# facebookresearch/EgoT2

Measured on AMD Instinct MI355X. Metric: clips/sec fwd+bwd, 3-task TTM translator (B=256,T=15,d=128), higher is better.
Workload: dtype f32 (operands split exactly into 3 bf16 parts; 6 bf16 MFMA products per K-block, f32 accumulate); 1 GPU; configs[1]: TTM 3-task translator, 1 layer d=128 h=4 d_ff=2048, B=256/GPU T=15 S=45, synthetic N(0,1) features, random-init weights, train mode dropout=0.5 (+0.1 on PE), weighted CE (evaluated in the forward's head epilogue), fwd+bwd; global_batch=256, parallelism=dp1, impl=auto, workgroups_per_clip=1, launch=one hipGraph replay per step, deterministic=False, compute_is_module_default=True, loss=weighted CE in the forward's head epilogue (egx_ce)

## Files before the change

### egot2_amd/_lib.py

```python
from __future__ import annotations

import ctypes as C
import os

_PKG = os.path.dirname(os.path.abspath(__file__))
LIB_PATH = os.environ.get("EGX_LIB") or os.path.join(_PKG, "libegot2x.so")

EGX_ABI_VERSION = 18
EGX_MAX_SEGMENTS = 8
EGX_F32, EGX_BF16, EGX_F32_SPLIT = 0, 1, 2
EGX_IMPL_AUTO, EGX_IMPL_GENERIC, EGX_IMPL_FUSED, EGX_IMPL_WIDE, EGX_IMPL_TILED = 0, 1, 2, 3, 4

_fp = C.c_void_p


class Segment(C.Structure):
    _fields_ = [("feat", _fp), ("T", C.c_int), ("d_in", C.c_int), ("proj_w", _fp), ("proj_b", _fp),
                ("add_vec", _fp), ("pos", _fp), ("pos_stride", C.c_int), ("feat_bf16", C.c_int), ("pool", C.c_int)]


class SegmentGrads(C.Structure):
    _fields_ = [("proj_w", _fp), ("proj_b", _fp), ("add_vec", _fp), ("pos", _fp), ("feat", _fp)]


_LAYER_FIELDS = ["in_proj_w", "in_proj_b", "out_proj_w", "out_proj_b", "lin1_w", "lin1_b", "lin2_w", "lin2_b",
                 "norm1_w", "norm1_b", "norm2_w", "norm2_b"]


class Layer(C.Structure):
    _fields_ = [(n, _fp) for n in _LAYER_FIELDS]


class LayerGrads(C.Structure):
    _fields_ = [(n, _fp) for n in _LAYER_FIELDS]


class Head(C.Structure):
    _fields_ = [("ln_w", _fp), ("ln_b", _fp), ("W", _fp), ("b", _fp), ("n_out", C.c_int)]


class HeadGrads(C.Structure):
    _fields_ = [("ln_w", _fp), ("ln_b", _fp), ("W", _fp), ("b", _fp)]


class Config(C.Structure):
    _fields_ = [("d_model", C.c_int), ("n_heads", C.c_int), ("d_ff", C.c_int), ("n_layers", C.c_int),
                ("n_segments", C.c_int), ("ln_eps", C.c_float), ("compute", C.c_int), ("impl", C.c_int),
                ("p_drop", C.c_float), ("p_pos", C.c_float), ("p_feat", C.c_float), ("seed_ptr", _fp),
                ("advance_seed", C.c_int), ("zero_buf", _fp), ("zero_bytes", C.c_size_t), ("bwd_stage", C.c_int),
                ("deterministic", C.c_int), ("out_tokens", C.c_int), ("bucket_cb", C.c_void_p), ("bucket_user", C.c_void_p),
                ("weight_cache", _fp), ("weight_cache_valid", C.c_int), ("d_logits_scale", _fp), ("ce", C.c_void_p),
                ("token_ce", C.c_void_p)]


class Ce(C.Structure):
    _fields_ = [("target", _fp), ("class_weight", _fp), ("loss", _fp), ("d_logits", _fp)]


class TokenCe(C.Structure):
    _fields_ = [("W", _fp), ("b", _fp), ("target", _fp), ("class_weight", _fp), ("C", C.c_int), ("logits", _fp), ("probs", _fp), ("pred", _fp),
                ("loss", _fp), ("correct", _fp), ("d_logits", _fp), ("d_W", _fp), ("d_b", _fp)]


BUCKET_CB = C.CFUNCTYPE(None, C.c_void_p, C.c_int)


class DecConfig(C.Structure):
    _fields_ = [("d_model", C.c_int), ("n_heads", C.c_int), ("d_ff", C.c_int), ("n_layers", C.c_int), ("vocab", C.c_int),
                ("sy", C.c_int), ("S", C.c_int), ("ln_eps", C.c_float), ("compute", C.c_int), ("p_drop", C.c_float),
                ("p_pos", C.c_float), ("seed_ptr", C.c_void_p)]


_DEC_LAYER_FIELDS = ["sa_in_w", "sa_in_b", "sa_out_w", "sa_out_b", "norm1_w", "norm1_b", "ca_in_w", "ca_in_b", "ca_out_w",
                     "ca_out_b", "norm2_w", "norm2_b", "lin1_w", "lin1_b", "lin2_w", "lin2_b", "norm3_w", "norm3_b"]


class DecLayer(C.Structure):
    _fields_ = [(n, _fp) for n in _DEC_LAYER_FIELDS]


class DecLayerGrads(C.Structure):
    _fields_ = [(n, _fp) for n in _DEC_LAYER_FIELDS]


SIGNATURES = {
    "egx_abi_version": (C.c_int, []),
    "egx_last_error": (C.c_char_p, []),
    "egx_launch_count": (C.c_longlong, [C.c_int]),
    "egx_tuning_reload": (None, []),
    "egx_weight_cache_bytes": (C.c_size_t, [C.POINTER(Config), C.POINTER(Segment)]),
    "egx_encoder_workspace": (C.c_int, [C.POINTER(Config), C.POINTER(Segment), C.c_int,
                                        C.POINTER(C.c_size_t), C.POINTER(C.c_size_t)]),
    "egx_encoder_uses_fused": (C.c_int, [C.POINTER(Config), C.POINTER(Segment), C.c_int]),
    "egx_encoder_token_ce_ok": (C.c_int, [C.POINTER(Config), C.POINTER(Segment), C.c_int]),
    "egx_encoder_impl": (C.c_int, [C.POINTER(Config), C.POINTER(Segment), C.c_int]),
    "egx_encoder_slices": (C.c_int, [C.POINTER(Config), C.POINTER(Segment), C.c_int]),
    "egx_wide_gemm_scratch": (C.c_size_t, [C.c_int, C.c_int, C.c_int, C.c_int]),
    "egx_wide_gemm": (C.c_int, [C.c_int, _fp, _fp, _fp, _fp, C.c_int, C.c_int, C.c_int, _fp, C.c_int, _fp, _fp, _fp]),
    "egx_wide_attention_fwd": (C.c_int, [_fp, _fp, _fp, C.c_int, C.c_int, C.c_int, C.c_int, C.c_float, C.c_uint64, _fp]),
    "egx_wide_attention_bwd": (C.c_int, [_fp, _fp, _fp, _fp, _fp, _fp, C.c_int, C.c_int, C.c_int, C.c_int, C.c_float, C.c_uint64, _fp]),
    "egx_encoder_fwd": (C.c_int, [C.POINTER(Config), C.POINTER(Segment), _fp, _fp, C.POINTER(Layer), C.c_int,
                                  _fp, _fp, _fp, C.c_int, C.c_uint64, _fp]),
    "egx_encoder_bwd": (C.c_int, [C.POINTER(Config), C.POINTER(Segment), _fp, _fp, C.POINTER(Layer), C.c_int,
                                  _fp, _fp, _fp, C.POINTER(SegmentGrads), _fp, _fp, C.POINTER(LayerGrads),
                                  C.c_int, C.c_uint64, _fp]),
# ... 142 lines not shown
```

### egot2_amd/csrc/ffn_cut.hip

```cpp
#include <stdlib.h>
#include "common.h"
#include "kernels.h"
#include "fused.h"
#include "fused_dev.h"

namespace egx {

__device__ unsigned long long g_cstamps[32];
#ifdef EGX_STAMPS
#define CSTAMP_INIT() unsigned long long ct_prev = __builtin_amdgcn_s_memtime(), ct_acc[8] = {0, 0, 0, 0, 0, 0, 0, 0}
#define CSTAMP(k) do { __builtin_amdgcn_sched_barrier(0); unsigned long long t_ = __builtin_amdgcn_s_memtime(); ct_acc[k] += t_ - ct_prev; ct_prev = t_; __builtin_amdgcn_sched_barrier(0); } while (0)
#define CSTAMP_FLUSH(base) do { if (blockIdx.x == 0 && (threadIdx.x == 0 || threadIdx.x == 256)) for (int k_ = 0; k_ < 8; ++k_) g_cstamps[(base) + (threadIdx.x >> 8) * 8 + k_] = ct_acc[k_]; } while (0)
#define ASTAMP(i) do { if (blockIdx.x == 0 && threadIdx.x == 0) g_cstamps[i] = __builtin_amdgcn_s_memtime(); } while (0)
#else
#define ASTAMP(i) do { } while (0)
#define CSTAMP_INIT() do { } while (0)
#define CSTAMP(k) do { } while (0)
#define CSTAMP_FLUSH(base) do { } while (0)
#endif
int debug_read_cstamps(unsigned long long* out) {
    return hipMemcpyFromSymbol(out, HIP_SYMBOL(g_cstamps), sizeof(unsigned long long) * 32) == hipSuccess ? 0 : 1;
}
#ifdef EGX_DIAG_NOLOAD
#define RING_REFILL(slot, k, hb, hbn) do { } while (0)
// ... 65 lines not shown
        const int row = i >> 5, c = (i & 31) << 2;
        const f32x4 v = *reinterpret_cast<const f32x4*>(blk + row * LDX + c);
        *reinterpret_cast<uint2*>(plane + row * LDXH + c) = make_uint2(pack_bf16x2(v[0], v[1]), pack_bf16x2(v[2], v[3]));
    }
}
__device__ __forceinline__ void block_to_split_planes(unsigned short* planes, const float* blk) {
    const int row = threadIdx.x >> 2, c0 = (threadIdx.x & 3) * 32;
    if (row < CSP) {
        float g[32];
        uint32_t h[16], m[16], lo[16];
        load32(blk + row * LDX + c0, g);
        split32(g, h, m, lo);
        store_parts32(planes + row * LDXH + c0, (size_t)CPS, h, m, lo);
    }
}

template <int CM, bool FWD>
__device__ __forceinline__ void cut_walk(int wave, int nit, int& j_begin, int& n_mine, int shift_code = 0) {
    const int shift = shift_code ? shift_code - 1 : (CM == CM_BF16 ? 0 : (FWD ? nit / 4 : nit / 8));
    const int n_old = nit + shift;
    j_begin = wave < 4 ? 0 : n_old;
    n_mine = wave < 4 ? n_old : 2 * nit - n_old;
}
constexpr int CP_FLOATS = 1024 + 8 * FD;
constexpr int CP_HEAD_ROWS = 8;
__device__ __forceinline__ int cut_rot(int rot_mode, int clip, int nit) {
    return rot_mode == 0 ? (int)((clip * 11u + (clip >> 3) * 5u) % (unsigned)nit)
         : rot_mode == 4 ? (int)(((unsigned)(clip >> 3) & 3u) % (unsigned)nit)
         : rot_mode == 5 ? (int)(((unsigned)(clip >> 3) & 7u) % (unsigned)nit) : 0;
}

__device__ __forceinline__ void reduce_partials8(f32x4 (&y)[8][CNT], float* blk0, int wave, int r, int q) {
    if (wave >= 4) {
        float* mine = blk0 + (wave - 4) * CBLK;
#pragma unroll
        for (int i = 0; i < 8; ++i)
#pragma unroll
            for (int t = 0; t < CNT; ++t)
                *reinterpret_cast<f32x4*>(mine + (t * 16 + r) * LDX + i * 16 + 4 * q) = y[i][t];
    }
    __syncthreads();
    if (wave < 4) {
        float* mine = blk0 + wave * CBLK;
#pragma unroll
        for (int i = 0; i < 8; ++i)
#pragma unroll
            for (int t = 0; t < CNT; ++t) {
                f32x4* a = reinterpret_cast<f32x4*>(mine + (t * 16 + r) * LDX + i * 16 + 4 * q);
                *a = y[i][t] + *a;
            }
    }
    __syncthreads();
}
}

template <int CM>
__global__ __launch_bounds__(CT) void ffn_fwd_kernel(FusedFwdParams p, int l) {
    extern __shared__ __attribute__((aligned(16))) float lds[];
    float* X1 = lds;
    float* R = lds + CBLK;
    unsigned short* XP = reinterpret_cast<unsigned short*>(R);
    constexpr int NPL = CM == CM_SPLIT ? 3 : 1;
    constexpr int D = RingDepth<CM>::v;
    const int tid = threadIdx.x, wave = tid >> 6, lane = tid & 63, r = lane & 15, q = lane >> 4;
    const int clip = blockIdx.x, S = p.S;
    const size_t tokbase = (size_t)clip * S;
    const FusedLayer& w = p.layer[l];
    const bool dev_seed = p.seed_ptr != nullptr;
    const uint64_t seed_dev = dev_seed ? *p.seed_ptr : 0ull;
    const uint64_t k_ffn = dev_seed ? site_key(seed_dev, l, SITE_FFN) : w.ffn_key;
    const uint64_t k_res2 = dev_seed ? site_key(seed_dev, l, SITE_RES2) : w.res2_key;

    ASTAMP(16);
    Touched tch = {{0, 0, 0, 0}};
    if (p.touch.n) tch = touch_lines<CT>(p.touch, blockIdx.x, gridDim.x, tid);
    const int nhb = p.d_ff / 32;
    int j_begin_, n_mine_;
    cut_walk<CM, true>(wave, nhb / 8, j_begin_, n_mine_, p.rot_mode >> 8);
    const int nit = __builtin_amdgcn_readfirstlane(n_mine_), j_begin = __builtin_amdgcn_readfirstlane(j_begin_);
    const int pair_s = __builtin_amdgcn_readfirstlane(wave & 3);
    const int rot = cut_rot(p.rot_mode & 255, clip, nit);
    auto hb_of = [&](int it) { int j = it + rot; if (j >= nit) j -= nit; return pair_s + 4 * (j_begin + j); };
    float* CP = lds + 5 * CBLK;
    const bool cp_hd = p.head.n_out > 0 && l + 1 == p.n_layers;
    const int cp_g = tid >> 5, cp_c4 = (tid & 31) << 2;
    f32x4 cp_v, cp_w;
    float cp_b;
    {
        const float* src = cp_g == 0 ? w.norm2_w : cp_g == 1 ? w.norm2_b : (cp_g == 3 && cp_hd) ? p.head.ln_w : (cp_g == 4 && cp_hd) ? p.head.ln_b : w.lin2_b;
        cp_v = *reinterpret_cast<const f32x4*>(src + cp_c4);
        const int nb = cp_hd ? p.head.n_out : 0, nw = cp_hd && p.head.n_out <= CP_HEAD_ROWS ? p.head.n_out * 32 : 0;
        cp_b = nb ? p.head.b[min(max(tid - 160, 0), nb - 1)] : 0.f;
        cp_w = *reinterpret_cast<const f32x4*>(nw ? p.head.W + (size_t)min(max(tid - 256, 0), nw - 1) * 4 : w.lin2_b);
    }
    auto cp_store = [&] {
        if (cp_g < 3 || (cp_g < 5 && cp_hd)) *reinterpret_cast<f32x4*>(CP + cp_g * FD + cp_c4) = cp_v;
        if (cp_hd) {
            if (tid >= 160 && tid < 160 + p.head.n_out) CP[5 * FD + (tid - 160)] = cp_b;
            if (p.head.n_out <= CP_HEAD_ROWS && tid >= 256 && tid < 256 + p.head.n_out * 32) *reinterpret_cast<f32x4*>(CP + 1024 + (tid - 256) * 4) = cp_w;
        }
    };
    auto frag_load = [&](int k, int hb) -> WRaw<CM> {
        return k < 8 ? load_w<CM>(w.lin1_wp, hb * 2 + (k & 1), FD / 32, k >> 1, lane) : load_w<CM>(w.lin2_wp, k - 8, nhb, hb, lane);
    };
    WRaw<CM> ring[D];
    float4 b1r[2];
    {
        const int hb0 = hb_of(0);
#pragma unroll
        for (int k = 0; k < D; ++k) ring[k] = frag_load(k, hb0);
#pragma unroll
        for (int i = 0; i < 2; ++i) b1r[i] = *reinterpret_cast<const float4*>(w.lin1_b + hb0 * 32 + i * 16 + 4 * q);
    }
    {
        constexpr int XR = CSP * (FD / 4) / CT;
        constexpr int NPV = CM == CM_F32 ? 1 : (NPL * CSP * (FD / 8) + CT - 1) / CT;
        static_assert(CSP * (FD / 4) % CT == 0, "the x1 block must divide among the threads");
        f32x4 xr[XR];
        u32x4 pv[NPV];
        const f32x4* xs = reinterpret_cast<const f32x4*>(p.x1f_out + ((size_t)l * p.Ntok + tokbase) * FD);
        const int nx = S * (FD / 4);
#pragma unroll
        for (int k = 0; k < XR; ++k) { const int i = tid + CT * k; xr[k] = xs[i < nx ? i : nx - 1]; }
        const bool have_planes = CM != CM_F32 && p.x1p_out != nullptr;
        if constexpr (CM != CM_F32) {
            constexpr int NPIECE = NPL * CSP * (FD / 8);
            const size_t plane = CM == CM_SPLIT ? (size_t)p.B * CSP * FD : 0;
            const unsigned short* src = !have_planes ? reinterpret_cast<const unsigned short*>(p.x1f_out)
                                      : CM == CM_SPLIT ? p.x1p_out + (size_t)l * 3 * plane + (size_t)clip * CSP * FD
                                                       : p.x1p_out + ((size_t)l * p.B + clip) * CSP * FD;
#pragma unroll
            for (int k = 0; k < NPV; ++k) {
                int i = tid + CT * k;
                i = i < NPIECE ? i : NPIECE - 1;
                const int part = i / (CSP * (FD / 8)), rem = i - part * (CSP * (FD / 8));
                pv[k] = *reinterpret_cast<const u32x4*>(src + (have_planes ? part * plane + (size_t)rem * 8 : 0));
            }
        }
        for (int i = tid; i < (CSP - S) * LDX; i += CT) X1[S * LDX + i] = 0.f;
        cp_store();
#pragma unroll
        for (int k = 0; k < XR; ++k) {
            const int i = tid + CT * k, row = i >> 5, c = (i & 31) << 2;
            if (i < nx) *reinterpret_cast<f32x4*>(X1 + row * LDX + c) = xr[k];
        }
        if constexpr (CM != CM_F32) {
            constexpr int NPIECE = NPL * CSP * (FD / 8);
            if (have_planes) {
#pragma unroll
                for (int k = 0; k < NPV; ++k) {
                    const int i = tid + CT * k;
                    const int part = i / (CSP * (FD / 8)), rem = i - part * (CSP * (FD / 8));
                    const int row = rem >> 4, c8 = rem & 15;
                    if (i < NPIECE) {
                        unsigned short* d = XP + part * CPS + row * LDXH + c8 * 8;
                        const bool live = row < S;
                        *reinterpret_cast<uint2*>(d) = live ? make_uint2(pv[k][0], pv[k][1]) : make_uint2(0, 0);
                        *reinterpret_cast<uint2*>(d + 4) = live ? make_uint2(pv[k][2], pv[k][3]) : make_uint2(0, 0);
                    }
                }
            }
        }
        __syncthreads();
        touch_sink(tch);
        if (CM != CM_F32 && !have_planes) {
            if constexpr (CM == CM_SPLIT) block_to_split_planes(XP, X1);
            else if constexpr (CM == CM_BF16) block_to_plane(XP, X1);
            __syncthreads();
        }
    }

    ASTAMP(17);
    f32x4 y[8][CNT];
#pragma unroll
    for (int i = 0; i < 8; ++i)
#pragma unroll
        for (int t = 0; t < CNT; ++t) y[i][t] = f32x4{0, 0, 0, 0};
    const float bscale = w.ffn_thresh ? w.drop_inv : 1.f;
    const size_t bits_base = ((size_t)l * p.B + clip) * nhb * 64 + lane;
    constexpr int ESZ = CM == CM_BF16 ? 2 : 4;
    const int nht = p.d_ff / 16;
    char* const hid_base = (char*)p.hid_out + ((size_t)l * p.B + clip) * CNT * nht * (size_t)(HTILE_ELEMS * ESZ);

    CSTAMP_INIT();
    for (int it = 0; it < nit; ++it) {
        const int hb = hb_of(it);
        const int hbn = hb_of(it + 1 < nit ? it + 1 : it);
        __builtin_amdgcn_sched_barrier(0);
        CSTAMP(0);
        f32x4 hacc[2][CNT];
#pragma unroll
        for (int i = 0; i < 2; ++i)
#pragma unroll
            for (int t = 0; t < CNT; ++t) hacc[i][t] = f32x4{0, 0, 0, 0};
        Frag<CM> xb[CNT];
#pragma unroll
        for (int k = 0; k < 8; ++k) {
            const int i = k & 1, kb = k >> 1;
            if (i == 0) {
#pragma unroll
                for (int t = 0; t < CNT; ++t) xb[t] = operand_frag<CM>(XP, X1, t * 16 + r, kb * 32, q);
            }
            pin(ring[k % D]);
            if (k == 0) { CSTAMP(1); }
            Frag<CM> a = w_frag<CM>(ring[k % D]);
#pragma unroll
            for (int t = 0; t < CNT; ++t) mma<CM>(hacc[i][t], a, xb[t]);
            __builtin_amdgcn_sched_barrier(0);
            RING_REFILL(k % D, k, hb, hbn);
            __builtin_amdgcn_sched_barrier(0);
        }
        CSTAMP(2);
        float bv[2][4];
#pragma unroll
        for (int i = 0; i < 2; ++i) {
            bv[i][0] = b1r[i].x * bscale; bv[i][1] = b1r[i].y * bscale; bv[i][2] = b1r[i].z * bscale; bv[i][3] = b1r[i].w * bscale;
        }
        __builtin_amdgcn_sched_barrier(0);
#pragma unroll
        for (int i = 0; i < 2; ++i) b1r[i] = *reinterpret_cast<const float4*>(w.lin1_b + hbn * 32 + i * 16 + 4 * q);
        __builtin_amdgcn_sched_barrier(0);
        if (w.ffn_thresh) {
#pragma unroll
            for (int i = 0; i < 2; ++i) {
                const uint32_t cq = (uint32_t)(hb * 32 + i * 16 + 4 * q) >> 2;
#pragma unroll
// ... 12 lines not shown
                for (int t = 0; t < CNT; ++t)
#pragma unroll
                    for (int e = 0; e < 4; ++e) hacc[i][t][e] += bv[i][e];
        }
        uint32_t dead = 0;
#pragma unroll
        for (int k = 2 * CNT * 4 - 1; k >= 0; --k) {
            const int i = k / (CNT * 4), t = (k / 4) % CNT, e = k & 3;
            dead = __builtin_amdgcn_alignbit(dead, __float_as_uint(hacc[i][t][e]), 31);
        }
        p.relu_bits[bits_base + (size_t)hb * 64] = ~dead & ((1u << (2 * CNT * 4)) - 1u);
#pragma unroll
        for (int i = 0; i < 2; ++i)
#pragma unroll
            for (int t = 0; t < CNT; ++t)
#pragma unroll
                for (int e = 0; e < 4; ++e) hacc[i][t][e] = __int_as_float(max(__float_as_int(hacc[i][t][e]), 0));
        Frag<CM> hbq[CNT];
#pragma unroll
        for (int t = 0; t < CNT; ++t) hbq[t] = chain_frag<CM>(hacc[0][t], hacc[1][t]);
#ifndef EGX_DIAG_NOSTORE
        {
            char* hb_base = hid_base + (size_t)hb * 2 * (HTILE_ELEMS * ESZ);
#pragma unroll
            for (int t = 0; t < CNT; ++t) {
                if constexpr (CM == CM_BF16) {
                    const u32x4 u = __builtin_bit_cast(u32x4, hbq[t].v);
                    store_hid_tile_bf16(hb_base + (size_t)t * nht * (HTILE_ELEMS * ESZ), u, lane, S - t * 16);
                } else {
#pragma unroll
                    for (int i = 0; i < 2; ++i)
                        store_hid_tile<CM>(hb_base + ((size_t)t * nht + i) * (HTILE_ELEMS * ESZ), hacc[i][t], lane, S - t * 16);
                }
            }
        }
#endif
        __builtin_amdgcn_sched_barrier(0);
        CSTAMP(3);
#pragma unroll
        for (int k = 8; k < 16; ++k) {
            pin(ring[k % D]);
            if (k == 8) { CSTAMP(4); }
            Frag<CM> a = w_frag<CM>(ring[k % D]);
#pragma unroll
            for (int t = 0; t < CNT; ++t) mma<CM>(y[k - 8][t], a, hbq[t]);
            __builtin_amdgcn_sched_barrier(0);
            RING_REFILL(k % D, k, hb, hbn);
            __builtin_amdgcn_sched_barrier(0);
        }
    }
    CSTAMP(5);
    CSTAMP_FLUSH(0);
    ASTAMP(18);
    __syncthreads();
    ASTAMP(19);
    reduce_partials8(y, R, wave, r, q);
    ASTAMP(20);

    for (int i = tid; i < S * (FD / 4); i += CT) {
        const int row = i >> 5, c = (i & 31) << 2, o = row * LDX + c;
        const f32x4 a0 = *reinterpret_cast<const f32x4*>(R + o), a1 = *reinterpret_cast<const f32x4*>(R + CBLK + o);
        const f32x4 a2 = *reinterpret_cast<const f32x4*>(R + 2 * CBLK + o), a3 = *reinterpret_cast<const f32x4*>(R + 3 * CBLK + o);
        f32x4 f = ((a0 + a1) + (a2 + a3)) + *reinterpret_cast<const f32x4*>(CP + 2 * FD + c);
        if (w.res_thresh) {
            float m4[4];
            drop_scale4(k_res2, (uint32_t)(tokbase + row), (uint32_t)c, w.res_thresh, w.drop_inv, m4);
            f = f * f32x4{m4[0], m4[1], m4[2], m4[3]};
        }
        *reinterpret_cast<f32x4*>(X1 + o) = f + *reinterpret_cast<const f32x4*>(X1 + o);
    }
    __syncthreads();
    ASTAMP(21);
    const bool last = l + 1 == p.n_layers;
    float* Y = R;
    ln_rows(X1, S, CP, CP + FD, p.eps, [&](int row, int c0, float (&x)[32], float (&yv)[32]) {
        if (last && p.tokens_out && row < p.out_T) store32(p.tokens_out + ((size_t)clip * p.out_T + row) * FD + c0, yv);
        store32(Y + row * LDX + c0, yv);
    }, [&] { rows_from_lds(p.saved_res + ((size_t)(2 * l + 1) * p.B + clip) * S * FD, X1, S); });
    __syncthreads();
    ASTAMP(22);
    if (!last) {
        rows_from_lds(p.xin_out + ((size_t)(l + 1) * p.B + clip) * S * FD, Y, S);
        return;
    }
    if (p.head.n_out > 0) {
        float* pooled = X1;
        const FusedCe ce{p.ce_target, p.ce_weight, p.ce_loss, p.ce_dlogits, p.ce_B, nullptr};
        CeReq rq;
        if (ce.target) { ce_request_labels<CT>(ce, tid, rq); ce_request_weights(ce, p.head.n_out, rq); }
        if (tid < FD) pooled[tid] = colsum_lds(Y, 0, S, tid) * (1.f / (float)S);
        if (ce.target) ce_weight_partials<CT>(ce, p.head.n_out, tid, rq, pooled + 256);
        __syncthreads();
        if (wave == 0) {
            float2 x = *reinterpret_cast<float2*>(pooled + 2 * lane);
            float mean = wsum(x.x + x.y) * (1.f / FD);
            float dx = x.x - mean, dy = x.y - mean;
            float rstd = rsqrtf(wsum(dx * dx + dy * dy) * (1.f / FD) + p.eps);
            float2 lw = *reinterpret_cast<const float2*>(CP + 3 * FD + 2 * lane);
            float2 lb = *reinterpret_cast<const float2*>(CP + 4 * FD + 2 * lane);
            float y0 = dx * rstd * lw.x + lb.x, y1 = dy * rstd * lw.y + lb.y;
            const bool w_lds = p.head.n_out <= CP_HEAD_ROWS;
            float zmine = 0.f;
            for (int o = 0; o < p.head.n_out; ++o) {
                float2 wv = w_lds ? *reinterpret_cast<const float2*>(CP + 1024 + o * FD + 2 * lane) : *reinterpret_cast<const float2*>(p.head.W + (size_t)o * FD + 2 * lane);
                float sdot = wsum(y0 * wv.x + y1 * wv.y) + CP[5 * FD + o];
                if (lane == 0) p.logits_out[(size_t)clip * p.head.n_out + o] = sdot;
                zmine = lane == o ? sdot : zmine;
            }
            if (ce.target) ce_clip<CT>(ce, p.head.n_out, clip, lane, zmine, pooled + 256, true);
        }
    }
    ASTAMP(23);
}

template <int CM>
__global__ __launch_bounds__(CT) void ffn_bwd_kernel(FusedBwdParams p, int l) {
    extern __shared__ __attribute__((aligned(16))) float lds[];
    float* B1 = lds;
    float* Gs = lds + 1 * CBLK;
    float* B2 = lds + 2 * CBLK;
    float* B3 = lds + 3 * CBLK;
    float* B4 = lds + 4 * CBLK;
    unsigned short* GP = reinterpret_cast<unsigned short*>(B3);
    constexpr int D = RingDepth<CM>::v;
    const int tid = threadIdx.x, wave = tid >> 6, lane = tid & 63, r = lane & 15, q = lane >> 4;
    const int clip = blockIdx.x, S = p.S;
    const size_t tok0 = (size_t)clip * S;
    const FusedBwdLayer& w = p.layer[l];
    const bool dev_seed = p.seed_ptr != nullptr;
    const uint64_t seed_dev = dev_seed ? *p.seed_ptr : 0ull;
    const uint64_t k_res2 = dev_seed ? site_key(seed_dev, l, SITE_RES2) : w.res2_key;
    const bool last = l + 1 == p.n_layers;

    ASTAMP(24);
    Touched tch = {{0, 0, 0, 0}};
    if (p.touch.n) tch = touch_lines<CT>(p.touch, blockIdx.x, gridDim.x, tid);
    if (p.zero_buf) {
        const size_t n4 = p.zero_n / 4, per = (n4 + gridDim.x - 1) / gridDim.x;
        const size_t b0 = (size_t)blockIdx.x * per, b1 = b0 + per < n4 ? b0 + per : n4;
        for (size_t k = b0 + threadIdx.x; k < b1; k += CT) reinterpret_cast<float4*>(p.zero_buf)[k] = make_float4(0, 0, 0, 0);
    }
    float* part = p.partials + (size_t)clip * p.P;
    float* pl = part + l * FUSED_P_LAYER;

    const int nhb = p.d_ff / 32;
    int j_begin_, n_mine_;
    cut_walk<CM, false>(wave, nhb / 8, j_begin_, n_mine_, p.rot_mode >> 8);
    const int nit = __builtin_amdgcn_readfirstlane(n_mine_), j_begin = __builtin_amdgcn_readfirstlane(j_begin_);
    const int pair_s = __builtin_amdgcn_readfirstlane(wave & 3);
    const int rot = cut_rot(p.rot_mode & 255, clip, nit);
    auto hb_of = [&](int it) { int j = it + rot; if (j >= nit) j -= nit; return pair_s + 4 * (j_begin + j); };
    float* CP = lds + 5 * CBLK;
    const bool cp_hd = p.head.n_out > 0 && last;
    const int cp_g = tid >> 5, cp_c4 = (tid & 31) << 2;
    f32x4 cp_v, cp_w;
    float cp_b;
    {
        const float* src = cp_g == 1 ? w.norm2_b : (cp_g == 3 && cp_hd) ? p.head.ln_w : (cp_g == 4 && cp_hd) ? p.head.ln_b : w.norm2_w;
        cp_v = *reinterpret_cast<const f32x4*>(src + cp_c4);
        const int nb = cp_hd ? p.head.n_out : 0, nw = cp_hd && p.head.n_out <= CP_HEAD_ROWS ? p.head.n_out * 32 : 0;
        cp_b = nb ? p.d_logits[(size_t)clip * p.head.n_out + min(max(tid - 160, 0), nb - 1)] : 0.f;
        if (nb && p.d_logits_scale) cp_b *= *p.d_logits_scale;
        cp_w = *reinterpret_cast<const f32x4*>(nw ? p.head.W + (size_t)min(max(tid - 256, 0), nw - 1) * 4 : w.norm2_w);
    }
    auto cp_store = [&] {
        if (cp_g < 2 || ((cp_g == 3 || cp_g == 4) && cp_hd)) *reinterpret_cast<f32x4*>(CP + cp_g * FD + cp_c4) = cp_v;
        if (cp_hd) {
            if (tid >= 160 && tid < 160 + p.head.n_out) CP[5 * FD + 64 + (tid - 160)] = cp_b;
            if (p.head.n_out <= CP_HEAD_ROWS && tid >= 256 && tid < 256 + p.head.n_out * 32) *reinterpret_cast<f32x4*>(CP + 1024 + (tid - 256) * 4) = cp_w;
        }
    };
    auto frag_load = [&](int k, int hb) -> WRaw<CM> {
        return k < 8 ? load_w<CM>(w.lin2_wtp, hb * 2 + (k & 1), FD / 32, k >> 1, lane) : load_w<CM>(w.lin1_wtp, k - 8, nhb, hb, lane);
    };
    const uint32_t* relu_bits = p.relu_bits + ((size_t)l * p.B + clip) * (size_t)nhb * 64 + lane;
    WRaw<CM> ring[D];
    uint32_t relu_word;
    {
        const int hb0 = hb_of(0);
#pragma unroll
        for (int k = 0; k < D; ++k) ring[k] = frag_load(k, hb0);
        relu_word = relu_bits[(size_t)hb0 * 64];
    }
    const float* res2 = p.saved_res + ((size_t)(2 * l + 1) * p.B + clip) * S * FD;
    const bool head_bwd = last && p.head.n_out > 0;
    {
        constexpr int XR = CSP * (FD / 4) / CT;
        f32x4 rr[XR], dr[XR];
        const f32x4* rs = reinterpret_cast<const f32x4*>(res2);
        const int ndy_rows = head_bwd ? 0 : (last ? p.out_T : S);
        const f32x4* ds = head_bwd ? rs : reinterpret_cast<const f32x4*>(last ? p.d_tokens + (size_t)clip * p.out_T * FD : p.dxin + tok0 * FD);
        const int nx = S * (FD / 4), nd = ndy_rows * (FD / 4);
#pragma unroll
        for (int k = 0; k < XR; ++k) {
            const int i = tid + CT * k;
            rr[k] = rs[i < nx ? i : nx - 1];
            dr[k] = ds[i < nd ? i : (nd > 0 ? nd - 1 : 0)];
        }
        for (int i = tid; i < 5 * CBLK / 4; i += CT) reinterpret_cast<f32x4*>(lds)[i] = f32x4{0, 0, 0, 0};
        cp_store();
        __syncthreads();
#pragma unroll
        for (int k = 0; k < XR; ++k) {
            const int i = tid + CT * k, row = i >> 5, c = (i & 31) << 2;
            if (i < nx) {
                *reinterpret_cast<f32x4*>(B1 + row * LDX + c) = rr[k];
                if (head_bwd) *reinterpret_cast<f32x4*>(Gs + row * LDX + c) = rr[k];
            }
            if (i < nd) *reinterpret_cast<f32x4*>(Gs + row * LDX + c) = dr[k];
        }
        touch_sink(tch);
    }
    ASTAMP(25);
    if (head_bwd) {
        float* hp = part + p.head_off;
        __syncthreads();
        ln_rows(Gs, S, CP, CP + FD, p.eps, [&](int row, int c0, float (&x)[32], float (&y)[32]) { store32(Gs + row * LDX + c0, y); });
        __syncthreads();
        float* pooled = B2;
        if (tid < FD) pooled[tid] = colsum_lds(Gs, 0, S, tid) * (1.f / (float)S);
        __syncthreads();
        if (wave == 0) {
            float2 x = *reinterpret_cast<float2*>(pooled + 2 * lane);
            float mean = wsum(x.x + x.y) * (1.f / FD);
            float xh0 = x.x - mean, xh1 = x.y - mean;
            float rstd = rsqrtf(wsum(xh0 * xh0 + xh1 * xh1) * (1.f / FD) + p.eps);
            xh0 *= rstd; xh1 *= rstd;
            float2 lw = *reinterpret_cast<const float2*>(CP + 3 * FD + 2 * lane);
            float2 lb = *reinterpret_cast<const float2*>(CP + 4 * FD + 2 * lane);
            float y0 = xh0 * lw.x + lb.x, y1 = xh1 * lw.y + lb.y;
            float d0 = 0.f, d1 = 0.f;
            const bool w_lds = p.head.n_out <= CP_HEAD_ROWS;
            for (int o = 0; o < p.head.n_out; ++o) {
                float go = CP[5 * FD + 64 + o];
                float2 wv = w_lds ? *reinterpret_cast<const float2*>(CP + 1024 + o * FD + 2 * lane) : *reinterpret_cast<const float2*>(p.head.W + (size_t)o * FD + 2 * lane);
                d0 += go * wv.x; d1 += go * wv.y;
                *reinterpret_cast<float2*>(hp + 256 + FUSED_HEAD_MAX_OUT + o * FD + 2 * lane) = make_float2(go * y0, go * y1);
                if (lane == 0) hp[256 + o] = go;
            }
            *reinterpret_cast<float2*>(hp + 2 * lane) = make_float2(d0 * xh0, d1 * xh1);
            *reinterpret_cast<float2*>(hp + 128 + 2 * lane) = make_float2(d0, d1);
            float g0 = d0 * lw.x, g1 = d1 * lw.y;
            float s1 = wsum(g0 + g1) * (1.f / FD);
            float s2 = wsum(g0 * xh0 + g1 * xh1) * (1.f / FD);
            float inv_s = 1.f / (float)S;
            *reinterpret_cast<float2*>(pooled + 128 + 2 * lane) =
                make_float2(rstd * (g0 - s1 - xh0 * s2) * inv_s, rstd * (g1 - s1 - xh1 * s2) * inv_s);
        }
        __syncthreads();
        f32x4 dp[1];
        {
            const int c = (tid & 31) << 2;
            dp[0] = *reinterpret_cast<const f32x4*>(pooled + 128 + c);
        }
        __syncthreads();
        for (int i = tid; i < S * (FD / 4); i += CT) {
            const int row = i >> 5, c = (i & 31) << 2;
            *reinterpret_cast<f32x4*>(Gs + row * LDX + c) = dp[0];
        }
        if (tid < 64) *reinterpret_cast<f32x4*>(B2 + 4 * tid) = f32x4{0, 0, 0, 0};
    }
    __syncthreads();
    ASTAMP(26);
    ln_bwd_rows(S, CP, p.eps,
        [&](int row, int c0, float (&dy)[32], float (&x)[32]) { load32(Gs + row * LDX + c0, dy); load32(B1 + row * LDX + c0, x); },
        [&](int row, int c0, float (&dy)[32], float (&dx)[32], float (&dyx)[32]) {
            store32(B1 + row * LDX + c0, dx);
            store32(B3 + row * LDX + c0, dyx);
            if (w.res_thresh) {
                const uint32_t orow = (uint32_t)(tok0 + row);
#pragma unroll
                for (int j = 0; j < 32; ++j) dx[j] *= drop_scale(k_res2, orow, (uint32_t)(c0 + j), w.res_thresh, w.drop_inv);
            }
            store32(B2 + row * LDX + c0, dx);
        });
    __syncthreads();
    if (tid < 128) pl[0 + tid] = colsum_lds(B3, 0, S, tid);
    else if (tid < 256) pl[128 + (tid - 128)] = colsum_lds(Gs, 0, S, tid - 128);
    else if (tid < 384) pl[256 + (tid - 256)] = colsum_lds(B2, 0, S, tid - 256);
    if (!(CM != CM_F32 && p.xg_planes)) rows_from_lds(w.g2_out + tok0 * FD, B2, S);
    __syncthreads();
    if constexpr (CM == CM_SPLIT) block_to_split_planes(GP, B2);
    else if constexpr (CM == CM_BF16) block_to_plane(GP, B2);
    __syncthreads();
    if (CM != CM_F32 && p.xg_planes) {
        if constexpr (CM == CM_SPLIT) {
            const size_t plane = (size_t)p.B * CSP * FD;
            planes_from_lds<3>(reinterpret_cast<unsigned short*>(w.g2_out) + (size_t)clip * CSP * FD, plane, GP);
        } else {
            planes_from_lds<1>(reinterpret_cast<unsigned short*>(w.g2_out) + (size_t)clip * CSP * FD, 0, GP);
        }
    }

    ASTAMP(27);
    f32x4 dxa[8][CNT];
#pragma unroll
    for (int i = 0; i < 8; ++i)
#pragma unroll
        for (int t = 0; t < CNT; ++t) dxa[i][t] = f32x4{0, 0, 0, 0};
    constexpr int ESZ = CM == CM_BF16 ? 2 : 4;
    const int nht = p.d_ff / 16;
    char* const dhid_base = (char*)p.dhid_out + ((size_t)l * p.B + clip) * CNT * nht * (size_t)(HTILE_ELEMS * ESZ);
    for (int it = 0; it < nit; ++it) {
        const int hb = hb_of(it);
        const int hbn = hb_of(it + 1 < nit ? it + 1 : it);
        __builtin_amdgcn_sched_barrier(0);
        f32x4 dacc[2][CNT];
#pragma unroll
        for (int i = 0; i < 2; ++i)
#pragma unroll
            for (int t = 0; t < CNT; ++t) dacc[i][t] = f32x4{0, 0, 0, 0};
        Frag<CM> gb[CNT];
#pragma unroll
        for (int k = 0; k < 8; ++k) {
            const int i = k & 1, kb = k >> 1;
            if (i == 0) {
#pragma unroll
                for (int t = 0; t < CNT; ++t) gb[t] = operand_frag<CM>(GP, B2, t * 16 + r, kb * 32, q);
            }
            pin(ring[k % D]);
            Frag<CM> a2 = w_frag<CM>(ring[k % D]);
#pragma unroll
            for (int t = 0; t < CNT; ++t) mma<CM>(dacc[i][t], a2, gb[t]);
            __builtin_amdgcn_sched_barrier(0);
            RING_REFILL(k % D, k, hb, hbn);
            __builtin_amdgcn_sched_barrier(0);
        }
        const uint32_t bits = relu_word;
        __builtin_amdgcn_sched_barrier(0);
        relu_word = relu_bits[(size_t)hbn * 64];
        __builtin_amdgcn_sched_barrier(0);
#pragma unroll
        for (int i = 0; i < 2; ++i)
#pragma unroll
            for (int t = 0; t < CNT; ++t)
#pragma unroll
                for (int e = 0; e < 4; ++e) {
                    const int k = (i * CNT + t) * 4 + e;
                    const int32_t m = ((int32_t)(bits << (31 - k))) >> 31;
                    dacc[i][t][e] = __uint_as_float(__float_as_uint(dacc[i][t][e]) & (uint32_t)m);
                }
        Frag<CM> dq_[CNT];
#pragma unroll
        for (int t = 0; t < CNT; ++t) dq_[t] = chain_frag<CM>(dacc[0][t], dacc[1][t]);
        {
            char* hb_base = dhid_base + (size_t)hb * 2 * (HTILE_ELEMS * ESZ);
#pragma unroll
            for (int t = 0; t < CNT; ++t) {
                if constexpr (CM == CM_BF16) {
                    const u32x4 u = __builtin_bit_cast(u32x4, dq_[t].v);
                    store_hid_tile_bf16(hb_base + (size_t)t * nht * (HTILE_ELEMS * ESZ), u, lane, S - t * 16);
                } else {
#pragma unroll
                    for (int i = 0; i < 2; ++i)
                        store_hid_tile<CM>(hb_base + ((size_t)t * nht + i) * (HTILE_ELEMS * ESZ), dacc[i][t], lane, S - t * 16);
                }
            }
        }
        __builtin_amdgcn_sched_barrier(0);
#pragma unroll
        for (int k = 8; k < 16; ++k) {
            pin(ring[k % D]);
            Frag<CM> a = w_frag<CM>(ring[k % D]);
#pragma unroll
            for (int t = 0; t < CNT; ++t) mma<CM>(dxa[k - 8][t], a, dq_[t]);
            __builtin_amdgcn_sched_barrier(0);
            RING_REFILL(k % D, k, hb, hbn);
            __builtin_amdgcn_sched_barrier(0);
        }
    }
    ASTAMP(28);
    __syncthreads();
    ASTAMP(29);
    reduce_partials8(dxa, Gs, wave, r, q);
    ASTAMP(30);
    {
        f32x4* dst = reinterpret_cast<f32x4*>(p.dy1 + tok0 * FD);
        for (int i = tid; i < S * (FD / 4); i += CT) {
            const int o = (i >> 5) * LDX + ((i & 31) << 2);
            const f32x4 a0 = *reinterpret_cast<const f32x4*>(Gs + o), a1 = *reinterpret_cast<const f32x4*>(B2 + o);
            const f32x4 a2 = *reinterpret_cast<const f32x4*>(B3 + o), a3 = *reinterpret_cast<const f32x4*>(B4 + o);
            dst[i] = (((a0 + a1) + a2) + a3) + *reinterpret_cast<const f32x4*>(B1 + o);
        }
    }
    ASTAMP(31);
}

bool ffn_cut_supported(int d_ff) { return d_ff % 256 == 0 && d_ff >= 256; }
size_t ffn_cut_lds_bytes() { return (size_t)(5 * CBLK + CP_FLOATS) * sizeof(float); }

template <int CM>
static int launch_cut_fwd(const FusedFwdParams& p, int l, hipStream_t st) {
    const size_t lds = ffn_cut_lds_bytes();
    static bool attr_set = false;
    if (!attr_set) {
        EGX_HIP(hipFuncSetAttribute(reinterpret_cast<const void*>(&ffn_fwd_kernel<CM>), hipFuncAttributeMaxDynamicSharedMemorySize, (int)lds));
        attr_set = true;
    }
    timing_begin(TIMER_FFN_FWD, st);
    hipLaunchKernelGGL((ffn_fwd_kernel<CM>), dim3(p.B), dim3(CT), lds, st, p, l);
    timing_end(TIMER_FFN_FWD, st);
    EGX_LAUNCH_CHECK();
    return 0;
}
template <int CM>
static int launch_cut_bwd(const FusedBwdParams& p, int l, hipStream_t st) {
    const size_t lds = ffn_cut_lds_bytes();
    static bool attr_set = false;
    if (!attr_set) {
        EGX_HIP(hipFuncSetAttribute(reinterpret_cast<const void*>(&ffn_bwd_kernel<CM>), hipFuncAttributeMaxDynamicSharedMemorySize, (int)lds));
        attr_set = true;
    }
    timing_begin(TIMER_FFN_BWD, st);
    hipLaunchKernelGGL((ffn_bwd_kernel<CM>), dim3(p.B), dim3(CT), lds, st, p, l);
    timing_end(TIMER_FFN_BWD, st);
    EGX_LAUNCH_CHECK();
    return 0;
}

int ffn_cut_forward(const FusedFwdParams& p, int l, int compute, hipStream_t st) {
    EGX_CHECK(ffn_cut_supported(p.d_ff) && p.S <= CSP && l >= 0 && l < p.n_layers, "ffn_cut_forward: d_ff=%d S=%d layer %d", p.d_ff, p.S, l);
    EGX_CHECK(p.x1f_out && p.xin_out && p.saved_res && p.relu_bits && p.hid_out, "ffn_cut_forward: missing buffers");
    return compute == CM_BF16 ? launch_cut_fwd<CM_BF16>(p, l, st) : compute == CM_SPLIT ? launch_cut_fwd<CM_SPLIT>(p, l, st) : launch_cut_fwd<CM_F32>(p, l, st);
}
int ffn_cut_backward(const FusedBwdParams& p, int l, int compute, hipStream_t st) {
    EGX_CHECK(ffn_cut_supported(p.d_ff) && p.S <= CSP && l >= 0 && l < p.n_layers, "ffn_cut_backward: d_ff=%d S=%d layer %d", p.d_ff, p.S, l);
    EGX_CHECK(p.dy1 && p.saved_res && p.relu_bits && p.dhid_out && p.partials && (l + 1 == p.n_layers || p.dxin), "ffn_cut_backward: missing buffers");
    return compute == CM_BF16 ? launch_cut_bwd<CM_BF16>(p, l, st) : compute == CM_SPLIT ? launch_cut_bwd<CM_SPLIT>(p, l, st) : launch_cut_bwd<CM_F32>(p, l, st);
}

}
```

### egot2_amd/csrc/fused.h

```cpp
#pragma once
#include "common.h"

namespace egx {

constexpr int FUSED_MAX_SEG = 4;
constexpr int FUSED_MAX_LAYERS = 6;

constexpr int TOUCH_MAX = 4;
struct TouchList { const void* base[TOUCH_MAX]; unsigned lines[TOUCH_MAX]; int n; };
static inline void touch_add(TouchList& t, const void* base, size_t bytes) {
    if (base && bytes >= 128 && t.n < TOUCH_MAX) { t.base[t.n] = base; t.lines[t.n] = (unsigned)(bytes >> 7); ++t.n; }
}

struct FusedSeg {
    const float* feat;
    const void* proj_wp;
    const float* proj_b;
    const float* add_vec;
    const float* pos;
    int T, d_in, off, pos_stride;
    int row0, Tfull;
    int seg_id, pad_;
};

// ... 6 lines not shown
    const float* norm2_w; const float* norm2_b;
    uint64_t attn_key, res1_key, ffn_key, res2_key;
    uint32_t attn_thresh, res_thresh, ffn_thresh;
    float drop_inv;
};

struct FusedHead {
    const float* ln_w; const float* ln_b;
    const float* W; const float* b;
    int n_out;
};
constexpr int FUSED_HEAD_MAX_OUT = 64;
static inline int fused_head_partial_len(int n_out) { return n_out > 0 ? 256 + FUSED_HEAD_MAX_OUT + n_out * 128 : 0; }

struct FusedFwdParams {
    FusedSeg seg[FUSED_MAX_SEG];
    FusedLayer layer[FUSED_MAX_LAYERS];
    const float* ln_w; const float* ln_b;
    float eps;
    int nseg, n_layers, B, S, d_ff;
    int rot_mode;
    float* tokens_out;
    int out_T;
    FusedHead head; float* logits_out;
    float* saved_pre;
    float* saved_res;
    uint32_t* relu_bits;
    void* hid_out;
    unsigned short* x1p_out;
    float* xin_out;
    float* qkv_out;
    uint64_t pos_key; uint32_t pos_thresh; float pos_inv;
    const uint64_t* seed_ptr;
    uint64_t feat_key[FUSED_MAX_SEG]; uint32_t feat_thresh; float feat_inv;
    int n_heads;
    int tpc, S_clip;
    size_t Ntok;
    int mode, l0;
    const float* attn_in;
    int n_slices;
    float* xchg;
    unsigned* xflags;
    int slice_drop;
    float* x1f_out;
    const int64_t* ce_target; const float* ce_weight; float* ce_loss; float* ce_dlogits; int ce_B;
    float* zero_word;
    const float* tce_W; const float* tce_b; const int64_t* tce_target; const float* tce_cw; int tce_C;
    float* tce_logits; float* tce_probs; float* tce_pred; float* tce_loss; float* tce_correct; float* tce_dlogits;
    unsigned* tce_ticket;
    unsigned* ce_ticket;
    TouchList touch;
    const int* rtab; int B_clips;
};
enum { FUSED_MODE_FULL = 0, FUSED_MODE_PRE = 1, FUSED_MODE_POST = 2, FUSED_MODE_ATTN = 3 };

struct PackDesc {
    const float* src; void* dst;
    int R, K, ld, transpose, first_block;
    float scale;
};
constexpr int PACK_MAX = 56;
struct PackParams {
    PackDesc d[PACK_MAX];
    int n, mode;
    uint64_t* seed_advance;
    unsigned* zero_words; int n_zero;
    float* zero_word2;
    unsigned* zero_ctl;
};
int pack_weights(PackParams& pp, hipStream_t st);
static inline size_t packed_bytes(int R, int K, int mode) { return (size_t)R * K * (mode == 1 ? 2 : mode == 2 ? 6 : 4); }

struct FfnDwParams {
    const float* x1;
    const float* g;
    const void* w1p;
    const void* w2tp;
    const float* b1;
    int N, S, d_ff;
    uint64_t drop_key; uint32_t drop_thresh; float drop_inv;
    const uint64_t* seed_ptr; int layer;
    const void* hs; const void* dhs; int B;
    int xg_planes;
    float* slab_w1; float* slab_w2t; float* slab_b1;
    int splits, kb_per_split;
};
constexpr int FUSED_TOK_TILES = 3;
constexpr int FUSED_TOK_PAD = FUSED_TOK_TILES * 16;
static inline size_t fused_hid_bytes(int B, int d_ff, int bf16) {
    return (size_t)B * FUSED_TOK_TILES * (d_ff / 16) * 256 * (bf16 ? 2 : 4);
}
size_t ffn_dw_scratch_bytes(int N, int d_ff, int* splits_out);
constexpr int FFN_ROT_XCD_STAGGER = 4;
struct ReducePartialsParams;
constexpr int SLAB_REDUCE_MAX = 3 * FUSED_MAX_LAYERS;
struct SlabReduce { const float* slab[SLAB_REDUCE_MAX]; float* out[SLAB_REDUCE_MAX]; size_t n[SLAB_REDUCE_MAX]; int nslab, narr; };
int ffn_dw(FfnDwParams p, int compute, float* dW1, float* db1, float* dW2, void* slabs, hipStream_t st,
           const ReducePartialsParams* rp = nullptr, bool deterministic = false, SlabReduce* defer = nullptr);
int ffn_dw_reduce(const SlabReduce& a, const ReducePartialsParams* rp, bool deterministic, hipStream_t st);

struct FusedBwdLayer {
    const void* in_proj_wp;
    const void* in_proj_wtp;
    const void* out_proj_wtp;
    const void* lin1_wp;
    const void* lin2_wtp;
    const void* lin1_wtp;
    const float* in_proj_b; const float* lin1_b;
    const float* norm1_w; const float* norm1_b; const float* norm2_w; const float* norm2_b;
    uint64_t attn_key, res1_key, ffn_key, res2_key;
    uint32_t attn_thresh, res_thresh, ffn_thresh;
    float drop_inv;
    float* x1_out; float* g2_out; float* attn_o_out; float* g1_out; float* x_in_out; float* dqkv_out;
};

constexpr int FUSED_P_LAYER = 1152;
static inline int fused_partial_len(int L, int nseg) { return L * FUSED_P_LAYER + 256 + nseg * 256; }

struct FusedBwdParams {
    FusedSeg seg[FUSED_MAX_SEG];
    float* dseg_out[FUSED_MAX_SEG];
    FusedBwdLayer layer[FUSED_MAX_LAYERS];
    const float* ln_w; const float* ln_b;
    float eps;
    int nseg, n_layers, B, S, d_ff;
    int rot_mode;
    const float* d_tokens;
    int out_T;
    FusedHead head; const float* d_logits; int head_off;
    const float* pooled;
    const float* saved_pre;
    const float* saved_res;
    const float* saved_qkv;
    const uint32_t* relu_bits;
    int xg_planes;
    void* dhid_out;
    float* zero_buf; size_t zero_n;
    float* partials; int P;
    uint64_t pos_key; uint32_t pos_thresh; float pos_inv;
    const uint64_t* seed_ptr;
    uint64_t feat_key[FUSED_MAX_SEG]; uint32_t feat_thresh; float feat_inv;
    int n_heads;
    float* dx0_out;
    int tpc, S_clip; size_t Ntok;
    int tiled, l_front, l_back;
    float* datt;
    float* dres;
    int n_slices; float* xchg; unsigned* xflags; int slice_drop;
    int cut, cut_layer;
    float* dy1;
    float* dxin;
    const float* d_logits_scale;
    const float* tce_W; const float* tce_dlogits; int tce_C;
    TouchList touch;
    const int* rtab; int B_clips; const int* rseg;
};
int fused_backward(const FusedBwdParams& p, int compute, hipStream_t st);
bool ffn_cut_supported(int d_ff);
size_t ffn_cut_lds_bytes();
int ffn_cut_forward(const FusedFwdParams& p, int l, int compute, hipStream_t st);
int ffn_cut_backward(const FusedBwdParams& p, int l, int compute, hipStream_t st);

struct SmallDwProblem {
    const float* G; const float* X; float* out;
    int R, C, K, ldg, ldx, first_block, splits;
};
constexpr int SMALL_DW_MAX = 8;
struct SmallDwParams {
    SmallDwProblem pr[SMALL_DW_MAX];
    int n, per;
    float* slabs;
};
int small_dw(SmallDwParams& p, int compute, hipStream_t st, void* slabs = nullptr, size_t slab_bytes = 0, bool reduce_here = true);
int seed_advance(uint64_t* seed, hipStream_t st);

struct PartialDst { float* dst; int off, len; };
constexpr int PARTIAL_MAX_DST = 64;
struct ReducePartialsParams {
    PartialDst d[PARTIAL_MAX_DST];
    int n, B, P;
    const float* partials;
};
int reduce_partials(const ReducePartialsParams& rp, hipStream_t st, bool deterministic = false);
struct SmallDwTail { SlabReduce red; ReducePartialsParams rp; unsigned slab_blocks; int rp_units, chunks; uint64_t* seed_advance;  TouchList touch;  };
int tail_reduce(const SmallDwParams* sp, const SlabReduce* red, const ReducePartialsParams* rp, uint64_t* seed_advance_ptr, const TouchList* touch, hipStream_t st);

enum { TIMER_FUSED_FWD = 0, TIMER_FUSED_BWD = 1, TIMER_FFN_DW = 2, TIMER_FFN_FWD = 3, TIMER_FFN_BWD = 4, TIMER_WIDE_GEMM = 5,
       TIMER_WIDE_ATTN_FWD = 6, TIMER_WIDE_ATTN_BWD = 7, TIMER_COUNT = 8 };
void timing_enable(int on);
void timing_begin(int which, hipStream_t st);
void timing_end(int which, hipStream_t st);
int timing_read(int which, double* total_ms, int* count);

struct TiledAttnParams {
    const float* qkv;
    float* attn_o;
    float* lse;
    const float* d_o;
    float* delta;
    float* dqkv;
    int B, S, tpc;
    uint64_t drop_key; uint32_t drop_thresh; float drop_inv;
    const uint64_t* seed_ptr; int layer;
    const int* rtab;
};
constexpr int TILED_MAX_S = 512;
constexpr int RAGGED_REC = 16;
enum { RG_TILE0 = 0, RG_S = 1, RG_TOK0 = 2, RG_OUT0 = 3, RG_OUTN = 4, RG_T = 5 , RG_OFF = 9  };
static_assert(RG_OFF + FUSED_MAX_SEG <= RAGGED_REC, "ragged clip record");
int upload_words(int* dst, const int* src, size_t n, hipStream_t st);
int ragged_rows(float* padded, float* packed, const int* rtab, const int* rseg, int B, int T_pad, int C, int k, int to_packed, hipStream_t st);
int tiled_attn_fwd(const TiledAttnParams& p, int compute, hipStream_t st);
int tiled_attn_bwd(const TiledAttnParams& p, int compute, hipStream_t st);

bool fused_supported(int d_model, int n_heads, int d_ff, int S, int nseg, const int* d_in, const int* T, const bool* has_proj);
size_t fused_lds_bytes(int NT);
long long slices_stolen_fwd(int reset);
long long slices_stolen_bwd(int reset);
int debug_read_stamps(unsigned long long* out, int n);
int debug_read_bstamps(unsigned long long* out, int n);
int fused_forward(const FusedFwdParams& p, int compute, hipStream_t st);

}
```

### egot2_amd/csrc/fused.hip

```cpp
#include "common.h"
#include "kernels.h"
#include "fused.h"
#include "fused_dev.h"
#include <stdlib.h>
#include <string.h>
#include <type_traits>
#include <vector>

namespace egx {

__global__ __launch_bounds__(64) void pack_weights_kernel(PackParams pp) {
    int blk = blockIdx.x;
    if (pp.seed_advance && blk == 0 && threadIdx.x == 0)
        *pp.seed_advance = *pp.seed_advance * 6364136223846793005ull + 1442695040888963407ull;
    if (pp.zero_words)
        for (int i = blk * 64 + threadIdx.x; i < pp.n_zero; i += gridDim.x * 64) pp.zero_words[i] = 0u;
    if (pp.zero_word2 && blk == 0 && threadIdx.x == 0) *pp.zero_word2 = 0.f;
    if (pp.zero_ctl && blk == 0 && threadIdx.x < 8) pp.zero_ctl[threadIdx.x] = 0u;
    if (pp.n == 0) return;
    int di = 0;
    while (di + 1 < pp.n && blk >= pp.d[di + 1].first_block) ++di;
    const PackDesc& d = pp.d[di];
    int local = blk - d.first_block;
    int nkb = d.K / 32;
// ... 1016 lines not shown
        if (lane == 0) { red[4 + wave] = lterm; red[8 + wave] = cterm; }
        __syncthreads();
        STAMP(13);
        if (tid == 0) {
            const float l = ((red[4] + red[5]) + (red[6] + red[7])) * inv, cn = (red[8] + red[9]) + (red[10] + red[11]);
            float* tacc = reinterpret_cast<float*>(p.tce_ticket + 1);
            atomicAdd(tacc, l);
            __threadfence();
            const unsigned mine = 1u + ((unsigned)cn << 12);
            const unsigned old = atomicAdd(p.tce_ticket, mine);
            if ((old & 4095u) == (unsigned)p.B - 1u) {
                __threadfence();
                *p.tce_loss = atomicExch(tacc, 0.f);
                if (p.tce_correct) *p.tce_correct = (float)((old + mine) >> 12);
                atomicExch(p.tce_ticket, 0u);
            }
        }
        STAMP(14);
    }

    if (!TILED && p.head.n_out > 0) {
        float* pooled = X1;
        const FusedCe ce{p.ce_target, p.ce_weight, p.ce_loss, p.ce_dlogits, p.ce_B, p.ce_ticket};
        CeReq rq;
        if (ce.target) { ce_request_labels<256>(ce, tid, rq); ce_request_weights(ce, p.head.n_out, rq); }
        if (tid < FD) pooled[tid] = colsum_lds(Xs, 0, S, tid) * (1.f / (float)S);
        if (ce.target) ce_weight_partials<256>(ce, p.head.n_out, tid, rq, pooled + 256);
        __syncthreads();
        if (wave == 0) {
            float2 x = *reinterpret_cast<float2*>(pooled + 2 * lane);
            float mean = wsum(x.x + x.y) * (1.f / FD);
            float dx = x.x - mean, dy = x.y - mean;
            float rstd = rsqrtf(wsum(dx * dx + dy * dy) * (1.f / FD) + p.eps);
            float2 lw = *reinterpret_cast<const float2*>(p.head.ln_w + 2 * lane);
            float2 lb = *reinterpret_cast<const float2*>(p.head.ln_b + 2 * lane);
            float y0 = dx * rstd * lw.x + lb.x, y1 = dy * rstd * lw.y + lb.y;
            float zmine = 0.f;
            for (int o = 0; o < p.head.n_out; ++o) {
                float2 wv = *reinterpret_cast<const float2*>(p.head.W + (size_t)o * FD + 2 * lane);
                float sdot = wsum(y0 * wv.x + y1 * wv.y) + p.head.b[o];
                if (lane == 0) p.logits_out[(size_t)clip * p.head.n_out + o] = sdot;
                zmine = lane == o ? sdot : zmine;
            }
            if (ce.target) ce_clip<256>(ce, p.head.n_out, clip, lane, zmine, pooled + 256, slice == 0);
        }
    }
}

namespace {
struct TimerSlot { std::vector<hipEvent_t> a, b; int n = 0; };
TimerSlot g_timers[TIMER_COUNT];
int g_timing_on = 0;
constexpr int TIMER_MAX_EVENTS = 4096;
}
void timing_enable(int on) {
    g_timing_on = on;
    for (int i = 0; i < TIMER_COUNT; ++i) g_timers[i].n = 0;
}
void timing_begin(int which, hipStream_t st) {
    if (!g_timing_on) return;
    TimerSlot& t = g_timers[which];
    if (t.n >= TIMER_MAX_EVENTS) return;
    if ((int)t.a.size() <= t.n) {
        hipEvent_t ea, eb;
        (void)hipEventCreate(&ea); (void)hipEventCreate(&eb);
        t.a.push_back(ea); t.b.push_back(eb);
    }
    (void)hipEventRecord(t.a[t.n], st);
}
void timing_end(int which, hipStream_t st) {
    if (!g_timing_on) return;
    TimerSlot& t = g_timers[which];
    if (t.n < (int)t.a.size() && t.n < TIMER_MAX_EVENTS) { (void)hipEventRecord(t.b[t.n], st); ++t.n; }
}
int timing_read(int which, double* total_ms, int* count) {
    if (which < 0 || which >= TIMER_COUNT) return 1;
    TimerSlot& t = g_timers[which];
    double tot = 0;
    for (int i = 0; i < t.n; ++i) {
        float ms = 0.f;
        if (hipEventSynchronize(t.b[i]) != hipSuccess || hipEventElapsedTime(&ms, t.a[i], t.b[i]) != hipSuccess) return 1;
        tot += ms;
    }
    if (total_ms) *total_ms = tot;
    if (count) *count = t.n;
    return 0;
}

size_t fused_lds_bytes(int NT) {
    int SP = NT * 16;
    return (size_t)(4 * SP * LDX + FD * LDV) * sizeof(float) + FUSED_MAX_SEG * sizeof(FusedSeg) + 16 + 21 * FD * sizeof(float);
}

bool fused_supported(int d_model, int n_heads, int d_ff, int S, int nseg, const int* d_in, const int* T, const bool* has_proj) {
    if (d_model != FD || (n_heads != FH && n_heads != 2 * FH)) return false;
    if (d_ff % 128 != 0 || d_ff < 128) return false;
    if (S < 1 || S > 48) return false;
    for (int i = 0; i < nseg; ++i) {
        if (!has_proj[i]) return false;
        if (d_in[i] % 128 != 0) return false;
        if (T[i] < 1) return false;
    }
    return true;
}

template <int CM, bool TILED, int DH>
static int launch_fwd(const FusedFwdParams& p, hipStream_t st) {
    EGX_CHECK(p.S <= 48, "fused: S=%d unsupported", p.S);
    const size_t lds = fused_lds_bytes(3);
    static bool attr_set = false;
    if (!attr_set) {
        EGX_HIP(hipFuncSetAttribute(reinterpret_cast<const void*>(&fused_fwd_kernel<CM, 3, TILED, DH>), hipFuncAttributeMaxDynamicSharedMemorySize, (int)lds));
        if constexpr (!TILED)
            EGX_HIP(hipFuncSetAttribute(reinterpret_cast<const void*>(&fused_fwd_kernel<CM, 3, false, DH, true>), hipFuncAttributeMaxDynamicSharedMemorySize, (int)lds));
        attr_set = true;
    }
    timing_begin(TIMER_FUSED_FWD, st);
    bool sliced = false;
    if constexpr (!TILED) sliced = p.n_slices > 1;
    if constexpr (!TILED) {
        if (p.mode == FUSED_MODE_ATTN) {
            static bool cut_attr = false;
            if (!cut_attr) {
                EGX_HIP(hipFuncSetAttribute(reinterpret_cast<const void*>(&fused_fwd_kernel<CM, 3, false, DH, false, true>), hipFuncAttributeMaxDynamicSharedMemorySize, (int)lds));
                cut_attr = true;
            }
            EGX_CHECK(!sliced && p.x1f_out, "cut mode: one workgroup per clip, x1f_out set");
            hipLaunchKernelGGL((fused_fwd_kernel<CM, 3, false, DH, false, true>), dim3(p.B), dim3(256), lds, st, p);
            timing_end(TIMER_FUSED_FWD, st);
            EGX_LAUNCH_CHECK();
            return 0;
        }
    }
    if (sliced) {
        if constexpr (!TILED)
            hipLaunchKernelGGL((fused_fwd_kernel<CM, 3, false, DH, true>), dim3((p.B + 7) / 8 * 8 * p.n_slices), dim3(256), lds, st, p);
    } else {
        hipLaunchKernelGGL((fused_fwd_kernel<CM, 3, TILED, DH>), dim3(p.B), dim3(256), lds, st, p);
// ... 53 lines not shown
```

### egot2_amd/csrc/fused_dev.h

```cpp
#pragma once
#include "common.h"
#include "fused.h"

namespace egx {

constexpr int FD = 128;
constexpr int FH = 4;
constexpr int FDH = 32;
constexpr int LDX = FD + 4;
constexpr int LDV = 64 + 4;

enum { CM_F32 = 0, CM_BF16 = 1, CM_SPLIT = 2 };
typedef uint32_t u32x4 __attribute__((ext_vector_type(4)));

template <int CM> struct Frag { float v[8]; };
template <> struct Frag<CM_BF16> { bf16x8 v; };
template <> struct Frag<CM_SPLIT> { bf16x8 p[3]; };

__device__ __forceinline__ uint32_t pack_bf16(float a, float b) { return pack_bf16x2(a, b); }

__device__ __forceinline__ void split_pair(float x, float y, uint32_t& h, uint32_t& m, uint32_t& l) {
    typedef float f32x2 __attribute__((ext_vector_type(2)));
    h = pack_bf16(x, y);
    f32x2 v = {x, y};
// ... 259 lines not shown
        t.v[k] = *reinterpret_cast<const uint32_t*>(reinterpret_cast<const char*>(tl.base[kk]) + ((size_t)i << 7));
    }
    return t;
}
__device__ __forceinline__ void touch_sink(const Touched& t) {
#pragma unroll
    for (int k = 0; k < TOUCH_MAX; ++k) asm volatile("" :: "v"(t.v[k]));
}

__device__ __forceinline__ float wmax(float v) {
#pragma unroll
    for (int o = 32; o > 0; o >>= 1) v = fmaxf(v, __shfl_xor(v, o, 64));
    return v;
}

struct FusedCe {
    const int64_t* target;
    const float* class_weight;
    float* loss;
    float* d_logits;
    int B;
    unsigned* ticket;
};
struct CeReq { int64_t y[2]; float w[2]; };
template <int NTHREADS>
__device__ __forceinline__ void ce_request_labels(const FusedCe& ce, int tid, CeReq& rq) {
#pragma unroll
    for (int k = 0; k < 2; ++k) { const int i = tid + k * NTHREADS; rq.y[k] = ce.target[i < ce.B ? i : ce.B - 1]; }
}
__device__ __forceinline__ void ce_request_weights(const FusedCe& ce, int n_out, CeReq& rq) {
#pragma unroll
    for (int k = 0; k < 2; ++k) {
        const int64_t y = rq.y[k];
        const int yc = (y >= 0 && y < n_out) ? (int)y : 0;
        rq.w[k] = ce.class_weight ? ce.class_weight[yc] : 1.f;
    }
}
template <int NTHREADS>
__device__ __forceinline__ void ce_weight_partials(const FusedCe& ce, int n_out, int tid, const CeReq& rq, float* red) {
    float s = 0.f;
#pragma unroll
    for (int k = 0; k < 2; ++k) {
        const int i = tid + k * NTHREADS;
        s += (i < ce.B && rq.y[k] >= 0 && rq.y[k] < n_out) ? rq.w[k] : 0.f;
    }
    for (int i = tid + 2 * NTHREADS; i < ce.B; i += NTHREADS) {
        const int64_t y = ce.target[i];
        if (y >= 0 && y < n_out) s += ce.class_weight ? ce.class_weight[y] : 1.f;
    }
    s = wsum(s);
    if ((tid & 63) == 0) red[tid >> 6] = s;
}
template <int NTHREADS>
__device__ __forceinline__ void ce_clip(const FusedCe& ce, int n_out, int clip, int lane, float z, const float* red, bool add_loss) {
    float wtot = 0.f;
#pragma unroll
    for (int w = 0; w < NTHREADS / 64; ++w) wtot += red[w];
    const int64_t y = ce.target[clip];
    const bool valid = y >= 0 && y < n_out;
    const float wy = valid ? (ce.class_weight ? ce.class_weight[y] : 1.f) : 0.f;
    const float zl = lane < n_out ? z : -INFINITY;
    const float m = wmax(zl);
    const float e = lane < n_out ? __expf(zl - m) : 0.f;
    const float s = wsum(e);
    const float zy = __shfl(zl, valid ? (int)y : 0, 64);
    const float k = wy / wtot;
    if (lane < n_out) ce.d_logits[(size_t)clip * n_out + lane] = valid ? k * (e / s - (lane == (int)y ? 1.f : 0.f)) : 0.f;
    if (lane == 0 && add_loss) {
        float term = valid ? k * (m + __logf(s) - zy) : 0.f;
        if (wtot == 0.f && clip == 0) term = __builtin_nanf("");
        if (!ce.ticket) {
            atomicAdd(ce.loss, term);
        } else {
            float* acc = reinterpret_cast<float*>(ce.ticket + 1);
            atomicAdd(acc, term);
            __threadfence();
            if (atomicInc(ce.ticket, (unsigned)ce.B - 1u) == (unsigned)ce.B - 1u) {
                __threadfence();
                *ce.loss = atomicExch(acc, 0.f);
            }
        }
    }
}


__device__ __forceinline__ float quad_sum4(float v) {
    v += __shfl_xor(v, 1, 64);
    v += __shfl_xor(v, 2, 64);
    return v;
}
template <class Fn, class Hook>
__device__ __forceinline__ void ln_rows(const float* buf, int S, const float* __restrict__ w, const float* __restrict__ b,
                                        float eps, Fn&& fn, Hook&& after_w) {
    const int row = threadIdx.x >> 2, part = threadIdx.x & 3;
    const int c0 = part * 32;
    f32x4 wq[8], bq[8];
#pragma unroll
    for (int j = 0; j < 8; ++j) {
        wq[j] = *reinterpret_cast<const f32x4*>(w + c0 + 4 * j);
        bq[j] = *reinterpret_cast<const f32x4*>(b + c0 + 4 * j);
    }
    after_w();
    if (row < S) {
        float x[32], y[32];
        float s = 0.f;
#pragma unroll
        for (int j = 0; j < 8; ++j) {
            float4 v = *reinterpret_cast<const float4*>(buf + row * LDX + c0 + 4 * j);
            x[4 * j] = v.x; x[4 * j + 1] = v.y; x[4 * j + 2] = v.z; x[4 * j + 3] = v.w;
            s += (v.x + v.y) + (v.z + v.w);
        }
        float mean = quad_sum4(s) * (1.f / FD);
        float ss = 0.f;
#pragma unroll
        for (int j = 0; j < 32; ++j) { float t = x[j] - mean; ss += t * t; }
        float rstd = rsqrtf(quad_sum4(ss) * (1.f / FD) + eps);
#pragma unroll
        for (int j = 0; j < 8; ++j) {
#pragma unroll
            for (int e = 0; e < 4; ++e) y[4 * j + e] = (x[4 * j + e] - mean) * rstd * wq[j][e] + bq[j][e];
        }
        fn(row, c0, x, y);
    } else {
        (void)quad_sum4(0.f);
        (void)quad_sum4(0.f);
    }
}
template <class Fn>
__device__ __forceinline__ void ln_rows(const float* buf, int S, const float* __restrict__ w, const float* __restrict__ b,
                                        float eps, Fn&& fn) {
    ln_rows(buf, S, w, b, eps, fn, [] {});
}
template <class Fn, class Hook>
__device__ __forceinline__ void ln_rows_lds(const float* buf, int S, const float* wl, const float* bl, float eps, Fn&& fn, Hook&& hook) {
    const int row = threadIdx.x >> 2, part = threadIdx.x & 3;
// ... 310 lines not shown
```

### egot2_amd/csrc/fused_host.hip

```cpp
#include <string.h>
#include <vector>

#include "../../include/egot2x.h"
#include "common.h"
#include "kernels.h"
#include "fused.h"
#include "fused_host.h"

namespace egx {

bool packed_feats(const egx_segment* segs, int nseg) {
    for (int i = 0; i < nseg; ++i)
        if (segs[i].feat_bf16 || segs[i].pool > 1) return true;
    return false;
}
bool fused_ok(const egx_config* cfg, const egx_segment* segs, const Plan& pl) {
    if (pl.nseg > FUSED_MAX_SEG || pl.L > FUSED_MAX_LAYERS || pl.L < 1) return false;
    if (packed_feats(segs, pl.nseg)) return false;
    int d_in[EGX_MAX_SEGMENTS], T[EGX_MAX_SEGMENTS];
    bool hp[EGX_MAX_SEGMENTS];
    for (int i = 0; i < pl.nseg; ++i) { d_in[i] = segs[i].d_in; T[i] = segs[i].T; hp[i] = segs[i].proj_w != nullptr; }
    return fused_supported(pl.d, pl.H, pl.dff, pl.S, pl.nseg, d_in, T, hp);
}
static size_t fused_mask_words(const Plan& pl) { return (size_t)pl.L * pl.vB * (pl.dff / 32) * 64; }
// ... 8 lines not shown
    FusedPackLayout L;
    memset(&L, 0, sizeof(L));
    int bf = cfg->compute;
    size_t cur = 0;
    auto take_p = [&](int R, int K) -> void* { void* q = base ? base + cur : nullptr; cur += align_up(packed_bytes(R, K, bf), 256); return q; };
    for (int i = 0; i < pl.nseg; ++i) L.proj[i] = take_p(pl.d, segs[i].d_in);
    for (int l = 0; l < pl.L && l < FUSED_MAX_LAYERS; ++l) {
        L.layer[l].in_w = take_p(3 * pl.d, pl.d);
        L.layer[l].in_wt = take_p(pl.d, 3 * pl.d);
        L.layer[l].out_w = take_p(pl.d, pl.d);
        L.layer[l].out_wt = take_p(pl.d, pl.d);
        L.layer[l].lin1_w = take_p(pl.dff, pl.d);
        L.layer[l].lin1_wt = take_p(pl.d, pl.dff);
        L.layer[l].lin2_w = take_p(pl.d, pl.dff);
        L.layer[l].lin2_wt = take_p(pl.dff, pl.d);
    }
    L.bytes = cur;
    return L;
}
static char* fused_pack_base(const egx_config* cfg, const void* saved, const Plan& vp) {
    return cfg->weight_cache ? (char*)cfg->weight_cache : (char*)const_cast<void*>(saved) + fused_act_bytes(vp);
}
static size_t fused_hid_total(const egx_config* cfg, const Plan& pl) {
    return align_up((size_t)pl.L * fused_hid_bytes(pl.vB, pl.dff, cfg->compute == EGX_BF16), 256);
}
static size_t fused_hid_offset(const egx_config* cfg, const egx_segment* segs, const Plan& pl) {
    return align_up(fused_act_bytes(pl) + fused_pack_layout(cfg, segs, pl, nullptr).bytes, 256);
}
static bool split_planes(const egx_config* cfg) {
    return cfg->compute == EGX_F32_SPLIT || cfg->compute == EGX_BF16;
}
static size_t plane_elem_bytes(const egx_config* cfg) { return cfg->compute == EGX_BF16 ? 2 : 6; }
static size_t fused_x1p_offset(const egx_config* cfg, const egx_segment* segs, const Plan& pl) {
    return fused_hid_offset(cfg, segs, pl) + fused_hid_total(cfg, pl);
}
static size_t fused_xin_offset(const egx_config* cfg, const egx_segment* segs, const Plan& pl) {
    return fused_x1p_offset(cfg, segs, pl) + (split_planes(cfg) ? align_up((size_t)pl.L * pl.vB * FUSED_TOK_PAD * pl.d * plane_elem_bytes(cfg), 256) : 0);
}
static size_t fused_qkv_offset(const egx_config* cfg, const egx_segment* segs, const Plan& pl) {
    return fused_xin_offset(cfg, segs, pl) + align_up((size_t)pl.L * pl.N * pl.d * 4, 256);
}
static size_t fused_x1f_offset(const egx_config* cfg, const egx_segment* segs, const Plan& pl) {
    return fused_qkv_offset(cfg, segs, pl) + align_up((size_t)pl.L * pl.vB * FUSED_TOK_PAD * 3 * pl.d * 4, 256);
}
static size_t fused_core_bytes(const egx_config* cfg, const egx_segment* segs, const Plan& pl) {
    return fused_x1f_offset(cfg, segs, pl) + (pl.tpc > 1 ? (size_t)0 : align_up((size_t)pl.L * pl.N * pl.d * 4, 256));
}
static bool use_cut(const Plan& pl, int n_slices, bool tiled, int compute) {
    if (tiled || n_slices != 1 || !ffn_cut_supported(pl.dff)) return false;
    if (tuning().ffn_cut >= 0) return tuning().ffn_cut != 0;
    return compute == EGX_F32_SPLIT && pl.L == 1 && pl.dff >= 1024;
}
static int fused_slices_layout(const Plan& pl);
static size_t sliced_xchg_bytes(const Plan& pl, int n);
static size_t sliced_flag_bytes(const Plan& pl, int n);
static size_t fused_saved_bytes(const egx_config* cfg, const egx_segment* segs, const Plan& pl) {
    const int n = (pl.tpc > 1 || pl.S > FUSED_TOK_PAD) ? 1 : fused_slices_layout(pl);
    return fused_core_bytes(cfg, segs, pl) + sliced_xchg_bytes(pl, n) + sliced_flag_bytes(pl, n);
}
static int device_cus() {
    static int cus[64] = {0};
    int dev = 0;
    if (hipGetDevice(&dev) != hipSuccess || dev < 0 || dev >= 64) return 0;
    if (!cus[dev]) {
        int v = 0;
        if (hipDeviceGetAttribute(&v, hipDeviceAttributeMultiprocessorCount, dev) != hipSuccess) return 0;
        cus[dev] = v;
    }
    return cus[dev];
}
static int slice_drop_mask(int n) {
    if (!tuning().has_drop) return 0;
    const int m = (int)tuning().slice_drop & ((1 << n) - 1);
    return m == (1 << n) - 1 ? 0 : m;
}
static bool device_slicing_ok() {
    static int ok[64] = {0};
    int dev = 0;
    if (hipGetDevice(&dev) != hipSuccess || dev < 0 || dev >= 64) return false;
    if (!ok[dev]) {
        hipDeviceProp_t pr;
        ok[dev] = (hipGetDeviceProperties(&pr, dev) == hipSuccess && (strncmp(pr.gcnArchName, "gfx950", 6) == 0 || strncmp(pr.gcnArchName, "gfx942", 6) == 0)) ? 1 : 2;
    }
    return ok[dev] == 1;
}
constexpr int SLICE_LAYOUT_CUS = 304;
static int fused_slices_layout(const Plan& pl) {
    const int nit = pl.dff / 128, bq = (pl.B + 7) / 8 * 8;
    int n = 1;
    while (n * 2 <= 8 && nit % (n * 2) == 0 && bq * n * 2 <= SLICE_LAYOUT_CUS) n *= 2;
    return n;
}
int fused_slices(const Plan& pl, int compute) {
    if (!device_slicing_ok()) return 1;
    const bool e = tuning().has_slices;
    int cap = e ? tuning().slices_cap : (compute == EGX_BF16 ? 4 : 8);
    if (cap < 1) cap = 1;
    const int cus = device_cus(), nit = pl.dff / 128, bq = (pl.B + 7) / 8 * 8;
    int n = 1;
    while (n * 2 <= cap && n * 2 <= 8 && nit % (n * 2) == 0 && bq * n * 2 <= cus) n *= 2;
    if (compute == EGX_BF16 && n == 2 && !e) n = 1;
    const int cap_layout = fused_slices_layout(pl);
    return n < cap_layout ? n : cap_layout;
}
static size_t sliced_xchg_bytes(const Plan& pl, int n) { return n > 1 ? align_up((size_t)pl.L * pl.B * n * FUSED_TOK_PAD * pl.d * 4, 256) : 0; }
static size_t sliced_flag_words(const Plan& pl) { return (size_t)pl.L * pl.B * 8; }
static size_t sliced_flag_bytes(const Plan& pl, int n) { return n > 1 ? align_up(2 * sliced_flag_words(pl) * 4, 256) : 0; }

static void plan_tiled(Plan& pl) { pl.tpc = cdiv(pl.S, FUSED_TOK_PAD); pl.vB = pl.B * pl.tpc; }
static size_t tiled_attn_offset(const egx_config* cfg, const egx_segment* segs, const Plan& vp) { return align_up(fused_saved_bytes(cfg, segs, vp), 256); }
static size_t tiled_lse_offset(const egx_config* cfg, const egx_segment* segs, const Plan& vp) { return tiled_attn_offset(cfg, segs, vp) + align_up((size_t)vp.L * vp.N * vp.d * 4, 256); }
static size_t tiled_tokens_offset(const egx_config* cfg, const egx_segment* segs, const Plan& vp) { return tiled_lse_offset(cfg, segs, vp) + align_up((size_t)vp.L * vp.B * vp.H * vp.S * 4, 256); }
static size_t tiled_saved_bytes(const egx_config* cfg, const egx_segment* segs, const Plan& vp) {
    return tiled_tokens_offset(cfg, segs, vp) + align_up((vp.N + (size_t)vp.B) * vp.d * 4, 256);
}
bool tiled_ok(const egx_config* cfg, const egx_segment* segs, const Plan& pl) {
    if (pl.d != 128 || pl.H != 4 || pl.dff % 128 != 0 || pl.dff < 128) return false;
    if (pl.S <= FUSED_TOK_PAD || pl.S > TILED_MAX_S) return false;
    if (pl.nseg > FUSED_MAX_SEG || pl.L > FUSED_MAX_LAYERS || pl.L < 1) return false;
    if (packed_feats(segs, pl.nseg) || cfg->p_feat > 0.f) return false;
    if (cfg->compute != EGX_BF16 && cfg->compute != EGX_F32_SPLIT) return false;
    if (cfg->out_tokens != 0 && cfg->out_tokens != pl.S) return false;
    for (int i = 0; i < pl.nseg; ++i)
        if (!segs[i].proj_w || segs[i].d_in % 128 != 0) return false;
    return true;
}

struct FusedBwdScratch {
    size_t x1[FUSED_MAX_LAYERS], g2[FUSED_MAX_LAYERS], attn_o[FUSED_MAX_LAYERS], g1[FUSED_MAX_LAYERS], dqkv[FUSED_MAX_LAYERS];
    size_t dseg[EGX_MAX_SEGMENTS];
    size_t partials, slabs, slab_bytes, dhid, bytes, dx0;
    size_t sdw_tiles, sdw_bytes;
    size_t dy1, dxin;
    size_t xchg;
    size_t datt, dres, delta, dtok;
    size_t ffn_slab[FUSED_MAX_LAYERS];
    int P;
};
static size_t bwd_scratch_prefix(FusedBwdScratch& s, const egx_config* cfg, const egx_segment* segs, const Plan& pl, const size_t* seg_rows, int head_n_out) {
    memset(&s, 0, sizeof(s));
    size_t cur = 0;
    const size_t nd = pl.N * pl.d * 4;
    const size_t nd3 = (size_t)pl.vB * FUSED_TOK_PAD * pl.d * 6;
    for (int l = 0; l < pl.L && l < FUSED_MAX_LAYERS; ++l) {
        s.x1[l] = take(cur, nd); s.g2[l] = take(cur, nd3); s.attn_o[l] = take(cur, nd);
        s.g1[l] = take(cur, nd); s.dqkv[l] = take(cur, 3 * nd);
    }
    for (int i = 0; i < pl.nseg; ++i) s.dseg[i] = take(cur, seg_rows[i] * pl.d * 4);
    s.P = fused_partial_len(pl.L, pl.nseg) + fused_head_partial_len(head_n_out);
    s.partials = take(cur, (size_t)pl.vB * s.P * 4);
    size_t slab = ffn_dw_scratch_bytes((int)pl.N, pl.dff, nullptr);
    slab = size_max(slab, gemm_scratch_bytes(2, 3 * pl.d, pl.d, (int)pl.N));
    slab = size_max(slab, gemm_scratch_bytes(2, pl.d, pl.d, (int)pl.N));
    for (int i = 0; i < pl.nseg; ++i) slab = size_max(slab, gemm_scratch_bytes(2, pl.d, segs[i].d_in, (int)seg_rows[i]));
    slab = size_max(slab, (size_t)(512 + SMALL_DW_MAX * 16) * 64 * 128 * sizeof(float));
    s.slab_bytes = slab;
    s.slabs = take(cur, slab);
    s.ffn_slab[0] = s.slabs;
    for (int l = 1; l < pl.L && l < FUSED_MAX_LAYERS; ++l) s.ffn_slab[l] = take(cur, ffn_dw_scratch_bytes((int)pl.N, pl.dff, nullptr));
    s.sdw_bytes = (size_t)(512 + SMALL_DW_MAX * 16) * 64 * 128 * sizeof(float);
    s.sdw_tiles = take(cur, s.sdw_bytes);
    s.dhid = take(cur, fused_hid_total(cfg, pl));
    return cur;
}
static FusedBwdScratch fused_bwd_scratch(const egx_config* cfg, const egx_segment* segs, const Plan& pl, int head_n_out = 0) {
    FusedBwdScratch s;
    size_t seg_rows[EGX_MAX_SEGMENTS];
    for (int i = 0; i < pl.nseg; ++i) seg_rows[i] = (size_t)pl.B * segs[i].T;
    size_t cur = bwd_scratch_prefix(s, cfg, segs, pl, seg_rows, head_n_out);
    const size_t nd = pl.N * pl.d * 4;
    s.dx0 = take(cur, nd);
    s.dy1 = take(cur, nd); s.dxin = take(cur, nd);
    if (pl.tpc > 1 || pl.S > FUSED_TOK_PAD) {
        s.datt = take(cur, nd); s.dres = take(cur, nd);
        s.delta = take(cur, (size_t)pl.B * pl.H * pl.S * 4);
        s.dtok = take(cur, nd);
    } else {
        s.xchg = take(cur, sliced_xchg_bytes(pl, fused_slices_layout(pl)));
    }
    s.bytes = cur;
    return s;
}

struct Packer {
    PackParams& pk;
    bool cache_hit;
    const void* operator()(const float* src, void* dst, int R, int K, int ld, int transpose, float scale = 1.f) {
        if (cache_hit) return dst;
        PackDesc& dsc = pk.d[pk.n++];
        dsc.src = src; dsc.dst = dst; dsc.R = R; dsc.K = K; dsc.ld = ld; dsc.transpose = transpose; dsc.scale = scale;
        return dst;
    }
};
static void fill_seg(FusedSeg& fs, const egx_segment& s, int i, const void* proj_wp = nullptr) {
    if (proj_wp) { fs.feat = s.feat; fs.proj_wp = proj_wp; fs.proj_b = s.proj_b; }
    fs.add_vec = s.add_vec; fs.pos = s.pos; fs.T = s.T; fs.d_in = s.d_in; fs.pos_stride = s.pos_stride;
    fs.Tfull = s.T; fs.seg_id = i;
}
static void fill_layer(FusedLayer& fl, const egx_layer& w, const FusedPackLayout::Layer& P, int d, int dff, float ffn_scale, Packer& pack) {
    fl.in_proj_wp = pack(w.in_proj_w, P.in_w, 3 * d, d, d, 0); fl.in_proj_b = w.in_proj_b;
    fl.out_proj_wp = pack(w.out_proj_w, P.out_w, d, d, d, 0); fl.out_proj_b = w.out_proj_b;
    fl.lin1_wp = pack(w.lin1_w, P.lin1_w, dff, d, d, 0, ffn_scale); fl.lin1_b = w.lin1_b;
    fl.lin2_wp = pack(w.lin2_w, P.lin2_w, d, dff, dff, 0); fl.lin2_b = w.lin2_b;
    pack(w.in_proj_w, P.in_wt, d, 3 * d, d, 1);
    pack(w.out_proj_w, P.out_wt, d, d, d, 1);
    pack(w.lin1_w, P.lin1_wt, d, dff, d, 1);
    pack(w.lin2_w, P.lin2_wt, dff, d, dff, 1, ffn_scale);
    fl.norm1_w = w.norm1_w; fl.norm1_b = w.norm1_b; fl.norm2_w = w.norm2_w; fl.norm2_b = w.norm2_b;
}
static void fill_bwd_layer(FusedBwdLayer& fl, const egx_layer& w, const FusedPackLayout::Layer& P) {
    fl.in_proj_wp = P.in_w; fl.in_proj_wtp = P.in_wt; fl.out_proj_wtp = P.out_wt;
    fl.lin1_wp = P.lin1_w; fl.lin2_wtp = P.lin2_wt; fl.lin1_wtp = P.lin1_wt;
    fl.in_proj_b = w.in_proj_b; fl.lin1_b = w.lin1_b;
    fl.norm1_w = w.norm1_w; fl.norm1_b = w.norm1_b; fl.norm2_w = w.norm2_w; fl.norm2_b = w.norm2_b;
}
template <class LayerT>
static void set_layer_drop(LayerT& fl, int training, float p, uint64_t seed, int l) {
    const Drop da = make_drop(training, p, seed, (uint32_t)l, SITE_ATTN);
    fl.attn_key = da.key; fl.attn_thresh = da.thresh; fl.drop_inv = da.inv_keep;
    fl.res_thresh = da.thresh; fl.ffn_thresh = da.thresh;
    fl.res1_key = make_drop(training, p, seed, (uint32_t)l, SITE_RES1).key;
    fl.ffn_key = make_drop(training, p, seed, (uint32_t)l, SITE_FFN).key;
// ... 189 lines not shown
        const FusedBwdLayer& fl = bp.layer[l];
        TiledAttnParams ap = tiled_attn_params(v, vp, l, bp.saved_qkv, fl.attn_o_out, fl.attn_key, fl.attn_thresh, fl.drop_inv, cfg->seed_ptr);
        ap.d_o = bp.datt; ap.delta = fptr(scratch, SC.delta); ap.dqkv = fl.dqkv_out;
        if (tiled_attn_bwd(ap, comp, st)) return 1;
    }
    bp.l_back = -1; bp.l_front = 0;
    return fused_backward(bp, comp, st);
}

static void partial_dsts(ReducePartialsParams& rp, const FusedBwdParams& bp, const egx_layer_grads* layer_grads, float* d_ln_w, float* d_ln_b,
                         const egx_segment_grads* seg_grads, const egx_head* head, const egx_head_grads* head_grads, const egx_token_ce* tce) {
    memset(&rp, 0, sizeof(rp));
    rp.B = bp.B; rp.P = bp.P; rp.partials = bp.partials;
    auto add_dst = [&](float* dst, int off, int len) { if (dst) { rp.d[rp.n].dst = dst; rp.d[rp.n].off = off; rp.d[rp.n].len = len; ++rp.n; } };
    for (int l = 0; l < bp.n_layers; ++l) {
        const egx_layer_grads& gw = layer_grads[l];
        int o = l * FUSED_P_LAYER;
        add_dst(gw.norm2_w, o + 0, 128); add_dst(gw.norm2_b, o + 128, 128); add_dst(gw.lin2_b, o + 256, 128);
        add_dst(gw.norm1_w, o + 384, 128); add_dst(gw.norm1_b, o + 512, 128); add_dst(gw.out_proj_b, o + 640, 128);
        add_dst(gw.in_proj_b, o + 768, 384);
    }
    const int og = bp.n_layers * FUSED_P_LAYER, oh = fused_partial_len(bp.n_layers, bp.nseg);
    add_dst(d_ln_w, og, 128); add_dst(d_ln_b, og + 128, 128);
    for (int i = 0; i < bp.nseg && seg_grads; ++i) {
        add_dst(seg_grads[i].add_vec, og + 256 + i * 256, 128);
        add_dst(seg_grads[i].proj_b, og + 256 + i * 256 + 128, 128);
    }
    if (head && head->W && head_grads) {
        add_dst(head_grads->ln_w, oh, 128); add_dst(head_grads->ln_b, oh + 128, 128);
        add_dst(head_grads->b, oh + 256, head->n_out);
        add_dst(head_grads->W, oh + 256 + FUSED_HEAD_MAX_OUT, head->n_out * 128);
    }
    if (tce) {
        add_dst(tce->d_b, oh + 256, tce->C);
        add_dst(tce->d_W, oh + 256 + FUSED_HEAD_MAX_OUT, tce->C * 128);
    }
}

static int launch_ffn_dw(int l, const FusedBwdParams& bp, const FusedPackLayout& PL, const FusedBwdScratch& SC, const TiledView& v, const egx_config* cfg,
                         const egx_segment* segs, const Plan& vp, const egx_layer* layers, const egx_layer_grads* layer_grads, void* scratch,
                         SlabReduce& red, hipStream_t st) {
    const egx_layer_grads& gw = layer_grads[l];
    if (!(gw.lin1_w || gw.lin1_b || gw.lin2_w)) return 0;
    const int comp = cfg->compute;
    FfnDwParams fp;
    memset(&fp, 0, sizeof(fp));
    fp.x1 = bp.layer[l].x1_out; fp.g = bp.layer[l].g2_out;
    fp.w1p = PL.layer[l].lin1_w; fp.w2tp = PL.layer[l].lin2_wt; fp.b1 = layers[l].lin1_b;
    fp.N = (int)vp.N; fp.S = vp.S; fp.d_ff = vp.dff;
    fp.drop_key = bp.layer[l].ffn_key; fp.drop_thresh = bp.layer[l].ffn_thresh; fp.drop_inv = bp.layer[l].drop_inv;
    fp.seed_ptr = cfg->seed_ptr; fp.layer = l;
    const size_t lo = (size_t)l * fused_hid_bytes(vp.vB, vp.dff, comp == EGX_BF16);
    fp.hs = v.base + fused_hid_offset(cfg, segs, vp) + lo;
    fp.dhs = (const char*)scratch + SC.dhid + lo;
    fp.B = vp.vB;
    fp.xg_planes = bp.xg_planes;
    if (fp.xg_planes) fp.x1 = (const float*)(v.base + fused_x1p_offset(cfg, segs, vp) + (size_t)l * vp.vB * FUSED_TOK_PAD * vp.d * plane_elem_bytes(cfg));
    return ffn_dw(fp, comp, gw.lin1_w, gw.lin1_b, gw.lin2_w, (char*)scratch + SC.ffn_slab[l], st, nullptr, cfg->deterministic != 0, &red);
}

struct TailArgs { const SlabReduce* red; const ReducePartialsParams* rp; uint64_t* adv; const TouchList* tl; };
struct SmallDwQueue {
    int comp; hipStream_t st;
    void* slabs; size_t slab_bytes;
    const TailArgs* tail;
    SmallDwParams sp;
    bool first;
    SmallDwQueue(int comp_, hipStream_t st_, void* slabs_, size_t slab_bytes_, const TailArgs* tail_)
        : comp(comp_), st(st_), slabs(slabs_), slab_bytes(slab_bytes_), tail(tail_), first(true) { memset(&sp, 0, sizeof(sp)); }
    int flush() {
        if (sp.n && small_dw(sp, comp, st, slabs, slab_bytes, !tail)) return 1;
        const int rc = (tail && (sp.n || first)) ? tail_reduce(sp.n ? &sp : nullptr, first ? tail->red : nullptr, first ? tail->rp : nullptr,
                                                               first ? tail->adv : nullptr, first ? tail->tl : nullptr, st) : 0;
        first = false;
        memset(&sp, 0, sizeof(sp));
        return rc;
    }
    int add(const float* G, int ldg, const float* X, int ldx, float* out, int R, int Cc, int K) {
        if (!out || K <= 0) return 0;
        if (sp.n == SMALL_DW_MAX && flush()) return 1;
        SmallDwProblem& q = sp.pr[sp.n++];
        q.G = G; q.X = X; q.out = out; q.R = R; q.C = Cc; q.K = K; q.ldg = ldg; q.ldx = ldx;
        return 0;
    }
};
static int small_dw_all(SmallDwQueue& q, const FusedBwdParams& bp, const Plan& vp, const egx_layer_grads* layer_grads, const egx_segment* segs,
                        const egx_segment_grads* seg_grads, const float* const* feat, const size_t* seg_rows) {
    const int d = vp.d, N = (int)vp.N;
    for (int l = 0; l < vp.L; ++l) {
        const egx_layer_grads& gw = layer_grads[l];
        if (q.add(bp.layer[l].g1_out, d, bp.layer[l].attn_o_out, d, gw.out_proj_w, d, d, N)) return 1;
        if (q.add(bp.layer[l].dqkv_out, 3 * d, bp.layer[l].x_in_out, d, gw.in_proj_w, 3 * d, d, N)) return 1;
    }
    for (int i = 0; i < vp.nseg && seg_grads; ++i)
        if (q.add(bp.dseg_out[i], d, feat[i], segs[i].d_in, seg_grads[i].proj_w, d, segs[i].d_in, (int)seg_rows[i])) return 1;
    return q.flush();
}

int fused_path_fwd(const egx_config* cfg, const egx_segment* segs, const Plan& pl, bool tiled, const float* ln_w, const float* ln_b,
                   const egx_layer* layers, const egx_head* head, float* tokens_out, float* logits_out, void* saved, int training,
                   uint64_t seed, hipStream_t st) {
    const int d = pl.d, S = pl.S, B = pl.B, comp = cfg->compute;
    const bool with_head = head && head->W;
    const egx_ce* ce = cfg->ce;
    const egx_token_ce* tce = cfg->token_ce;
    Plan vp = pl;
    if (tiled) plan_tiled(vp);
    const TiledView v = uniform_view(cfg, segs, vp, saved, tiled);
    FusedPackLayout PL = fused_pack_layout(cfg, segs, vp, fused_pack_base(cfg, saved, vp));
    FusedFwdParams fp;
    PackParams pk;
    fill_fwd(fp, pk, PL, v, cfg, segs, vp, ln_w, ln_b, layers, training, seed);
    for (int i = 0; i < pl.nseg; ++i) {
        fp.seg[i].off = pl.seg_off[i]; fp.seg[i].row0 = 0;
        Drop df = make_drop(training, cfg->p_feat, seed, (uint32_t)i, SITE_FEAT);
        fp.feat_key[i] = df.key; fp.feat_thresh = df.thresh; fp.feat_inv = df.inv_keep;
    }
    fp.tokens_out = tokens_out;
    fp.out_T = cfg->out_tokens > 0 ? cfg->out_tokens : S;
    if (tiled) {
        if (!fp.tokens_out) fp.tokens_out = (float*)(v.base + v.off_tokens);
        if (pack_weights(pk, st)) return 1;
        return tiled_forward(fp, v, cfg, vp, head, logits_out, st);
    }
    if (with_head) {
        fp.head.ln_w = head->ln_w; fp.head.ln_b = head->ln_b; fp.head.W = head->W; fp.head.b = head->b; fp.head.n_out = head->n_out;
        fp.logits_out = logits_out;
    }
    fp.n_slices = fused_slices(pl, comp);
    if (fp.n_slices > 1) {
        fp.xchg = (float*)((char*)saved + fused_core_bytes(cfg, segs, vp));
        fp.xflags = (unsigned*)((char*)saved + fused_core_bytes(cfg, segs, vp) + sliced_xchg_bytes(pl, fused_slices_layout(pl)));
        pk.zero_words = fp.xflags; pk.n_zero = (int)sliced_flag_words(pl);
        fp.slice_drop = slice_drop_mask(fp.n_slices);
    }
    fp.x1f_out = (float*)((char*)saved + fused_x1f_offset(cfg, segs, vp));
    const bool cut = use_cut(pl, fp.n_slices, false, comp);
    const bool ce_fused = ce && with_head && !cfg->deterministic;
    if (ce_fused) {
        fp.ce_target = ce->target; fp.ce_weight = ce->class_weight; fp.ce_loss = ce->loss; fp.ce_dlogits = ce->d_logits; fp.ce_B = B;
        if (pk.n || pk.seed_advance || pk.zero_words) pk.zero_word2 = ce->loss;
        else if (cut) fp.zero_word = ce->loss;
        else if (cfg->weight_cache) fp.ce_ticket = (unsigned*)((char*)cfg->weight_cache + align_up(PL.bytes, 256));
        else EGX_HIP(hipMemsetAsync(ce->loss, 0, sizeof(float), st));
    }
    if (tce) {
        fp.tce_W = tce->W; fp.tce_b = tce->b; fp.tce_target = tce->target; fp.tce_cw = tce->class_weight; fp.tce_C = tce->C;
        fp.tce_logits = tce->logits; fp.tce_probs = tce->probs; fp.tce_pred = tce->pred; fp.tce_loss = tce->loss; fp.tce_correct = tce->correct;
        fp.tce_dlogits = tce->d_logits;
        fp.tce_ticket = (unsigned*)((char*)cfg->weight_cache + align_up(PL.bytes, 256)) + 4;
    }
    if (pack_weights(pk, st)) return 1;
    const bool touch = cfg->weight_cache != nullptr;
    const size_t ffn_pb = packed_bytes(pl.dff, d, comp), in_pb = packed_bytes(3 * d, d, comp), out_pb = packed_bytes(d, d, comp);
    if (cut) {
        fp.mode = FUSED_MODE_ATTN;
        for (int l = 0; l < pl.L; ++l) {
            fp.l0 = l;
            memset(&fp.touch, 0, sizeof(fp.touch));
            if (touch) { touch_add(fp.touch, PL.layer[l].lin1_w, ffn_pb); touch_add(fp.touch, PL.layer[l].lin2_w, ffn_pb); }
            if (fused_forward(fp, comp, st)) return 1;
            fp.zero_word = nullptr;
            memset(&fp.touch, 0, sizeof(fp.touch));
            if (touch && l + 1 < pl.L) { touch_add(fp.touch, PL.layer[l + 1].in_w, in_pb); touch_add(fp.touch, PL.layer[l + 1].out_w, out_pb); }
            else if (touch && training) { touch_add(fp.touch, PL.layer[l].lin2_wt, ffn_pb); touch_add(fp.touch, PL.layer[l].lin1_wt, ffn_pb); }
            if (ffn_cut_forward(fp, l, comp, st)) return 1;
        }
    } else {
        if (touch) {
            touch_add(fp.touch, PL.layer[0].lin1_w, ffn_pb); touch_add(fp.touch, PL.layer[0].lin2_w, ffn_pb);
            if (training) { touch_add(fp.touch, PL.layer[pl.L - 1].lin2_wt, ffn_pb); touch_add(fp.touch, PL.layer[pl.L - 1].lin1_wt, ffn_pb); }
        }
        if (fused_forward(fp, comp, st)) return 1;
    }
    if (ce && with_head && !ce_fused) return weighted_ce(logits_out, ce->target, ce->class_weight, B, head->n_out, ce->loss, ce->d_logits, st);
    return 0;
}

int fused_path_bwd(const egx_config* cfg, const egx_segment* segs, const Plan& pl, bool tiled, const float* ln_w, const float* ln_b,
                   const egx_layer* layers, const egx_head* head, float* d_tokens, const float* d_logits, const void* saved, void* scratch,
                   const egx_segment_grads* seg_grads, float* d_ln_w, float* d_ln_b, const egx_layer_grads* layer_grads,
                   const egx_head_grads* head_grads, int training, uint64_t seed, hipStream_t st) {
    const int d = pl.d, S = pl.S, B = pl.B, comp = cfg->compute;
    const bool with_head = head && head->W;
    Plan vp = pl;
    if (tiled) plan_tiled(vp);
    const TiledView v = uniform_view(cfg, segs, vp, saved, tiled);
    FusedPackLayout PL = fused_pack_layout(cfg, segs, vp, fused_pack_base(cfg, saved, vp));
    const egx_token_ce* tce = cfg->token_ce;
    if (tce) {
        EGX_CHECK(!with_head && !tiled && fused_token_ce_ok(cfg, pl), "egx_config.token_ce: not on this configuration (egx_encoder_token_ce_ok)");
        EGX_CHECK(tce->W && tce->d_logits && tce->C >= 1 && tce->C <= 8, "egx_config.token_ce: W, d_logits and 1 <= C <= 8 must be set");
    }
    FusedBwdScratch SC = fused_bwd_scratch(cfg, segs, vp, with_head ? head->n_out : tce ? tce->C : 0);
    FusedBwdParams bp;
    if (fill_bwd(bp, PL, SC, v, cfg, segs, vp, ln_w, ln_b, layers, head, d_logits, d_tokens, scratch, training, seed)) return 1;
    const bool touch = cfg->weight_cache != nullptr && !tiled;
    const size_t ffn_pb = packed_bytes(pl.dff, d, comp), in_pb = packed_bytes(3 * d, d, comp), out_pb = packed_bytes(d, d, comp);
    for (int i = 0; i < pl.nseg; ++i) {
        bp.seg[i].off = pl.seg_off[i]; bp.seg[i].row0 = 0;
        Drop df = make_drop(training, cfg->p_feat, seed, (uint32_t)i, SITE_FEAT);
        bp.feat_key[i] = df.key; bp.feat_thresh = df.thresh; bp.feat_inv = df.inv_keep;
    }
    bool want_pos = false;
    for (int i = 0; i < pl.nseg && seg_grads; ++i) want_pos = want_pos || seg_grads[i].pos;
    bp.dx0_out = want_pos ? fptr(scratch, SC.dx0) : nullptr;
    bp.out_T = cfg->out_tokens > 0 ? cfg->out_tokens : S;
    if (tce) {
        bp.tce_W = tce->W; bp.tce_dlogits = tce->d_logits; bp.tce_C = tce->C;
        bp.d_logits_scale = cfg->d_logits_scale;
        bp.head_off = fused_partial_len(pl.L, pl.nseg);
    }
    const int stage = cfg->bwd_stage;
    EGX_CHECK(stage >= 0 && stage <= 2, "bwd_stage=%d", stage);
    if (stage == 2) bp.zero_buf = nullptr;
    if (!tiled) bp.n_slices = fused_slices(pl, comp);
    if (bp.n_slices > 1 && stage != 2) {
        bp.xchg = fptr(scratch, SC.xchg);
        bp.xflags = (unsigned*)((char*)const_cast<void*>(saved) + fused_core_bytes(cfg, segs, vp) + sliced_xchg_bytes(pl, fused_slices_layout(pl))) + sliced_flag_words(pl);
        EGX_HIP(hipMemsetAsync(bp.xflags, 0, sliced_flag_words(pl) * 4, st));
        bp.slice_drop = slice_drop_mask(bp.n_slices);
    }
    if (stage != 2 && tiled) {
        if (tiled_backward(bp, SC, v, cfg, vp, scratch, st)) return 1;
    } else if (stage != 2 && use_cut(pl, bp.n_slices, tiled, comp)) {
        bp.cut = 1; bp.dy1 = fptr(scratch, SC.dy1); bp.dxin = fptr(scratch, SC.dxin);
        for (int l = pl.L - 1; l >= 0; --l) {
            bp.cut_layer = l;
            memset(&bp.touch, 0, sizeof(bp.touch));
            if (touch) { touch_add(bp.touch, PL.layer[l].out_wt, out_pb); touch_add(bp.touch, PL.layer[l].in_wt, in_pb); }
            if (ffn_cut_backward(bp, l, comp, st)) return 1;
            bp.zero_buf = nullptr;
            memset(&bp.touch, 0, sizeof(bp.touch));
            if (touch && l > 0) { touch_add(bp.touch, PL.layer[l - 1].lin2_wt, ffn_pb); touch_add(bp.touch, PL.layer[l - 1].lin1_wt, ffn_pb); }
            if (fused_backward(bp, comp, st)) return 1;
        }
    } else if (stage != 2) {
        if (touch) { touch_add(bp.touch, PL.layer[pl.L - 1].out_wt, out_pb); touch_add(bp.touch, PL.layer[pl.L - 1].in_wt, in_pb); }
        if (fused_backward(bp, comp, st)) return 1;
    }

    for (int i = 0; i < pl.nseg && seg_grads; ++i)
        EGX_CHECK(!seg_grads[i].feat, "fused backward: feature gradients are not supported (use impl=generic)");
    ReducePartialsParams rp;
    partial_dsts(rp, bp, layer_grads, d_ln_w, d_ln_b, seg_grads, head, head_grads, tce);
    if (bp.dx0_out && stage != 2)
        for (int i = 0; i < pl.nseg; ++i)
            if (seg_grads[i].pos && pos_grad_accum(bp.dx0_out, B, S, pl.seg_off[i], segs[i].T, d, seg_grads[i].pos, segs[i].pos_stride, 0, 0, 1.f, st)) return 1;
    bool rp_pending = stage != 2;
    SlabReduce red;
    red.narr = 0; red.nslab = 0;
    for (int l = 0; l < pl.L && stage != 2; ++l)
        if (launch_ffn_dw(l, bp, PL, SC, v, cfg, segs, vp, layers, layer_grads, scratch, red, st)) return 1;
    uint64_t* adv = (cfg->advance_seed == 2 && cfg->seed_ptr && training && stage != 1) ? const_cast<uint64_t*>(cfg->seed_ptr) : nullptr;
    const float* feat[EGX_MAX_SEGMENTS];
    size_t seg_rows[EGX_MAX_SEGMENTS];
    for (int i = 0; i < pl.nseg; ++i) { feat[i] = segs[i].feat; seg_rows[i] = (size_t)(B * segs[i].T); }
    if (stage == 0) {
        TouchList tl;
        memset(&tl, 0, sizeof(tl));
        if (touch) {
            touch_add(tl, PL.proj[0], (size_t)((const char*)PL.layer[0].in_wt - (const char*)PL.proj[0]));
            touch_add(tl, PL.layer[0].out_w, out_pb);
        }
        const TailArgs tail = {&red, &rp, adv, &tl};
        SmallDwQueue q(comp, st, (char*)scratch + SC.sdw_tiles, SC.sdw_bytes, &tail);
        return small_dw_all(q, bp, vp, layer_grads, segs, seg_grads, feat, seg_rows);
    }
    if (red.narr) {
        if (ffn_dw_reduce(red, rp_pending ? &rp : nullptr, cfg->deterministic != 0, st)) return 1;
        rp_pending = false;
    }
    if (rp_pending && reduce_partials(rp, st, cfg->deterministic != 0)) return 1;
    if (stage != 1) {
        SmallDwQueue q(comp, st, cfg->deterministic ? (char*)scratch + SC.slabs : nullptr, SC.slab_bytes, nullptr);
        if (small_dw_all(q, bp, vp, layer_grads, segs, seg_grads, feat, seg_rows)) return 1;
    }
    if (adv && seed_advance(adv, st)) return 1;
    return 0;
}

// ... 249 lines not shown
```

### egot2_amd/functional.py

```python
from __future__ import annotations

import ctypes as C
import dataclasses
from dataclasses import dataclass, field
from typing import List, Optional, Sequence

import torch

from . import _lib
from ._lib import (Ce, Config, Head, HeadGrads, Layer, LayerGrads, Segment, SegmentGrads, check, ptr,
                   EGX_F32, EGX_BF16, EGX_F32_SPLIT, EGX_IMPL_AUTO, EGX_IMPL_GENERIC, EGX_IMPL_FUSED, EGX_IMPL_WIDE, EGX_IMPL_TILED)

COMPUTE = {"f32": EGX_F32, "fp32": EGX_F32, "float32": EGX_F32, "bf16": EGX_BF16, "bfloat16": EGX_BF16, "f32s": EGX_F32_SPLIT}
IMPL = {"auto": EGX_IMPL_AUTO, "generic": EGX_IMPL_GENERIC, "fused": EGX_IMPL_FUSED, "wide": EGX_IMPL_WIDE, "tiled": EGX_IMPL_TILED}


@dataclass
class SegmentSpec:
    T: int
    d_in: int
    has_proj: bool
    add_row: Optional[int] = None
    pos_row0: Optional[int] = None
    pool: int = 1


_weights_epoch = [0]


def note_weights_changed():
    _weights_epoch[0] += 1


class WeightCache:

    def __init__(self, frozen: bool = False):
        self.buf: Optional[torch.Tensor] = None
        self.sig = None
        self.frozen = bool(frozen)
        self.hits = 0
        self.packs = 0

    def invalidate(self):
        self.sig = None


@dataclass
class EncoderSpec:
    d_model: int
    n_heads: int
    d_ff: int
    n_layers: int
    segments: List[SegmentSpec] = field(default_factory=list)
    ln_eps: float = 1e-5
    compute: str = "f32"
    impl: str = "auto"
    p_drop: float = 0.0
    p_pos: float = 0.0
    p_feat: float = 0.0
    training: bool = False
    seed: int = 0
    seed_ptr: int = 0
    head_n_out: int = 0
    advance_seed: int = 0
    defer_small: bool = False
    deterministic: bool = False
    out_tokens: int = 0
    wcache: Optional[WeightCache] = None
    token_ce: int = 0
    ce: bool = False

    def config(self) -> Config:
        return Config(self.d_model, self.n_heads, self.d_ff, self.n_layers, len(self.segments), float(self.ln_eps),
                      COMPUTE[self.compute], IMPL[self.impl], float(self.p_drop), float(self.p_pos), float(self.p_feat),
                      self.seed_ptr or None, int(self.advance_seed) if self.seed_ptr else 0, None, 0, 0,
                      int(bool(self.deterministic)), int(self.out_tokens))


reload_tuning_each_call = False

_scratch_cache = {}
_last_impl = [EGX_IMPL_AUTO]
_last_slices = [1]
IMPL_RAGGED, IMPL_GROUPED = 100, 101
_IMPL_NAMES = {**{v: k for k, v in IMPL.items()}, IMPL_RAGGED: "ragged", IMPL_GROUPED: "grouped"}


def last_encoder_slices() -> int:
    return _last_slices[0]


def last_encoder_impl() -> str:
    return _IMPL_NAMES.get(_last_impl[0], "auto")

_POISON = bool(int(__import__("os").environ.get("EGX_POISON", "0") or 0))


def _workspace(tag: str, device: torch.device, nbytes: int) -> torch.Tensor:
    key = (tag, device.index)
    buf = _scratch_cache.get(key)
    if buf is None or buf.numel() < nbytes:
        buf = torch.empty(max(nbytes, 256), dtype=torch.uint8, device=device)
        _scratch_cache[key] = buf
    if _POISON:
        buf.fill_(255)
    return buf


def _stream() -> int:
    return torch.cuda.current_stream().cuda_stream


def _dev_f32(t: torch.Tensor, name: str) -> torch.Tensor:
    if not t.is_cuda:
        raise _lib.EgxError(f"{name} is on {t.device}: the translator runs only on the GPU through libegot2x.so "
                            "(no CPU fallback)")
    if t.dtype != torch.float32:
        raise _lib.EgxError(f"{name} has dtype {t.dtype}; libegot2x stores activations and weights in fp32")
    return t.contiguous()


def _dev_feat(t: torch.Tensor, name: str) -> torch.Tensor:
    if not t.is_cuda:
# ... 276 lines not shown
    ttgt = ttgt.contiguous()
    t_logits = torch.empty((Mrows, Cn), dtype=torch.float32, device=device)
    t_probs, t_dl = torch.empty_like(t_logits), torch.empty_like(t_logits)
    t_pred = torch.empty((Mrows,), dtype=torch.float32, device=device)
    t_loss = torch.empty((), dtype=torch.float32, device=device)
    t_correct = torch.empty((), dtype=torch.float32, device=device)
    tce_struct = _lib.TokenCe(ptr(tw), ptr(tb), ptr(ttgt), ptr(tcw), Cn, ptr(t_logits), ptr(t_probs), ptr(t_pred), ptr(t_loss),
                              ptr(t_correct), ptr(t_dl), None, None)
    cfg.token_ce = C.cast(C.pointer(tce_struct), C.c_void_p)
    if not lib.egx_encoder_token_ce_ok(C.byref(cfg), segs, B):
        raise _lib.EgxError(refusal)
    return (tw, tb, ttgt, tcw, tce_struct), (t_loss, t_logits, t_probs, t_pred, t_correct), t_dl, tw, tb


class EncoderFn(torch.autograd.Function):

    @staticmethod
    def forward(ctx, spec: EncoderSpec, task_embed, pos_table, ln_w, ln_b, *rest):
        lib = _load()
        nseg = len(spec.segments)
        nhead = 4 if spec.head_n_out else 0
        if spec.token_ce and (nhead or spec.ce):
            raise _lib.EgxError("EncoderSpec.token_ce cannot be combined with the pooled head")
        if spec.ce and not nhead:
            raise _lib.EgxError("EncoderSpec.ce needs the pooled head (head_n_out > 0)")
        feats, proj, layer_t, head_t, tail = _EncArgs.split(spec, rest)
        feats, proj, layer_t, head_t, ln_w, ln_b, task_embed, pos_table = _dev_params(feats, proj, layer_t, head_t, ln_w, ln_b, task_embed,
                                                                                      pos_table)
        assert len(layer_t) == 12 * spec.n_layers, "layer parameter count mismatch"
        d = spec.d_model
        B = feats[0].shape[0]
        device = feats[0].device
        segs = _segments(spec, feats, proj, task_embed, pos_table, B)
        layers = _layers(layer_t, spec.n_layers)

        nig = ctx.needs_input_grad
        if spec.impl == "auto" and (nig[2] or any(nig[5:5 + nseg])):
            feat_grad = [bool(nig[5 + i]) for i in range(nseg)]
            probe_cfg = spec.config()
            wide_ident_only = (lib.egx_encoder_impl(C.byref(probe_cfg), segs, B) == EGX_IMPL_WIDE
                               and not any(fg and ss.has_proj for fg, ss in zip(feat_grad, spec.segments)))
            if any(feat_grad) and not wide_ident_only:
                spec = dataclasses.replace(spec, impl="generic")
        py_slice = 0
        if spec.out_tokens and nhead:
            raise _lib.EgxError("out_tokens (first-tokens-only output) cannot be combined with the fused pooled head: the head pools "
                                "every token of the clip")
        if spec.out_tokens:
            full = dataclasses.replace(spec, out_tokens=0)
            probe = full.config()
            if nhead or lib.egx_encoder_impl(C.byref(probe), segs, B) != EGX_IMPL_FUSED:
                py_slice, spec = spec.out_tokens, full
        cfg = spec.config()
        sv, sc = C.c_size_t(0), C.c_size_t(0)
        ws = lib.egx_translator_workspace if nhead else lib.egx_encoder_workspace
        check(ws(C.byref(cfg), segs, B, C.byref(sv), C.byref(sc)))
        S = sum(s.T for s in spec.segments)
        saved = _saved_buffer(any(nig), "saved", device, sv.value)
        scratch = _workspace("scratch", device, sc.value)
        seed = _seed64(spec.seed)
        wc, wc_sig = _attach_weight_cache(lib, spec, cfg, segs, proj, layer_t, device)
        keep = tw = tb = None
        if spec.ce:
            loss, ctx.ce_dl, keep = _ce_attach(spec, cfg, tail[0], tail[1], B, device)
        if spec.token_ce:
            keep, tce_out, ctx.tce_dl, tw, tb = _token_ce_attach(lib, spec, cfg, segs, tail, wc is not None and not py_slice, B, S, device)
        if nhead:
            head = _head(head_t, spec.head_n_out)
            tokens = torch.empty((B, spec.head_n_out), dtype=torch.float32, device=device)
            check(lib.egx_translator_fwd(C.byref(cfg), segs, ptr(ln_w), ptr(ln_b), layers, C.byref(head), B, ptr(tokens),
                                         None, ptr(saved), ptr(scratch), int(spec.training), seed, _stream()))
        else:
            tokens = torch.empty((B, spec.out_tokens or S, d), dtype=torch.float32, device=device)
            check(lib.egx_encoder_fwd(C.byref(cfg), segs, ptr(ln_w), ptr(ln_b), layers, B, ptr(tokens), ptr(saved),
                                      ptr(scratch), int(spec.training), seed, _stream()))
            if py_slice:
                tokens = tokens[:, :py_slice].contiguous()
        del keep
        if wc is not None:
            wc.sig = wc_sig
        ctx.wcache_buf = wc.buf if wc is not None else None
        ctx.py_slice, ctx.S, ctx.B = py_slice, S, B
        ctx.spec = spec
        ctx.impl = lib.egx_encoder_impl(C.byref(cfg), segs, B)
        _last_impl[0] = ctx.impl
        _last_slices[0] = lib.egx_encoder_slices(C.byref(cfg), segs, B) if ctx.impl == EGX_IMPL_FUSED else 1
        ctx.saved_buf, ctx.scratch_bytes = saved, sc.value
        _EncArgs.save(ctx, task_embed, pos_table, ln_w, ln_b, feats, proj, layer_t, head_t, [t for t in (tw, tb) if t is not None])
        if spec.token_ce:
            ctx.mark_non_differentiable(*tce_out[1:])
            ctx.set_materialize_grads(False)
            return (tokens,) + tce_out
        if spec.ce:
            ctx.set_materialize_grads(False)
            return tokens, loss
        return tokens

    @staticmethod
    def backward(ctx, d_tokens, d_loss=None, *_aux):
        spec: EncoderSpec = ctx.spec
        dl_scale = None
        if spec.token_ce:
            if d_tokens is not None:
                raise _lib.EgxError("EncoderSpec.token_ce: a gradient through the returned tokens as well as through the fused loss is not supported "
                                    "(compose encoder() and linear_cross_entropy() instead)")
            if d_loss is None:
                return (None,) * len(ctx.needs_input_grad)
            dl_scale = _f32c(d_loss)
            d_tokens = ctx.tce_dl
        if spec.ce:
            up = _ce_upstream(ctx, d_tokens, d_loss)
            if up is None:
                return (None,) * len(ctx.needs_input_grad)
            d_tokens, dl_scale = up
        if ctx.py_slice:
            full = torch.zeros((d_tokens.shape[0], ctx.S, d_tokens.shape[2]), dtype=torch.float32, device=d_tokens.device)
            full[:, :ctx.py_slice] = d_tokens
            d_tokens = full
        lib = _load()
        tensors = _EncArgs.load(ctx)
        task_embed, pos_table, ln_w, ln_b, feats, proj, layer_t, head_t, tce_t = tensors
        B = ctx.B
        device = d_tokens.device
        hook = bucket_hook
        gr = _EncGrads(spec, ctx.needs_input_grad, 5, tensors, device, late=hook is None, bucketed=hook is not None)
        pk = gr.pk
        segs, sgr = _segments(spec, feats, proj, task_embed, pos_table, B, grads=gr.segments())
        layers, lgr = _layers(layer_t, spec.n_layers, gr.layers)

        cfg = spec.config()
        gr.attach(cfg)
        if ctx.wcache_buf is not None:
            cfg.weight_cache = ctx.wcache_buf.data_ptr()
        if dl_scale is not None:
            cfg.d_logits_scale = dl_scale.data_ptr()
        tce_keep = None
        if spec.token_ce:
            tce_keep = _lib.TokenCe(ptr(tce_t[0]), None, None, None, int(spec.token_ce), None, None, None, None, None, ptr(ctx.tce_dl),
                                    *map(ptr, (gr.tail + [None])[:2]))
            cfg.token_ce = C.cast(C.pointer(tce_keep), C.c_void_p)
        announced = set()
        cb_keep = None
        if hook is not None and ctx.impl == EGX_IMPL_WIDE:
            flat_for_cb, spans = pk.flat, dict(pk.rank_span)

            cb_error = []

            def _cb(_user, bucket):
                if cb_error or bucket not in spans or bucket in announced:
                    return
                try:
                    hook(flat_for_cb, spans[bucket][0], spans[bucket][1])
                    announced.add(bucket)
                except BaseException as e:
                    cb_error.append(e)
            cb_keep = _lib.BUCKET_CB(_cb)
            cfg.bucket_cb = C.cast(cb_keep, C.c_void_p)
        defer = bool(spec.defer_small) and ctx.impl == EGX_IMPL_FUSED
        cfg.bwd_stage = 1 if defer else 0
        scratch = _workspace("scratch", device, ctx.scratch_bytes)
        seed = _seed64(spec.seed)
        saved_buf = ctx.saved_buf
        p_lnw, p_lnb, flat_buf = ptr(gr.first[2]), ptr(gr.first[3]), pk.flat
        if head_t:
            head, hg = _head(head_t, spec.head_n_out), gr.head_grads()
            dtok = _f32c(d_tokens)

            def launch(c):
                check(lib.egx_translator_bwd(C.byref(c), segs, ptr(ln_w), ptr(ln_b), layers, C.byref(head), B, ptr(dtok),
                                             ptr(saved_buf), ptr(scratch), sgr, p_lnw, p_lnb, lgr,
                                             C.byref(hg), int(spec.training), seed, _stream()))
        else:
            if spec.token_ce:
                dtok = None
            else:
                dtok = _f32c(d_tokens)
                if dtok.data_ptr() == d_tokens.data_ptr() and ctx.impl == EGX_IMPL_GENERIC:
                    dtok = dtok.clone()

            def launch(c):
                check(lib.egx_encoder_bwd(C.byref(c), segs, ptr(ln_w), ptr(ln_b), layers, B, ptr(dtok), ptr(saved_buf),
                                          ptr(scratch), sgr, p_lnw, p_lnb, lgr, int(spec.training), seed,
                                          _stream()))
        launch(cfg)
        del tce_keep
        if cb_keep is not None and cb_error:
            raise cb_error[0]
        if hook is not None and not defer:
            done = sorted(pk.rank_span[b] for b in announced)
            cur = 0
            for lo, hi in done + [(pk.total, pk.total)]:
                if lo > cur:
                    hook(pk.flat, cur, lo)
                cur = max(cur, hi)
        last_grad_layout.update(flat=pk.flat, late_floats=pk.late_floats if defer else 0)
        if defer:
            cfg2 = spec.config()
            cfg2.bwd_stage = 2
            if ctx.wcache_buf is not None:
                cfg2.weight_cache = ctx.wcache_buf.data_ptr()
            keep = (flat_buf, tensors, dtok, scratch, saved_buf)

            def finish(_keep=keep):
                launch(cfg2)
            _deferred.append(finish)
        return gr.result(2 if spec.ce else 4 - len(gr.tail) if spec.token_ce else 0)


def encoder(spec: EncoderSpec, feats: Sequence[torch.Tensor], task_embed, pos_table, ln_w, ln_b,
            proj: Sequence[torch.Tensor], layer_params: Sequence[torch.Tensor],
            head_params: Sequence[torch.Tensor] = (), ce=None):
    if spec.ce:
        return EncoderFn.apply(spec, task_embed, pos_table, ln_w, ln_b, *feats, *proj, *layer_params, *head_params, ce[0], ce[1])
    return EncoderFn.apply(spec, task_embed, pos_table, ln_w, ln_b, *feats, *proj, *layer_params, *head_params)


def ragged_lengths(lengths, B: int, T_pad: Sequence[int], order: Optional[Sequence[int]] = None) -> torch.Tensor:
    K = len(T_pad)
    t = lengths.detach() if isinstance(lengths, torch.Tensor) else torch.as_tensor(lengths)
    if t.dtype.is_floating_point or t.dtype.is_complex or t.dtype == torch.bool:
        raise ValueError(f"lengths must be integers, got {t.dtype}")
    t = t.to("cpu", torch.int64)
    if t.dim() == 1:
        t = t[:, None].expand(t.shape[0], K)
    if t.dim() != 2 or tuple(t.shape) != (B, K):
        raise ValueError(f"lengths has shape {tuple(t.shape)}: expected ({B},) or ({B}, {K}), one column per feature")
    if order is not None:
        t = t[:, list(order)]
    for k in range(K):
        col = t[:, k]
        if B and (int(col.min()) < 1 or int(col.max()) > T_pad[k]):
            raise ValueError(f"lengths of segment {k} must lie in 1 .. {T_pad[k]} (the padded length of its feature), got "
                             f"{int(col.min())} .. {int(col.max())}")
    return t.to(torch.int32).contiguous()


def _check_host_lengths(lengths, B: int, nseg: int) -> torch.Tensor:
    if not isinstance(lengths, torch.Tensor) or lengths.dtype != torch.int32 or lengths.device.type != "cpu" or tuple(lengths.shape) != (B, nseg):
        raise ValueError(f"lengths must be the ({B}, {nseg}) int32 host tensor of ragged_lengths()")
    return lengths.contiguous()


def _length_groups(spec: EncoderSpec, feats, lengths: torch.Tensor, first_only: bool = False):
    groups = {}
    for b, row in enumerate(lengths.tolist()):
        groups.setdefault(tuple(row), []).append(b)
    for key, idx in groups.items():
        it = torch.tensor(idx, dtype=torch.int64, device=feats[0].device)
        fs = [f.index_select(0, it)[:, :T * max(ss.pool, 1)] for f, T, ss in zip(feats, key, spec.segments)]
        gspec = dataclasses.replace(spec, segments=[dataclasses.replace(ss, T=T) for ss, T in zip(spec.segments, key)],
                                    out_tokens=key[0] if first_only else spec.out_tokens)
# ... 1081 lines not shown
```

### egot2_amd/translator.py

```python
from __future__ import annotations

import math
from typing import List, Optional, Sequence

import torch
import torch.nn as nn

from . import functional as F_egx
from .functional import EncoderSpec, SegmentSpec


class PositionalEncoding(nn.Module):

    def __init__(self, d_model, dropout=0.1, max_len=1000):
        super().__init__()
        self.dropout = nn.Dropout(p=dropout)
        pe = torch.zeros(max_len, d_model)
        position = torch.arange(0, max_len, dtype=torch.float).unsqueeze(1)
        div_term = torch.exp(torch.arange(0, d_model, 2).float() * (-math.log(10000.0) / d_model))
        pe[:, 0::2] = torch.sin(position * div_term)
        pe[:, 1::2] = torch.cos(position * div_term)
        pe = pe.unsqueeze(0).transpose(0, 1)
        self.register_buffer('pe', pe)

    def forward(self, x):
        x = x + self.pe[:x.size(0), :]
        return self.dropout(x)


def encoder_layer_tensors(encoder: nn.TransformerEncoder) -> List[torch.Tensor]:
    out = []
    for layer in encoder.layers:
        if getattr(layer, "norm_first", False):
            raise ValueError("libegot2x implements the post-LN encoder layer only (norm_first=False)")
        sa = layer.self_attn
        if sa.in_proj_weight is None:
            raise ValueError("separate q/k/v projection weights are not supported")
        out += [sa.in_proj_weight, sa.in_proj_bias, sa.out_proj.weight, sa.out_proj.bias,
                layer.linear1.weight, layer.linear1.bias, layer.linear2.weight, layer.linear2.bias,
                layer.norm1.weight, layer.norm1.bias, layer.norm2.weight, layer.norm2.bias]
    return out


class TranslatorMixin:

    egx_compute: str = "f32s"
    egx_impl: str = "auto"
    egx_defer_small: bool = False
    egx_deterministic: bool = False
    _egx_step: int = 0

    def set_compute(self, compute: str = "f32", impl: str = "auto"):
        assert compute in F_egx.COMPUTE and impl in F_egx.IMPL
        self.egx_compute, self.egx_impl = compute, impl
        return self

    def set_deterministic(self, on: bool = True):
        self.egx_deterministic = bool(on)
        return self

    def enable_weight_cache(self, frozen: bool = False):
        self._egx_wcache = F_egx.WeightCache(frozen=frozen)
        return self

    def disable_weight_cache(self):
        self._egx_wcache = None
        return self

    def invalidate_weight_cache(self):
        wc = getattr(self, "_egx_wcache", None)
        if wc is not None:
            wc.invalidate()
        return self

    def enable_device_seed(self, device=None):
        dev = device or next(self.parameters()).device
        self._egx_seed_dev = torch.tensor([torch.initial_seed() & (2**62 - 1)], dtype=torch.int64, device=dev)
        return self

    def _egx_seed(self) -> int:
        self._egx_step += 1
        return (torch.initial_seed() * 0x9E3779B97F4A7C15 + self._egx_step * 0xD1B54A32D192ED03) & (2**63 - 1)

    def _egx_spec(self, segments, encoder: nn.TransformerEncoder, ln: nn.LayerNorm, projs, head, **call):
        layer0 = encoder.layers[0]
        spec = EncoderSpec(d_model=ln.normalized_shape[0], n_heads=layer0.self_attn.num_heads, d_ff=layer0.linear1.out_features,
                           n_layers=len(encoder.layers), segments=segments, ln_eps=ln.eps, compute=self.egx_compute, impl=self.egx_impl,
                           head_n_out=head[1].out_features if head is not None else 0, **call)
        proj_t = [t for s, p in zip(segments, projs) if s.has_proj for t in (p.weight, p.bias)]
        head_t = (head[0].weight, head[0].bias, head[1].weight, head[1].bias) if head is not None else ()
        return spec, proj_t, head_t

    def _egx_check_inference(self, what: str, subject: str = "ragged batches are"):
        if self.training:
            raise ValueError(f"{subject} inference-only: call model.eval() before passing {what}")
        if torch.is_grad_enabled() and any(p.requires_grad for p in self.parameters()):
            raise ValueError(f"{subject} inference-only: run them under torch.no_grad() / torch.inference_mode() "
                             "(or with every parameter frozen)")

    def _egx_encode(self, feats: Sequence[torch.Tensor], segments: List[SegmentSpec], *, encoder: nn.TransformerEncoder,
                    ln: nn.LayerNorm, projs: Sequence[Optional[nn.Linear]], task_embed: Optional[torch.Tensor],
                    pos_table: Optional[torch.Tensor], p_drop: float, p_pos: float = 0.0, p_feat: float = 0.0,
                    head=None, out_tokens: int = 0, ce=None, token_ce=None, lengths=None) -> torch.Tensor:
        if lengths is not None:
            return self._egx_encode_ragged(feats, segments, lengths, encoder=encoder, ln=ln, projs=projs, task_embed=task_embed,
                                           pos_table=pos_table, head=head, ce=ce, token_ce=token_ce)
        seed_dev = getattr(self, "_egx_seed_dev", None)
        wcache = getattr(self, "_egx_wcache", None)
        adv = 0 if (seed_dev is None or not self.training) else (2 if (wcache is not None and wcache.frozen and torch.is_grad_enabled()) else 1)
        spec, proj_t, head_t = self._egx_spec(segments, encoder, ln, projs, head, p_drop=p_drop, p_pos=p_pos, p_feat=p_feat,
                                              training=bool(self.training), seed=self._egx_seed() if self.training else 0,
                                              seed_ptr=seed_dev.data_ptr() if seed_dev is not None else 0,
                                              advance_seed=adv,
                                              defer_small=bool(self.egx_defer_small), deterministic=bool(self.egx_deterministic),
                                              out_tokens=int(out_tokens), wcache=wcache, ce=ce is not None)
        if ce is not None and head is None:
            raise ValueError("the fused cross entropy needs the pooled head")
        if token_ce is not None:
            if head is not None or not out_tokens:
                raise ValueError("the token classifier works on the first out_tokens tokens of every clip, without the pooled head")
            return F_egx.encoder_token_ce(spec, list(feats), task_embed, pos_table, ln.weight, ln.bias, proj_t,
                                          encoder_layer_tensors(encoder), *token_ce)
        return F_egx.encoder(spec, list(feats), task_embed, pos_table, ln.weight, ln.bias, proj_t,
                             encoder_layer_tensors(encoder), head_t, ce=ce)

    def _egx_encode_ragged(self, feats, segments, lengths, *, encoder, ln, projs, task_embed, pos_table, head, ce, token_ce):
        self._egx_check_inference("lengths=")
        if ce is not None or token_ce is not None:
            raise ValueError("ragged batches are inference-only: no fused loss (target= / lossav=); apply the loss to the returned outputs")
        lens = F_egx.ragged_lengths(lengths, feats[0].shape[0], [s.T for s in segments])
        spec, proj_t, head_t = self._egx_spec(segments, encoder, ln, projs, head, wcache=getattr(self, "_egx_wcache", None))
        return F_egx.encoder_ragged(spec, list(feats), lens, task_embed, pos_table, ln.weight, ln.bias, proj_t,
                                    encoder_layer_tensors(encoder), head_t)

    def _egx_train_ragged(self, feats, segments, lengths, *, encoder, ln, projs, task_embed, pos_table, p_drop, p_pos=0.0, head=None,
                          ce=None):
        if self.egx_defer_small:
            raise ValueError("ragged training: the staged backward (egx_defer_small) is not supported; clear it for ragged batches")
        if ce is not None and head is None:
            raise ValueError("the fused cross entropy needs the pooled head")
        seed_dev = getattr(self, "_egx_seed_dev", None)
        training = bool(self.training)
        spec, proj_t, head_t = self._egx_spec(segments, encoder, ln, projs, head, p_drop=p_drop, p_pos=p_pos, training=training,
                                              seed=self._egx_seed() if training else 0,
                                              seed_ptr=seed_dev.data_ptr() if seed_dev is not None else 0,
                                              advance_seed=1 if (seed_dev is not None and training) else 0,
                                              deterministic=bool(self.egx_deterministic), ce=ce is not None)
        return F_egx.encoder_ragged_train(spec, list(feats), lengths, task_embed, pos_table, ln.weight, ln.bias, proj_t,
                                          encoder_layer_tensors(encoder), head_t, ce=ce)
```

### include/egot2x.h

```cpp
#ifndef EGOT2X_H
#define EGOT2X_H

#include <stddef.h>
#include <stdint.h>

#ifdef __cplusplus
extern "C" {
#endif

#define EGX_ABI_VERSION 18
#define EGX_MAX_SEGMENTS 8

enum { EGX_F32 = 0, EGX_BF16 = 1, EGX_F32_SPLIT = 2 };
enum { EGX_IMPL_AUTO = 0, EGX_IMPL_GENERIC = 1, EGX_IMPL_FUSED = 2, EGX_IMPL_WIDE = 3, EGX_IMPL_TILED = 4 };

typedef struct egx_segment {
    const float* feat;
    int T;
    int d_in;
    const float* proj_w;
    const float* proj_b;
    const float* add_vec;
    const float* pos;
    int pos_stride;
// ... 17 lines not shown
    const float* lin1_w;
    const float* lin1_b;
    const float* lin2_w;
    const float* lin2_b;
    const float* norm1_w;
    const float* norm1_b;
    const float* norm2_w;
    const float* norm2_b;
} egx_layer;

typedef struct egx_layer_grads {
    float* in_proj_w;
    float* in_proj_b;
    float* out_proj_w;
    float* out_proj_b;
    float* lin1_w;
    float* lin1_b;
    float* lin2_w;
    float* lin2_b;
    float* norm1_w;
    float* norm1_b;
    float* norm2_w;
    float* norm2_b;
} egx_layer_grads;

struct egx_ce;
struct egx_token_ce;
typedef struct egx_config {
    int d_model;
    int n_heads;
    int d_ff;
    int n_layers;
    int n_segments;
    float ln_eps;
    int compute;
    int impl;
    float p_drop;
    float p_pos;
    float p_feat;
    const uint64_t* seed_ptr;
    int advance_seed;
    void* zero_buf;
    size_t zero_bytes;
    int bwd_stage;
    int deterministic;
    int out_tokens;
    void (*bucket_cb)(void* user, int bucket);
    void* bucket_user;
    void* weight_cache;
    int weight_cache_valid;
    const float* d_logits_scale;
    const struct egx_ce* ce;
    const struct egx_token_ce* token_ce;
} egx_config;

typedef struct egx_ce {
    const int64_t* target;
    const float* class_weight;
    float* loss;
    float* d_logits;
} egx_ce;

typedef struct egx_token_ce {
    const float* W;
    const float* b;
    const int64_t* target;
    const float* class_weight;
    int C;
    float* logits;
    float* probs;
    float* pred;
    float* loss;
    float* correct;
    float* d_logits;
    float* d_W; float* d_b;
} egx_token_ce;

int egx_abi_version(void);
int egx_encoder_token_ce_ok(const egx_config* cfg, const egx_segment* segs, int B);
void egx_tuning_reload(void);
size_t egx_weight_cache_bytes(const egx_config* cfg, const egx_segment* segs);
long long egx_launch_count(int reset);
const char* egx_last_error(void);

int egx_encoder_workspace(const egx_config* cfg, const egx_segment* segs, int B,
                          size_t* saved_bytes, size_t* scratch_bytes);

int egx_encoder_uses_fused(const egx_config* cfg, const egx_segment* segs, int B);
int egx_encoder_impl(const egx_config* cfg, const egx_segment* segs, int B);
int egx_encoder_slices(const egx_config* cfg, const egx_segment* segs, int B);

int egx_encoder_fwd(const egx_config* cfg, const egx_segment* segs,
                    const float* ln_w, const float* ln_b,
                    const egx_layer* layers, int B,
                    float* tokens_out, void* saved, void* scratch,
                    int training, uint64_t seed, void* stream);

int egx_encoder_bwd(const egx_config* cfg, const egx_segment* segs,
                    const float* ln_w, const float* ln_b,
                    const egx_layer* layers, int B,
                    float* d_tokens, const void* saved, void* scratch,
                    const egx_segment_grads* seg_grads, float* d_ln_w, float* d_ln_b,
                    const egx_layer_grads* layer_grads,
                    int training, uint64_t seed, void* stream);

typedef struct egx_head {
// ... 187 lines not shown
```

Before: 702,100 clips/s.

## Speculatively run last-layer FFN backward inside the forward FFN kernel

Adds a fused ffn_fwd_bwd kernel for the last layer. After the forward FFN, LN and head with fused CE, the same kernel computes the head backward and the FFN/LN backward tail, using the CE gradient produced in the epilogue. It writes g2, d_hidden tiles, dy1 and partials into saved buffers, and the backward skips that stage when the upstream loss gradient is the default. This removes one kernel launch and re-reading of activations and weights. In exchange the forward does more work and holds more registers, and the speculated results are only valid when the loss scale is unmodified.

```diff
diff --git a/egot2_amd/_lib.py b/egot2_amd/_lib.py
--- a/egot2_amd/_lib.py
+++ b/egot2_amd/_lib.py
@@ -50,7 +50,8 @@
                 ("advance_seed", C.c_int), ("zero_buf", _fp), ("zero_bytes", C.c_size_t), ("bwd_stage", C.c_int),
                 ("deterministic", C.c_int), ("out_tokens", C.c_int), ("bucket_cb", C.c_void_p), ("bucket_user", C.c_void_p),
                 ("weight_cache", _fp), ("weight_cache_valid", C.c_int), ("d_logits_scale", _fp), ("ce", C.c_void_p),
-                ("token_ce", C.c_void_p)]
+                ("token_ce", C.c_void_p),
+                ("speculate_bwd", C.c_int), ("spec_done", C.c_int)]
 
 
 class Ce(C.Structure):
diff --git a/egot2_amd/csrc/ffn_cut.hip b/egot2_amd/csrc/ffn_cut.hip
--- a/egot2_amd/csrc/ffn_cut.hip
+++ b/egot2_amd/csrc/ffn_cut.hip
@@ -141,10 +141,200 @@
     }
     __syncthreads();
 }
-}
-
-template <int CM>
-__global__ __launch_bounds__(CT) void ffn_fwd_kernel(FusedFwdParams p, int l) {
+struct CutBwd {
+    const void* lin2_wtp; const void* lin1_wtp;
+    const uint32_t* relu_bits;
+    float* g2_out;
+    char* dhid_base;
+    float* dy1;
+    float* pl;
+    int S, clip, B, nhb, xg_planes;
+    int nit, j_begin, pair_s, rot;
+    size_t tok0;
+    uint64_t k_res2; uint32_t res_thresh; float drop_inv, eps;
+    __device__ __forceinline__ int hb_of(int it) const { int j = it + rot; if (j >= nit) j -= nit; return pair_s + 4 * (j_begin + j); }
+};
+template <int CM>
+__device__ __forceinline__ void cut_bwd_walk(CutBwd& c, int wave, int rot_mode) {
+    int j_begin_, n_mine_;
+    cut_walk<CM, false>(wave, c.nhb / 8, j_begin_, n_mine_, rot_mode >> 8);
+    c.nit = __builtin_amdgcn_readfirstlane(n_mine_); c.j_begin = __builtin_amdgcn_readfirstlane(j_begin_);
+    c.pair_s = __builtin_amdgcn_readfirstlane(wave & 3);
+    c.rot = cut_rot(rot_mode & 255, c.clip, c.nit);
+}
+template <int CM>
+__device__ __forceinline__ WRaw<CM> cut_bwd_frag(const CutBwd& c, int k, int hb, int lane) {
+    return k < 8 ? load_w<CM>(c.lin2_wtp, hb * 2 + (k & 1), FD / 32, k >> 1, lane) : load_w<CM>(c.lin1_wtp, k - 8, c.nhb, hb, lane);
+}
+template <int CM>
+__device__ __forceinline__ void cut_bwd_prime(const CutBwd& c, WRaw<CM> (&ring)[RingDepth<CM>::v], uint32_t& relu_word, int lane) {
+    const int hb0 = c.hb_of(0);
+#pragma unroll
+    for (int k = 0; k < RingDepth<CM>::v; ++k) ring[k] = cut_bwd_frag<CM>(c, k, hb0, lane);
+    relu_word = c.relu_bits[(size_t)hb0 * 64];
+}
+template <class Go>
+__device__ __forceinline__ void cut_head_bwd(const FusedHead& head, const float* CP, float* hp, float* dpooled, int S, int lane,
+                                             float xh0, float xh1, float rstd, float2 lw, float y0, float y1, Go&& go_of) {
+    float d0 = 0.f, d1 = 0.f;
+    const bool w_lds = head.n_out <= CP_HEAD_ROWS;
+    for (int o = 0; o < head.n_out; ++o) {
+        float go = go_of(o);
+        float2 wv = w_lds ? *reinterpret_cast<const float2*>(CP + 1024 + o * FD + 2 * lane) : *reinterpret_cast<const float2*>(head.W + (size_t)o * FD + 2 * lane);
+        d0 += go * wv.x; d1 += go * wv.y;
+        *reinterpret_cast<float2*>(hp + 256 + FUSED_HEAD_MAX_OUT + o * FD + 2 * lane) = make_float2(go * y0, go * y1);
+        if (lane == 0) hp[256 + o] = go;
+    }
+    *reinterpret_cast<float2*>(hp + 2 * lane) = make_float2(d0 * xh0, d1 * xh1);
+    *reinterpret_cast<float2*>(hp + 128 + 2 * lane) = make_float2(d0, d1);
+    float g0 = d0 * lw.x, g1 = d1 * lw.y;
+    float s1 = wsum(g0 + g1) * (1.f / FD);
+    float s2 = wsum(g0 * xh0 + g1 * xh1) * (1.f / FD);
+    float inv_s = 1.f / (float)S;
+    *reinterpret_cast<float2*>(dpooled + 2 * lane) =
+        make_float2(rstd * (g0 - s1 - xh0 * s2) * inv_s, rstd * (g1 - s1 - xh1 * s2) * inv_s);
+}
+template <int CM>
+__device__ __forceinline__ void cut_bwd_tail(const CutBwd& c, float* lds, WRaw<CM> (&ring)[RingDepth<CM>::v], uint32_t relu_word, int tid) {
+    float* B1 = lds;
+    float* Gs = lds + 1 * CBLK;
+    float* B2 = lds + 2 * CBLK;
+    float* B3 = lds + 3 * CBLK;
+    float* B4 = lds + 4 * CBLK;
+    float* CP = lds + 5 * CBLK;
+    unsigned short* GP = reinterpret_cast<unsigned short*>(B3);
+    constexpr int D = RingDepth<CM>::v;
+    const int wave = tid >> 6, lane = tid & 63, r = lane & 15, q = lane >> 4;
+    const int S = c.S, nit = c.nit;
+    float* pl = c.pl;
+    auto frag_load = [&](int k, int hb) -> WRaw<CM> { return cut_bwd_frag<CM>(c, k, hb, lane); };
+    ln_bwd_rows(S, CP, c.eps,
+        [&](int row, int c0, float (&dy)[32], float (&x)[32]) { load32(Gs + row * LDX + c0, dy); load32(B1 + row * LDX + c0, x); },
+        [&](int row, int c0, float (&dy)[32], float (&dx)[32], float (&dyx)[32]) {
+            store32(B1 + row * LDX + c0, dx);
+            store32(B3 + row * LDX + c0, dyx);
+            if (c.res_thresh) {
+                const uint32_t orow = (uint32_t)(c.tok0 + row);
+#pragma unroll
+                for (int j = 0; j < 32; ++j) dx[j] *= drop_scale(c.k_res2, orow, (uint32_t)(c0 + j), c.res_thresh, c.drop_inv);
+            }
+            store32(B2 + row * LDX + c0, dx);
+        });
+    __syncthreads();
+    if (tid < 128) pl[0 + tid] = colsum_lds(B3, 0, S, tid);
+    else if (tid < 256) pl[128 + (tid - 128)] = colsum_lds(Gs, 0, S, tid - 128);
+    else if (tid < 384) pl[256 + (tid - 256)] = colsum_lds(B2, 0, S, tid - 256);
+    if (!(CM != CM_F32 && c.xg_planes)) rows_from_lds(c.g2_out + c.tok0 * FD, B2, S);
+    __syncthreads();
+    if constexpr (CM == CM_SPLIT) block_to_split_planes(GP, B2);
+    else if constexpr (CM == CM_BF16) block_to_plane(GP, B2);
+    __syncthreads();
+    if (CM != CM_F32 && c.xg_planes) {
+        if constexpr (CM == CM_SPLIT) {
+            const size_t plane = (size_t)c.B * CSP * FD;
+            planes_from_lds<3>(reinterpret_cast<unsigned short*>(c.g2_out) + (size_t)c.clip * CSP * FD, plane, GP);
+        } else {
+            planes_from_lds<1>(reinterpret_cast<unsigned short*>(c.g2_out) + (size_t)c.clip * CSP * FD, 0, GP);
+        }
+    }
+
+    ASTAMP(27);
+    f32x4 dxa[8][CNT];
+#pragma unroll
+    for (int i = 0; i < 8; ++i)
+#pragma unroll
+        for (int t = 0; t < CNT; ++t) dxa[i][t] = f32x4{0, 0, 0, 0};
+    constexpr int ESZ = CM == CM_BF16 ? 2 : 4;
+    const int nht = c.nhb * 2;
+    char* const dhid_base = c.dhid_base;
+    for (int it = 0; it < nit; ++it) {
+        const int hb = c.hb_of(it);
+        const int hbn = c.hb_of(it + 1 < nit ? it + 1 : it);
+        __builtin_amdgcn_sched_barrier(0);
+        f32x4 dacc[2][CNT];
+#pragma unroll
+        for (int i = 0; i < 2; ++i)
+#pragma unroll
+            for (int t = 0; t < CNT; ++t) dacc[i][t] = f32x4{0, 0, 0, 0};
+        Frag<CM> gb[CNT];
+#pragma unroll
+        for (int k = 0; k < 8; ++k) {
+            const int i = k & 1, kb = k >> 1;
+            if (i == 0) {
+#pragma unroll
+                for (int t = 0; t < CNT; ++t) gb[t] = operand_frag<CM>(GP, B2, t * 16 + r, kb * 32, q);
+            }
+            pin(ring[k % D]);
+            Frag<CM> a2 = w_frag<CM>(ring[k % D]);
+#pragma unroll
+            for (int t = 0; t < CNT; ++t) mma<CM>(dacc[i][t], a2, gb[t]);
+            __builtin_amdgcn_sched_barrier(0);
+            RING_REFILL(k % D, k, hb, hbn);
+            __builtin_amdgcn_sched_barrier(0);
+        }
+        const uint32_t bits = relu_word;
+        __builtin_amdgcn_sched_barrier(0);
+        relu_word = c.relu_bits[(size_t)hbn * 64];
+        __builtin_amdgcn_sched_barrier(0);
+#pragma unroll
+        for (int i = 0; i < 2; ++i)
+#pragma unroll
+            for (int t = 0; t < CNT; ++t)
+#pragma unroll
+                for (int e = 0; e < 4; ++e) {
+                    const int k = (i * CNT + t) * 4 + e;
+                    const int32_t m = ((int32_t)(bits << (31 - k))) >> 31;
+                    dacc[i][t][e] = __uint_as_float(__float_as_uint(dacc[i][t][e]) & (uint32_t)m);
+                }
+        Frag<CM> dq_[CNT];
+#pragma unroll
+        for (int t = 0; t < CNT; ++t) dq_[t] = chain_frag<CM>(dacc[0][t], dacc[1][t]);
+        {
+            char* hb_base = dhid_base + (size_t)hb * 2 * (HTILE_ELEMS * ESZ);
+#pragma unroll
+            for (int t = 0; t < CNT; ++t) {
+                if constexpr (CM == CM_BF16) {
+                    const u32x4 u = __builtin_bit_cast(u32x4, dq_[t].v);
+                    store_hid_tile_bf16(hb_base + (size_t)t * nht * (HTILE_ELEMS * ESZ), u, lane, S - t * 16);
+                } else {
+#pragma unroll
+                    for (int i = 0; i < 2; ++i)
+                        store_hid_tile<CM>(hb_base + ((size_t)t * nht + i) * (HTILE_ELEMS * ESZ), dacc[i][t], lane, S - t * 16);
+                }
+            }
+        }
+        __builtin_amdgcn_sched_barrier(0);
+#pragma unroll
+        for (int k = 8; k < 16; ++k) {
+            pin(ring[k % D]);
+            Frag<CM> a = w_frag<CM>(ring[k % D]);
+#pragma unroll
+            for (int t = 0; t < CNT; ++t) mma<CM>(dxa[k - 8][t], a, dq_[t]);
+            __builtin_amdgcn_sched_barrier(0);
+            RING_REFILL(k % D, k, hb, hbn);
+            __builtin_amdgcn_sched_barrier(0);
+        }
+    }
+    ASTAMP(28);
+    __syncthreads();
+    ASTAMP(29);
+    reduce_partials8(dxa, Gs, wave, r, q);
+    ASTAMP(30);
+    {
+        f32x4* dst = reinterpret_cast<f32x4*>(c.dy1);
+        for (int i = tid; i < S * (FD / 4); i += CT) {
+            const int o = (i >> 5) * LDX + ((i & 31) << 2);
+            const f32x4 a0 = *reinterpret_cast<const f32x4*>(Gs + o), a1 = *reinterpret_cast<const f32x4*>(B2 + o);
+            const f32x4 a2 = *reinterpret_cast<const f32x4*>(B3 + o), a3 = *reinterpret_cast<const f32x4*>(B4 + o);
+            dst[i] = (((a0 + a1) + a2) + a3) + *reinterpret_cast<const f32x4*>(B1 + o);
+        }
+    }
+    ASTAMP(31);
+}
+}
+
+template <int CM>
+__device__ __forceinline__ void ffn_fwd_loop(const FusedFwdParams& p, int l, f32x4 (&y)[8][CNT]) {
     extern __shared__ __attribute__((aligned(16))) float lds[];
     float* X1 = lds;
     float* R = lds + CBLK;
@@ -158,7 +348,6 @@
     const bool dev_seed = p.seed_ptr != nullptr;
     const uint64_t seed_dev = dev_seed ? *p.seed_ptr : 0ull;
     const uint64_t k_ffn = dev_seed ? site_key(seed_dev, l, SITE_FFN) : w.ffn_key;
-    const uint64_t k_res2 = dev_seed ? site_key(seed_dev, l, SITE_RES2) : w.res2_key;
 
     ASTAMP(16);
     Touched tch = {{0, 0, 0, 0}};
@@ -260,7 +449,6 @@
     }
 
     ASTAMP(17);
-    f32x4 y[8][CNT];
 #pragma unroll
     for (int i = 0; i < 8; ++i)
 #pragma unroll
@@ -379,8 +567,44 @@
     CSTAMP(5);
     CSTAMP_FLUSH(0);
     ASTAMP(18);
+}
+template <int CM, bool SPEC>
+__device__ __forceinline__ void ffn_fwd_finish(const FusedFwdParams& p, const FfnSpecParams& sp, int l, f32x4 (&y)[8][CNT]) {
+    extern __shared__ __attribute__((aligned(16))) float lds[];
+    float* X1 = lds;
+    float* R = lds + CBLK;
+    float* CP = lds + 5 * CBLK;
+    constexpr int D = RingDepth<CM>::v;
+    constexpr int ESZ = CM == CM_BF16 ? 2 : 4;
+    int tid_ = threadIdx.x;
+    if constexpr (SPEC) {
+        tid_ = (__builtin_amdgcn_readfirstlane(tid_ >> 6) << 6) | (int)__builtin_amdgcn_mbcnt_hi(~0u, __builtin_amdgcn_mbcnt_lo(~0u, 0u));
+    }
+    const int tid = tid_, wave = tid >> 6, lane = tid & 63, r = lane & 15, q = lane >> 4;
+    const int clip = blockIdx.x, S = p.S;
+    const size_t tokbase = (size_t)clip * S;
+    const FusedLayer& w = p.layer[l];
+    const uint64_t k_res2 = p.seed_ptr != nullptr ? site_key(*p.seed_ptr, l, SITE_RES2) : w.res2_key;
+    const int nhb = p.d_ff / 32, nht = p.d_ff / 16;
     __syncthreads();
     ASTAMP(19);
+    CutBwd cb;
+    WRaw<CM> bring[D];
+    uint32_t relu_word = 0;
+    if constexpr (SPEC) {
+        cb.lin2_wtp = sp.lin2_wtp; cb.lin1_wtp = sp.lin1_wtp;
+        cb.relu_bits = p.relu_bits + ((size_t)l * p.B + clip) * nhb * 64 + lane;
+        cb.g2_out = sp.g2_out;
+        cb.dhid_base = (char*)sp.dhid_out + ((size_t)l * p.B + clip) * CNT * nht * (size_t)(HTILE_ELEMS * ESZ);
+        cb.dy1 = sp.dy1 + tokbase * FD;
+        cb.pl = sp.partials + (size_t)clip * sp.P + l * FUSED_P_LAYER;
+        cb.S = S; cb.clip = clip; cb.B = p.B; cb.nhb = nhb; cb.xg_planes = sp.xg_planes;
+        cb.tok0 = tokbase; cb.k_res2 = k_res2; cb.res_thresh = w.res_thresh; cb.drop_inv = w.drop_inv; cb.eps = p.eps;
+        cut_bwd_walk<CM>(cb, wave, p.rot_mode);
+        __builtin_amdgcn_sched_barrier(0);
+        cut_bwd_prime<CM>(cb, bring, relu_word, lane);
+        __builtin_amdgcn_sched_barrier(0);
+    }
     reduce_partials8(y, R, wave, r, q);
     ASTAMP(20);
 
@@ -398,7 +622,7 @@
     }
     __syncthreads();
     ASTAMP(21);
-    const bool last = l + 1 == p.n_layers;
+    const bool last = SPEC || l + 1 == p.n_layers;
     float* Y = R;
     ln_rows(X1, S, CP, CP + FD, p.eps, [&](int row, int c0, float (&x)[32], float (&yv)[32]) {
         if (last && p.tokens_out && row < p.out_T) store32(p.tokens_out + ((size_t)clip * p.out_T + row) * FD + c0, yv);
@@ -406,17 +630,20 @@
     }, [&] { rows_from_lds(p.saved_res + ((size_t)(2 * l + 1) * p.B + clip) * S * FD, X1, S); });
     __syncthreads();
     ASTAMP(22);
-    if (!last) {
+    if (!SPEC && !last) {
         rows_from_lds(p.xin_out + ((size_t)(l + 1) * p.B + clip) * S * FD, Y, S);
         return;
     }
-    if (p.head.n_out > 0) {
-        float* pooled = X1;
+    if (SPEC || p.head.n_out > 0) {
+        float* pooled = SPEC ? R + 2 * CBLK : X1;
         const FusedCe ce{p.ce_target, p.ce_weight, p.ce_loss, p.ce_dlogits, p.ce_B, nullptr};
         CeReq rq;
-        if (ce.target) { ce_request_labels<CT>(ce, tid, rq); ce_request_weights(ce, p.head.n_out, rq); }
+        if (SPEC || ce.target) { ce_request_labels<CT>(ce, tid, rq); ce_request_weights(ce, p.head.n_out, rq); }
         if (tid < FD) pooled[tid] = colsum_lds(Y, 0, S, tid) * (1.f / (float)S);
-        if (ce.target) ce_weight_partials<CT>(ce, p.head.n_out, tid, rq, pooled + 256);
+        if (SPEC || ce.target) ce_weight_partials<CT>(ce, p.head.n_out, tid, rq, pooled + 256);
+        if constexpr (SPEC) {
+            for (int i = tid; i < (CSP - S) * LDX; i += CT) R[CBLK + S * LDX + i] = 0.f;
+        }
         __syncthreads();
         if (wave == 0) {
             float2 x = *reinterpret_cast<float2*>(pooled + 2 * lane);
@@ -434,11 +661,47 @@
                 if (lane == 0) p.logits_out[(size_t)clip * p.head.n_out + o] = sdot;
                 zmine = lane == o ? sdot : zmine;
             }
-            if (ce.target) ce_clip<CT>(ce, p.head.n_out, clip, lane, zmine, pooled + 256, true);
+            float dl = 0.f;
+            if (SPEC || ce.target) dl = ce_clip<CT>(ce, p.head.n_out, clip, lane, zmine, pooled + 256, true);
+            if constexpr (SPEC) {
+                if (sp.clocks && blockIdx.x == 0 && tid == 0) sp.clocks[1] = __builtin_amdgcn_s_memtime();
+                cut_head_bwd(p.head, CP, sp.partials + (size_t)clip * sp.P + sp.head_off, pooled + 128, S, lane, dx * rstd, dy * rstd, rstd, lw, y0, y1,
+                             [&](int o) { return __shfl(dl, o, 64); });
+            }
         }
     }
     ASTAMP(23);
-}
+    if constexpr (SPEC) {
+        __syncthreads();
+        const f32x4 dp = *reinterpret_cast<const f32x4*>(R + 2 * CBLK + 128 + ((tid & 31) << 2));
+        for (int i = tid; i < S * (FD / 4); i += CT) {
+            const int row = i >> 5, c = (i & 31) << 2;
+            *reinterpret_cast<f32x4*>(R + row * LDX + c) = dp;
+        }
+        __syncthreads();
+        cut_bwd_tail<CM>(cb, lds, bring, relu_word, tid);
+        if (tid == 0) sp.valid[clip] = 1u;
+        if (sp.clocks && blockIdx.x == 0 && tid == 0) sp.clocks[2] = __builtin_amdgcn_s_memtime();
+    }
+}
+template <int CM>
+__global__ __launch_bounds__(CT) void ffn_fwd_kernel(FusedFwdParams p, int l) {
+    f32x4 y[8][CNT];
+    ffn_fwd_loop<CM>(p, l, y);
+    ffn_fwd_finish<CM, false>(p, FfnSpecParams{}, l, y);
+}
+struct FfnFwdBwdArgs { FusedFwdParams p; FfnSpecParams sp; int l; };
+template <int CM>
+__global__ __launch_bounds__(CT) void ffn_fwd_bwd_kernel(FfnFwdBwdArgs a) {
+    if (a.sp.clocks && blockIdx.x == 0 && threadIdx.x == 0) a.sp.clocks[0] = __builtin_amdgcn_s_memtime();
+    f32x4 y[8][CNT];
+    ffn_fwd_loop<CM>(a.p, a.l, y);
+    const __attribute__((address_space(4))) char* ka = (const __attribute__((address_space(4))) char*)__builtin_amdgcn_kernarg_segment_ptr();
+    asm volatile("" : "+s"(ka));
+    const FfnFwdBwdArgs& b = *(const FfnFwdBwdArgs*)ka;
+    ffn_fwd_finish<CM, true>(b.p, b.sp, b.l, y);
+}
+
 
 template <int CM>
 __global__ __launch_bounds__(CT) void ffn_bwd_kernel(FusedBwdParams p, int l) {
@@ -446,11 +709,8 @@
     float* B1 = lds;
     float* Gs = lds + 1 * CBLK;
     float* B2 = lds + 2 * CBLK;
-    float* B3 = lds + 3 * CBLK;
-    float* B4 = lds + 4 * CBLK;
-    unsigned short* GP = reinterpret_cast<unsigned short*>(B3);
     constexpr int D = RingDepth<CM>::v;
-    const int tid = threadIdx.x, wave = tid >> 6, lane = tid & 63, r = lane & 15, q = lane >> 4;
+    const int tid = threadIdx.x, wave = tid >> 6, lane = tid & 63;
     const int clip = blockIdx.x, S = p.S;
     const size_t tok0 = (size_t)clip * S;
     const FusedBwdLayer& w = p.layer[l];
@@ -467,16 +727,25 @@
         const size_t b0 = (size_t)blockIdx.x * per, b1 = b0 + per < n4 ? b0 + per : n4;
         for (size_t k = b0 + threadIdx.x; k < b1; k += CT) reinterpret_cast<float4*>(p.zero_buf)[k] = make_float4(0, 0, 0, 0);
     }
+    if (p.spec_valid && last) {
+        if (p.spec_done && p.spec_valid[clip] && (p.d_logits_scale == nullptr || *p.d_logits_scale == 1.0f)) { touch_sink(tch); return; }
+        if (tid == 0) p.spec_valid[clip] = 0;
+    }
     float* part = p.partials + (size_t)clip * p.P;
     float* pl = part + l * FUSED_P_LAYER;
 
     const int nhb = p.d_ff / 32;
-    int j_begin_, n_mine_;
-    cut_walk<CM, false>(wave, nhb / 8, j_begin_, n_mine_, p.rot_mode >> 8);
-    const int nit = __builtin_amdgcn_readfirstlane(n_mine_), j_begin = __builtin_amdgcn_readfirstlane(j_begin_);
-    const int pair_s = __builtin_amdgcn_readfirstlane(wave & 3);
-    const int rot = cut_rot(p.rot_mode & 255, clip, nit);
-    auto hb_of = [&](int it) { int j = it + rot; if (j >= nit) j -= nit; return pair_s + 4 * (j_begin + j); };
+    constexpr int ESZ = CM == CM_BF16 ? 2 : 4;
+    CutBwd c;
+    c.lin2_wtp = w.lin2_wtp; c.lin1_wtp = w.lin1_wtp;
+    c.relu_bits = p.relu_bits + ((size_t)l * p.B + clip) * (size_t)nhb * 64 + lane;
+    c.g2_out = w.g2_out;
+    c.dhid_base = (char*)p.dhid_out + ((size_t)l * p.B + clip) * CNT * (nhb * 2) * (size_t)(HTILE_ELEMS * ESZ);
+    c.dy1 = p.dy1 + tok0 * FD;
+    c.pl = pl;
+    c.S = S; c.clip = clip; c.B = p.B; c.nhb = nhb; c.xg_planes = p.xg_planes;
+    c.tok0 = tok0; c.k_res2 = k_res2; c.res_thresh = w.res_thresh; c.drop_inv = w.drop_inv; c.eps = p.eps;
+    cut_bwd_walk<CM>(c, wave, p.rot_mode);
     float* CP = lds + 5 * CBLK;
     const bool cp_hd = p.head.n_out > 0 && last;
     const int cp_g = tid >> 5, cp_c4 = (tid & 31) << 2;
@@ -497,18 +766,9 @@
             if (p.head.n_out <= CP_HEAD_ROWS && tid >= 256 && tid < 256 + p.head.n_out * 32) *reinterpret_cast<f32x4*>(CP + 1024 + (tid - 256) * 4) = cp_w;
         }
     };
-    auto frag_load = [&](int k, int hb) -> WRaw<CM> {
-        return k < 8 ? load_w<CM>(w.lin2_wtp, hb * 2 + (k & 1), FD / 32, k >> 1, lane) : load_w<CM>(w.lin1_wtp, k - 8, nhb, hb, lane);
-    };
-    const uint32_t* relu_bits = p.relu_bits + ((size_t)l * p.B + clip) * (size_t)nhb * 64 + lane;
     WRaw<CM> ring[D];
     uint32_t relu_word;
-    {
-        const int hb0 = hb_of(0);
-#pragma unroll
-        for (int k = 0; k < D; ++k) ring[k] = frag_load(k, hb0);
-        relu_word = relu_bits[(size_t)hb0 * 64];
-    }
+    cut_bwd_prime<CM>(c, ring, relu_word, lane);
     const float* res2 = p.saved_res + ((size_t)(2 * l + 1) * p.B + clip) * S * FD;
     const bool head_bwd = last && p.head.n_out > 0;
     {
@@ -556,23 +816,7 @@
             float2 lw = *reinterpret_cast<const float2*>(CP + 3 * FD + 2 * lane);
             float2 lb = *reinterpret_cast<const float2*>(CP + 4 * FD + 2 * lane);
             float y0 = xh0 * lw.x + lb.x, y1 = xh1 * lw.y + lb.y;
-            float d0 = 0.f, d1 = 0.f;
-            const bool w_lds = p.head.n_out <= CP_HEAD_ROWS;
-            for (int o = 0; o < p.head.n_out; ++o) {
-                float go = CP[5 * FD + 64 + o];
-                float2 wv = w_lds ? *reinterpret_cast<const float2*>(CP + 1024 + o * FD + 2 * lane) : *reinterpret_cast<const float2*>(p.head.W + (size_t)o * FD + 2 * lane);
-                d0 += go * wv.x; d1 += go * wv.y;
-                *reinterpret_cast<float2*>(hp + 256 + FUSED_HEAD_MAX_OUT + o * FD + 2 * lane) = make_float2(go * y0, go * y1);
-                if (lane == 0) hp[256 + o] = go;
-            }
-            *reinterpret_cast<float2*>(hp + 2 * lane) = make_float2(d0 * xh0, d1 * xh1);
-            *reinterpret_cast<float2*>(hp + 128 + 2 * lane) = make_float2(d0, d1);
-            float g0 = d0 * lw.x, g1 = d1 * lw.y;
-            float s1 = wsum(g0 + g1) * (1.f / FD);
-            float s2 = wsum(g0 * xh0 + g1 * xh1) * (1.f / FD);
-            float inv_s = 1.f / (float)S;
-            *reinterpret_cast<float2*>(pooled + 128 + 2 * lane) =
-                make_float2(rstd * (g0 - s1 - xh0 * s2) * inv_s, rstd * (g1 - s1 - xh1 * s2) * inv_s);
+            cut_head_bwd(p.head, CP, hp, pooled + 128, S, lane, xh0, xh1, rstd, lw, y0, y1, [&](int o) { return CP[5 * FD + 64 + o]; });
         }
         __syncthreads();
         f32x4 dp[1];
@@ -589,128 +833,7 @@
     }
     __syncthreads();
     ASTAMP(26);
-    ln_bwd_rows(S, CP, p.eps,
-        [&](int row, int c0, float (&dy)[32], float (&x)[32]) { load32(Gs + row * LDX + c0, dy); load32(B1 + row * LDX + c0, x); },
-        [&](int row, int c0, float (&dy)[32], float (&dx)[32], float (&dyx)[32]) {
-            store32(B1 + row * LDX + c0, dx);
-            store32(B3 + row * LDX + c0, dyx);
-            if (w.res_thresh) {
-                const uint32_t orow = (uint32_t)(tok0 + row);
-#pragma unroll
-                for (int j = 0; j < 32; ++j) dx[j] *= drop_scale(k_res2, orow, (uint32_t)(c0 + j), w.res_thresh, w.drop_inv);
-            }
-            store32(B2 + row * LDX + c0, dx);
-        });
-    __syncthreads();
-    if (tid < 128) pl[0 + tid] = colsum_lds(B3, 0, S, tid);
-    else if (tid < 256) pl[128 + (tid - 128)] = colsum_lds(Gs, 0, S, tid - 128);
-    else if (tid < 384) pl[256 + (tid - 256)] = colsum_lds(B2, 0, S, tid - 256);
-    if (!(CM != CM_F32 && p.xg_planes)) rows_from_lds(w.g2_out + tok0 * FD, B2, S);
-    __syncthreads();
-    if constexpr (CM == CM_SPLIT) block_to_split_planes(GP, B2);
-    else if constexpr (CM == CM_BF16) block_to_plane(GP, B2);
-    __syncthreads();
-    if (CM != CM_F32 && p.xg_planes) {
-        if constexpr (CM == CM_SPLIT) {
-            const size_t plane = (size_t)p.B * CSP * FD;
-            planes_from_lds<3>(reinterpret_cast<unsigned short*>(w.g2_out) + (size_t)clip * CSP * FD, plane, GP);
-        } else {
-            planes_from_lds<1>(reinterpret_cast<unsigned short*>(w.g2_out) + (size_t)clip * CSP * FD, 0, GP);
-        }
-    }
-
-    ASTAMP(27);
-    f32x4 dxa[8][CNT];
-#pragma unroll
-    for (int i = 0; i < 8; ++i)
-#pragma unroll
-        for (int t = 0; t < CNT; ++t) dxa[i][t] = f32x4{0, 0, 0, 0};
-    constexpr int ESZ = CM == CM_BF16 ? 2 : 4;
-    const int nht = p.d_ff / 16;
-    char* const dhid_base = (char*)p.dhid_out + ((size_t)l * p.B + clip) * CNT * nht * (size_t)(HTILE_ELEMS * ESZ);
-    for (int it = 0; it < nit; ++it) {
-        const int hb = hb_of(it);
-        const int hbn = hb_of(it + 1 < nit ? it + 1 : it);
-        __builtin_amdgcn_sched_barrier(0);
-        f32x4 dacc[2][CNT];
-#pragma unroll
-        for (int i = 0; i < 2; ++i)
-#pragma unroll
-            for (int t = 0; t < CNT; ++t) dacc[i][t] = f32x4{0, 0, 0, 0};
-        Frag<CM> gb[CNT];
-#pragma unroll
-        for (int k = 0; k < 8; ++k) {
-            const int i = k & 1, kb = k >> 1;
-            if (i == 0) {
-#pragma unroll
-                for (int t = 0; t < CNT; ++t) gb[t] = operand_frag<CM>(GP, B2, t * 16 + r, kb * 32, q);
-            }
-            pin(ring[k % D]);
-            Frag<CM> a2 = w_frag<CM>(ring[k % D]);
-#pragma unroll
-            for (int t = 0; t < CNT; ++t) mma<CM>(dacc[i][t], a2, gb[t]);
-            __builtin_amdgcn_sched_barrier(0);
-            RING_REFILL(k % D, k, hb, hbn);
-            __builtin_amdgcn_sched_barrier(0);
-        }
-        const uint32_t bits = relu_word;
-        __builtin_amdgcn_sched_barrier(0);
-        relu_word = relu_bits[(size_t)hbn * 64];
-        __builtin_amdgcn_sched_barrier(0);
-#pragma unroll
-        for (int i = 0; i < 2; ++i)
-#pragma unroll
-            for (int t = 0; t < CNT; ++t)
-#pragma unroll
-                for (int e = 0; e < 4; ++e) {
-                    const int k = (i * CNT + t) * 4 + e;
-                    const int32_t m = ((int32_t)(bits << (31 - k))) >> 31;
-                    dacc[i][t][e] = __uint_as_float(__float_as_uint(dacc[i][t][e]) & (uint32_t)m);
-                }
-        Frag<CM> dq_[CNT];
-#pragma unroll
-        for (int t = 0; t < CNT; ++t) dq_[t] = chain_frag<CM>(dacc[0][t], dacc[1][t]);
-        {
-            char* hb_base = dhid_base + (size_t)hb * 2 * (HTILE_ELEMS * ESZ);
-#pragma unroll
-            for (int t = 0; t < CNT; ++t) {
-                if constexpr (CM == CM_BF16) {
-                    const u32x4 u = __builtin_bit_cast(u32x4, dq_[t].v);
-                    store_hid_tile_bf16(hb_base + (size_t)t * nht * (HTILE_ELEMS * ESZ), u, lane, S - t * 16);
-                } else {
-#pragma unroll
-                    for (int i = 0; i < 2; ++i)
-                        store_hid_tile<CM>(hb_base + ((size_t)t * nht + i) * (HTILE_ELEMS * ESZ), dacc[i][t], lane, S - t * 16);
-                }
-            }
-        }
-        __builtin_amdgcn_sched_barrier(0);
-#pragma unroll
-        for (int k = 8; k < 16; ++k) {
-            pin(ring[k % D]);
-            Frag<CM> a = w_frag<CM>(ring[k % D]);
-#pragma unroll
-            for (int t = 0; t < CNT; ++t) mma<CM>(dxa[k - 8][t], a, dq_[t]);
-            __builtin_amdgcn_sched_barrier(0);
-            RING_REFILL(k % D, k, hb, hbn);
-            __builtin_amdgcn_sched_barrier(0);
-        }
-    }
-    ASTAMP(28);
-    __syncthreads();
-    ASTAMP(29);
-    reduce_partials8(dxa, Gs, wave, r, q);
-    ASTAMP(30);
-    {
-        f32x4* dst = reinterpret_cast<f32x4*>(p.dy1 + tok0 * FD);
-        for (int i = tid; i < S * (FD / 4); i += CT) {
-            const int o = (i >> 5) * LDX + ((i & 31) << 2);
-            const f32x4 a0 = *reinterpret_cast<const f32x4*>(Gs + o), a1 = *reinterpret_cast<const f32x4*>(B2 + o);
-            const f32x4 a2 = *reinterpret_cast<const f32x4*>(B3 + o), a3 = *reinterpret_cast<const f32x4*>(B4 + o);
-            dst[i] = (((a0 + a1) + a2) + a3) + *reinterpret_cast<const f32x4*>(B1 + o);
-        }
-    }
-    ASTAMP(31);
+    cut_bwd_tail<CM>(c, lds, ring, relu_word, tid);
 }
 
 bool ffn_cut_supported(int d_ff) { return d_ff % 256 == 0 && d_ff >= 256; }
@@ -731,6 +854,23 @@
     return 0;
 }
 template <int CM>
+static int launch_cut_fwd_bwd(const FusedFwdParams& p, FfnSpecParams sp, int l, hipStream_t st) {
+    const size_t lds = ffn_cut_lds_bytes();
+    static bool attr_set = false;
+    if (!attr_set) {
+        EGX_HIP(hipFuncSetAttribute(reinterpret_cast<const void*>(&ffn_fwd_bwd_kernel<CM>), hipFuncAttributeMaxDynamicSharedMemorySize, (int)lds));
+        attr_set = true;
+    }
+    sp.clocks = timing_clocks();
+    timing_begin(TIMER_FFN_FWD_BWD, st);
+    FfnFwdBwdArgs a;
+    a.p = p; a.sp = sp; a.l = l;
+    hipLaunchKernelGGL((ffn_fwd_bwd_kernel<CM>), dim3(p.B), dim3(CT), lds, st, a);
+    timing_end(TIMER_FFN_FWD_BWD, st);
+    EGX_LAUNCH_CHECK();
+    return 0;
+}
+template <int CM>
 static int launch_cut_bwd(const FusedBwdParams& p, int l, hipStream_t st) {
     const size_t lds = ffn_cut_lds_bytes();
     static bool attr_set = false;
@@ -738,9 +878,10 @@
         EGX_HIP(hipFuncSetAttribute(reinterpret_cast<const void*>(&ffn_bwd_kernel<CM>), hipFuncAttributeMaxDynamicSharedMemorySize, (int)lds));
         attr_set = true;
     }
-    timing_begin(TIMER_FFN_BWD, st);
+    const bool timed = !p.spec_done;
+    if (timed) timing_begin(TIMER_FFN_BWD, st);
     hipLaunchKernelGGL((ffn_bwd_kernel<CM>), dim3(p.B), dim3(CT), lds, st, p, l);
-    timing_end(TIMER_FFN_BWD, st);
+    if (timed) timing_end(TIMER_FFN_BWD, st);
     EGX_LAUNCH_CHECK();
     return 0;
 }
@@ -750,6 +891,13 @@
     EGX_CHECK(p.x1f_out && p.xin_out && p.saved_res && p.relu_bits && p.hid_out, "ffn_cut_forward: missing buffers");
     return compute == CM_BF16 ? launch_cut_fwd<CM_BF16>(p, l, st) : compute == CM_SPLIT ? launch_cut_fwd<CM_SPLIT>(p, l, st) : launch_cut_fwd<CM_F32>(p, l, st);
 }
+int ffn_cut_forward_backward(const FusedFwdParams& p, const FfnSpecParams& sp, int l, int compute, hipStream_t st) {
+    EGX_CHECK(ffn_cut_supported(p.d_ff) && p.S <= CSP && l + 1 == p.n_layers, "ffn_cut_forward_backward: d_ff=%d S=%d layer %d of %d", p.d_ff, p.S, l, p.n_layers);
+    EGX_CHECK(p.x1f_out && p.saved_res && p.relu_bits && p.hid_out, "ffn_cut_forward_backward: missing buffers");
+    EGX_CHECK(p.head.n_out > 0 && p.ce_target && p.ce_dlogits, "ffn_cut_forward_backward: needs the pooled head and the fused cross entropy");
+    EGX_CHECK(sp.lin2_wtp && sp.lin1_wtp && sp.g2_out && sp.dhid_out && sp.dy1 && sp.partials && sp.valid, "ffn_cut_forward_backward: missing backward buffers");
+    return compute == CM_BF16 ? launch_cut_fwd_bwd<CM_BF16>(p, sp, l, st) : compute == CM_SPLIT ? launch_cut_fwd_bwd<CM_SPLIT>(p, sp, l, st) : launch_cut_fwd_bwd<CM_F32>(p, sp, l, st);
+}
 int ffn_cut_backward(const FusedBwdParams& p, int l, int compute, hipStream_t st) {
     EGX_CHECK(ffn_cut_supported(p.d_ff) && p.S <= CSP && l >= 0 && l < p.n_layers, "ffn_cut_backward: d_ff=%d S=%d layer %d", p.d_ff, p.S, l);
     EGX_CHECK(p.dy1 && p.saved_res && p.relu_bits && p.dhid_out && p.partials && (l + 1 == p.n_layers || p.dxin), "ffn_cut_backward: missing buffers");
diff --git a/egot2_amd/csrc/fused.h b/egot2_amd/csrc/fused.h
--- a/egot2_amd/csrc/fused.h
+++ b/egot2_amd/csrc/fused.h
@@ -82,6 +82,14 @@
     TouchList touch;
     const int* rtab; int B_clips;
 };
+struct FfnSpecParams {
+    const void* lin2_wtp; const void* lin1_wtp;
+    float* g2_out; void* dhid_out; float* dy1;
+    float* partials; int P, head_off;
+    int xg_planes;
+    unsigned* valid;
+    unsigned long long* clocks;
+};
 enum { FUSED_MODE_FULL = 0, FUSED_MODE_PRE = 1, FUSED_MODE_POST = 2, FUSED_MODE_ATTN = 3 };
 
 struct PackDesc {
@@ -181,6 +189,8 @@
     float* dy1;
     float* dxin;
     const float* d_logits_scale;
+    int spec_done;
+    unsigned* spec_valid;
     const float* tce_W; const float* tce_dlogits; int tce_C;
     TouchList touch;
     const int* rtab; int B_clips; const int* rseg;
@@ -190,6 +200,7 @@
 size_t ffn_cut_lds_bytes();
 int ffn_cut_forward(const FusedFwdParams& p, int l, int compute, hipStream_t st);
 int ffn_cut_backward(const FusedBwdParams& p, int l, int compute, hipStream_t st);
+int ffn_cut_forward_backward(const FusedFwdParams& p, const FfnSpecParams& sp, int l, int compute, hipStream_t st);
 
 struct SmallDwProblem {
     const float* G; const float* X; float* out;
@@ -216,7 +227,8 @@
 int tail_reduce(const SmallDwParams* sp, const SlabReduce* red, const ReducePartialsParams* rp, uint64_t* seed_advance_ptr, const TouchList* touch, hipStream_t st);
 
 enum { TIMER_FUSED_FWD = 0, TIMER_FUSED_BWD = 1, TIMER_FFN_DW = 2, TIMER_FFN_FWD = 3, TIMER_FFN_BWD = 4, TIMER_WIDE_GEMM = 5,
-       TIMER_WIDE_ATTN_FWD = 6, TIMER_WIDE_ATTN_BWD = 7, TIMER_COUNT = 8 };
+       TIMER_WIDE_ATTN_FWD = 6, TIMER_WIDE_ATTN_BWD = 7, TIMER_FFN_FWD_BWD = 8, TIMER_COUNT = 9 };
+unsigned long long* timing_clocks();
 void timing_enable(int on);
 void timing_begin(int which, hipStream_t st);
 void timing_end(int which, hipStream_t st);
diff --git a/egot2_amd/csrc/fused.hip b/egot2_amd/csrc/fused.hip
--- a/egot2_amd/csrc/fused.hip
+++ b/egot2_amd/csrc/fused.hip
@@ -1092,10 +1092,16 @@
 TimerSlot g_timers[TIMER_COUNT];
 int g_timing_on = 0;
 constexpr int TIMER_MAX_EVENTS = 4096;
+unsigned long long* g_split_clocks = nullptr;
 }
 void timing_enable(int on) {
     g_timing_on = on;
     for (int i = 0; i < TIMER_COUNT; ++i) g_timers[i].n = 0;
+    if (on && !g_split_clocks && hipMalloc(&g_split_clocks, sizeof(unsigned long long) * 3 * TIMER_MAX_EVENTS) != hipSuccess) g_split_clocks = nullptr;
+}
+unsigned long long* timing_clocks() {
+    const int n = g_timers[TIMER_FFN_FWD_BWD].n;
+    return g_timing_on && g_split_clocks && n < TIMER_MAX_EVENTS ? g_split_clocks + 3 * (size_t)n : nullptr;
 }
 void timing_begin(int which, hipStream_t st) {
     if (!g_timing_on) return;
@@ -1122,8 +1128,22 @@
         if (hipEventSynchronize(t.b[i]) != hipSuccess || hipEventElapsedTime(&ms, t.a[i], t.b[i]) != hipSuccess) return 1;
         tot += ms;
     }
+    int n = t.n;
+    if ((which == TIMER_FFN_FWD || which == TIMER_FFN_BWD) && g_split_clocks) {
+        TimerSlot& m = g_timers[TIMER_FFN_FWD_BWD];
+        std::vector<unsigned long long> ck(3 * (size_t)m.n);
+        for (int i = 0; i < m.n; ++i) {
+            float ms = 0.f;
+            if (hipEventSynchronize(m.b[i]) != hipSuccess || hipEventElapsedTime(&ms, m.a[i], m.b[i]) != hipSuccess) return 1;
+            if (i == 0 && hipMemcpy(ck.data(), g_split_clocks, ck.size() * sizeof(unsigned long long), hipMemcpyDeviceToHost) != hipSuccess) return 1;
+            const double fwd = (double)(ck[3 * i + 1] - ck[3 * i]), all = (double)(ck[3 * i + 2] - ck[3 * i]);
+            const double share = all > 0 ? fwd / all : 0.5;
+            tot += ms * (which == TIMER_FFN_FWD ? share : 1.0 - share);
+        }
+        n += m.n;
+    }
     if (total_ms) *total_ms = tot;
-    if (count) *count = t.n;
+    if (count) *count = n;
     return 0;
 }
 
diff --git a/egot2_amd/csrc/fused_dev.h b/egot2_amd/csrc/fused_dev.h
--- a/egot2_amd/csrc/fused_dev.h
+++ b/egot2_amd/csrc/fused_dev.h
@@ -335,7 +335,7 @@
     if ((tid & 63) == 0) red[tid >> 6] = s;
 }
 template <int NTHREADS>
-__device__ __forceinline__ void ce_clip(const FusedCe& ce, int n_out, int clip, int lane, float z, const float* red, bool add_loss) {
+__device__ __forceinline__ float ce_clip(const FusedCe& ce, int n_out, int clip, int lane, float z, const float* red, bool add_loss) {
     float wtot = 0.f;
 #pragma unroll
     for (int w = 0; w < NTHREADS / 64; ++w) wtot += red[w];
@@ -348,7 +348,8 @@
     const float s = wsum(e);
     const float zy = __shfl(zl, valid ? (int)y : 0, 64);
     const float k = wy / wtot;
-    if (lane < n_out) ce.d_logits[(size_t)clip * n_out + lane] = valid ? k * (e / s - (lane == (int)y ? 1.f : 0.f)) : 0.f;
+    const float dl = lane < n_out ? (valid ? k * (e / s - (lane == (int)y ? 1.f : 0.f)) : 0.f) : 0.f;
+    if (lane < n_out) ce.d_logits[(size_t)clip * n_out + lane] = dl;
     if (lane == 0 && add_loss) {
         float term = valid ? k * (m + __logf(s) - zy) : 0.f;
         if (wtot == 0.f && clip == 0) term = __builtin_nanf("");
@@ -364,6 +365,7 @@
             }
         }
     }
+    return dl;
 }
 
 
diff --git a/egot2_amd/csrc/fused_host.hip b/egot2_amd/csrc/fused_host.hip
--- a/egot2_amd/csrc/fused_host.hip
+++ b/egot2_amd/csrc/fused_host.hip
@@ -84,11 +84,34 @@
     return compute == EGX_F32_SPLIT && pl.L == 1 && pl.dff >= 1024;
 }
 static int fused_slices_layout(const Plan& pl);
+int fused_slices(const Plan& pl, int compute);
 static size_t sliced_xchg_bytes(const Plan& pl, int n);
 static size_t sliced_flag_bytes(const Plan& pl, int n);
-static size_t fused_saved_bytes(const egx_config* cfg, const egx_segment* segs, const Plan& pl) {
+static size_t fused_saved_base_bytes(const egx_config* cfg, const egx_segment* segs, const Plan& pl) {
     const int n = (pl.tpc > 1 || pl.S > FUSED_TOK_PAD) ? 1 : fused_slices_layout(pl);
     return fused_core_bytes(cfg, segs, pl) + sliced_xchg_bytes(pl, n) + sliced_flag_bytes(pl, n);
+}
+static bool spec_layout_on(const egx_config* cfg, const Plan& pl) {
+    if (!cfg->speculate_bwd || cfg->deterministic || pl.tpc > 1 || pl.S > FUSED_TOK_PAD) return false;
+    return use_cut(pl, fused_slices(pl, cfg->compute), false, cfg->compute);
+}
+static size_t spec_g2_bytes(const Plan& pl) { return (size_t)pl.vB * FUSED_TOK_PAD * pl.d * 6; }
+struct SpecLayout { size_t g2, dhid, dy1, partials, valid, end; };
+static SpecLayout spec_layout(const egx_config* cfg, const egx_segment* segs, const Plan& pl, int P) {
+    SpecLayout s;
+    size_t cur = align_up(fused_saved_base_bytes(cfg, segs, pl), 256);
+    s.g2 = take(cur, spec_g2_bytes(pl));
+    s.dhid = take(cur, fused_hid_total(cfg, pl));
+    s.dy1 = take(cur, pl.N * pl.d * 4);
+    s.partials = take(cur, (size_t)pl.vB * P * 4);
+    s.valid = take(cur, (size_t)pl.vB * 4);
+    s.end = cur;
+    return s;
+}
+static int spec_partial_len(const Plan& pl, int head_n_out) { return fused_partial_len(pl.L, pl.nseg) + fused_head_partial_len(head_n_out); }
+static size_t fused_saved_bytes(const egx_config* cfg, const egx_segment* segs, const Plan& pl) {
+    if (spec_layout_on(cfg, pl)) return spec_layout(cfg, segs, pl, spec_partial_len(pl, FUSED_HEAD_MAX_OUT)).end;
+    return fused_saved_base_bytes(cfg, segs, pl);
 }
 static int device_cus() {
     static int cus[64] = {0};
@@ -169,18 +192,19 @@
     size_t ffn_slab[FUSED_MAX_LAYERS];
     int P;
 };
-static size_t bwd_scratch_prefix(FusedBwdScratch& s, const egx_config* cfg, const egx_segment* segs, const Plan& pl, const size_t* seg_rows, int head_n_out) {
+static size_t bwd_scratch_prefix(FusedBwdScratch& s, const egx_config* cfg, const egx_segment* segs, const Plan& pl, const size_t* seg_rows, int head_n_out,
+                                 bool spec = false) {
     memset(&s, 0, sizeof(s));
     size_t cur = 0;
     const size_t nd = pl.N * pl.d * 4;
     const size_t nd3 = (size_t)pl.vB * FUSED_TOK_PAD * pl.d * 6;
     for (int l = 0; l < pl.L && l < FUSED_MAX_LAYERS; ++l) {
-        s.x1[l] = take(cur, nd); s.g2[l] = take(cur, nd3); s.attn_o[l] = take(cur, nd);
+        s.x1[l] = take(cur, nd); s.g2[l] = take(cur, spec && l + 1 == pl.L ? 0 : nd3); s.attn_o[l] = take(cur, nd);
         s.g1[l] = take(cur, nd); s.dqkv[l] = take(cur, 3 * nd);
     }
     for (int i = 0; i < pl.nseg; ++i) s.dseg[i] = take(cur, seg_rows[i] * pl.d * 4);
     s.P = fused_partial_len(pl.L, pl.nseg) + fused_head_partial_len(head_n_out);
-    s.partials = take(cur, (size_t)pl.vB * s.P * 4);
+    s.partials = take(cur, spec ? 0 : (size_t)pl.vB * s.P * 4);
     size_t slab = ffn_dw_scratch_bytes((int)pl.N, pl.dff, nullptr);
     slab = size_max(slab, gemm_scratch_bytes(2, 3 * pl.d, pl.d, (int)pl.N));
     slab = size_max(slab, gemm_scratch_bytes(2, pl.d, pl.d, (int)pl.N));
@@ -192,14 +216,14 @@
     for (int l = 1; l < pl.L && l < FUSED_MAX_LAYERS; ++l) s.ffn_slab[l] = take(cur, ffn_dw_scratch_bytes((int)pl.N, pl.dff, nullptr));
     s.sdw_bytes = (size_t)(512 + SMALL_DW_MAX * 16) * 64 * 128 * sizeof(float);
     s.sdw_tiles = take(cur, s.sdw_bytes);
-    s.dhid = take(cur, fused_hid_total(cfg, pl));
+    s.dhid = take(cur, spec ? 0 : fused_hid_total(cfg, pl));
     return cur;
 }
 static FusedBwdScratch fused_bwd_scratch(const egx_config* cfg, const egx_segment* segs, const Plan& pl, int head_n_out = 0) {
     FusedBwdScratch s;
     size_t seg_rows[EGX_MAX_SEGMENTS];
     for (int i = 0; i < pl.nseg; ++i) seg_rows[i] = (size_t)pl.B * segs[i].T;
-    size_t cur = bwd_scratch_prefix(s, cfg, segs, pl, seg_rows, head_n_out);
+    size_t cur = bwd_scratch_prefix(s, cfg, segs, pl, seg_rows, head_n_out, spec_layout_on(cfg, pl));
     const size_t nd = pl.N * pl.d * 4;
     s.dx0 = take(cur, nd);
     s.dy1 = take(cur, nd); s.dxin = take(cur, nd);
@@ -495,7 +519,7 @@
     fp.seed_ptr = cfg->seed_ptr; fp.layer = l;
     const size_t lo = (size_t)l * fused_hid_bytes(vp.vB, vp.dff, comp == EGX_BF16);
     fp.hs = v.base + fused_hid_offset(cfg, segs, vp) + lo;
-    fp.dhs = (const char*)scratch + SC.dhid + lo;
+    fp.dhs = (const char*)bp.dhid_out + lo;
     fp.B = vp.vB;
     fp.xg_planes = bp.xg_planes;
     if (fp.xg_planes) fp.x1 = (const float*)(v.base + fused_x1p_offset(cfg, segs, vp) + (size_t)l * vp.vB * FUSED_TOK_PAD * vp.d * plane_elem_bytes(cfg));
@@ -596,18 +620,35 @@
     if (pack_weights(pk, st)) return 1;
     const bool touch = cfg->weight_cache != nullptr;
     const size_t ffn_pb = packed_bytes(pl.dff, d, comp), in_pb = packed_bytes(3 * d, d, comp), out_pb = packed_bytes(d, d, comp);
+    const bool spec = cut && spec_layout_on(cfg, pl);
+    EGX_CHECK(!spec || (ce_fused && with_head), "egx_config.speculate_bwd needs the pooled head and the fused cross entropy (egx_config.ce)");
     if (cut) {
         fp.mode = FUSED_MODE_ATTN;
         for (int l = 0; l < pl.L; ++l) {
+            const bool spec_l = spec && l + 1 == pl.L;
             fp.l0 = l;
             memset(&fp.touch, 0, sizeof(fp.touch));
             if (touch) { touch_add(fp.touch, PL.layer[l].lin1_w, ffn_pb); touch_add(fp.touch, PL.layer[l].lin2_w, ffn_pb); }
+            if (touch && spec_l) { touch_add(fp.touch, PL.layer[l].lin2_wt, ffn_pb); touch_add(fp.touch, PL.layer[l].lin1_wt, ffn_pb); }
             if (fused_forward(fp, comp, st)) return 1;
             fp.zero_word = nullptr;
             memset(&fp.touch, 0, sizeof(fp.touch));
             if (touch && l + 1 < pl.L) { touch_add(fp.touch, PL.layer[l + 1].in_w, in_pb); touch_add(fp.touch, PL.layer[l + 1].out_w, out_pb); }
+            else if (touch && spec_l) { touch_add(fp.touch, PL.layer[l].out_wt, out_pb); touch_add(fp.touch, PL.layer[l].in_wt, in_pb); }
             else if (touch && training) { touch_add(fp.touch, PL.layer[l].lin2_wt, ffn_pb); touch_add(fp.touch, PL.layer[l].lin1_wt, ffn_pb); }
-            if (ffn_cut_forward(fp, l, comp, st)) return 1;
+            if (spec_l) {
+                const int P = spec_partial_len(pl, head->n_out);
+                const SpecLayout SL = spec_layout(cfg, segs, vp, P);
+                char* sv = (char*)saved;
+                FfnSpecParams sp;
+                memset(&sp, 0, sizeof(sp));
+                sp.lin2_wtp = PL.layer[l].lin2_wt; sp.lin1_wtp = PL.layer[l].lin1_wt;
+                sp.g2_out = (float*)(sv + SL.g2); sp.dhid_out = sv + SL.dhid; sp.dy1 = (float*)(sv + SL.dy1);
+                sp.partials = (float*)(sv + SL.partials); sp.P = P; sp.head_off = fused_partial_len(pl.L, pl.nseg);
+                sp.xg_planes = split_planes(cfg) ? 1 : 0;
+                sp.valid = (unsigned*)(sv + SL.valid);
+                if (ffn_cut_forward_backward(fp, sp, l, comp, st)) return 1;
+            } else if (ffn_cut_forward(fp, l, comp, st)) return 1;
         }
     } else {
         if (touch) {
@@ -654,6 +695,18 @@
         bp.d_logits_scale = cfg->d_logits_scale;
         bp.head_off = fused_partial_len(pl.L, pl.nseg);
     }
+    const bool spec = !tiled && spec_layout_on(cfg, pl);
+    float* spec_dy1 = nullptr;
+    if (spec) {
+        EGX_CHECK(with_head, "egx_config.speculate_bwd: the forward of this backward had the pooled head");
+        const SpecLayout SL = spec_layout(cfg, segs, vp, SC.P);
+        char* sv = (char*)const_cast<void*>(saved);
+        bp.layer[pl.L - 1].g2_out = (float*)(sv + SL.g2);
+        bp.dhid_out = sv + SL.dhid;
+        bp.partials = (float*)(sv + SL.partials);
+        bp.spec_valid = (unsigned*)(sv + SL.valid);
+        spec_dy1 = (float*)(sv + SL.dy1);
+    }
     const int stage = cfg->bwd_stage;
     EGX_CHECK(stage >= 0 && stage <= 2, "bwd_stage=%d", stage);
     if (stage == 2) bp.zero_buf = nullptr;
@@ -670,6 +723,7 @@
         bp.cut = 1; bp.dy1 = fptr(scratch, SC.dy1); bp.dxin = fptr(scratch, SC.dxin);
         for (int l = pl.L - 1; l >= 0; --l) {
             bp.cut_layer = l;
+            if (spec) { bp.dy1 = l + 1 == pl.L ? spec_dy1 : fptr(scratch, SC.dy1); bp.spec_done = (l + 1 == pl.L && cfg->spec_done) ? 1 : 0; }
             memset(&bp.touch, 0, sizeof(bp.touch));
             if (touch) { touch_add(bp.touch, PL.layer[l].out_wt, out_pb); touch_add(bp.touch, PL.layer[l].in_wt, in_pb); }
             if (ffn_cut_backward(bp, l, comp, st)) return 1;
diff --git a/egot2_amd/functional.py b/egot2_amd/functional.py
--- a/egot2_amd/functional.py
+++ b/egot2_amd/functional.py
@@ -69,6 +69,7 @@
     wcache: Optional[WeightCache] = None
     token_ce: int = 0
     ce: bool = False
+    speculate_backward: bool = True
 
     def config(self) -> Config:
         return Config(self.d_model, self.n_heads, self.d_ff, self.n_layers, len(self.segments), float(self.ln_eps),
@@ -451,6 +452,8 @@
             if nhead or lib.egx_encoder_impl(C.byref(probe), segs, B) != EGX_IMPL_FUSED:
                 py_slice, spec = spec.out_tokens, full
         cfg = spec.config()
+        ctx.speculated = bool(spec.speculate_backward and spec.ce and nhead and any(nig))
+        cfg.speculate_bwd = int(ctx.speculated)
         sv, sc = C.c_size_t(0), C.c_size_t(0)
         ws = lib.egx_translator_workspace if nhead else lib.egx_encoder_workspace
         check(ws(C.byref(cfg), segs, B, C.byref(sv), C.byref(sc)))
@@ -507,10 +510,12 @@
                 return (None,) * len(ctx.needs_input_grad)
             dl_scale = _f32c(d_loss)
             d_tokens = ctx.tce_dl
+        spec_done = False
         if spec.ce:
             up = _ce_upstream(ctx, d_tokens, d_loss)
             if up is None:
                 return (None,) * len(ctx.needs_input_grad)
+            spec_done = ctx.speculated and d_tokens is None
             d_tokens, dl_scale = up
         if ctx.py_slice:
             full = torch.zeros((d_tokens.shape[0], ctx.S, d_tokens.shape[2]), dtype=torch.float32, device=d_tokens.device)
@@ -529,6 +534,7 @@
 
         cfg = spec.config()
         gr.attach(cfg)
+        cfg.speculate_bwd, cfg.spec_done = int(ctx.speculated), int(spec_done)
         if ctx.wcache_buf is not None:
             cfg.weight_cache = ctx.wcache_buf.data_ptr()
         if dl_scale is not None:
@@ -596,6 +602,7 @@
         if defer:
             cfg2 = spec.config()
             cfg2.bwd_stage = 2
+            cfg2.speculate_bwd = int(ctx.speculated)
             if ctx.wcache_buf is not None:
                 cfg2.weight_cache = ctx.wcache_buf.data_ptr()
             keep = (flat_buf, tensors, dtok, scratch, saved_buf)
diff --git a/egot2_amd/translator.py b/egot2_amd/translator.py
--- a/egot2_amd/translator.py
+++ b/egot2_amd/translator.py
@@ -48,6 +48,7 @@
     egx_impl: str = "auto"
     egx_defer_small: bool = False
     egx_deterministic: bool = False
+    egx_speculate_backward: bool = True
     _egx_step: int = 0
 
     def set_compute(self, compute: str = "f32", impl: str = "auto"):
@@ -57,6 +58,10 @@
 
     def set_deterministic(self, on: bool = True):
         self.egx_deterministic = bool(on)
+        return self
+
+    def set_speculate_backward(self, on: bool = True):
+        self.egx_speculate_backward = bool(on)
         return self
 
     def enable_weight_cache(self, frozen: bool = False):
@@ -113,7 +118,8 @@
                                               seed_ptr=seed_dev.data_ptr() if seed_dev is not None else 0,
                                               advance_seed=adv,
                                               defer_small=bool(self.egx_defer_small), deterministic=bool(self.egx_deterministic),
-                                              out_tokens=int(out_tokens), wcache=wcache, ce=ce is not None)
+                                              out_tokens=int(out_tokens), wcache=wcache, ce=ce is not None,
+                                              speculate_backward=bool(self.egx_speculate_backward))
         if ce is not None and head is None:
             raise ValueError("the fused cross entropy needs the pooled head")
         if token_ce is not None:
diff --git a/include/egot2x.h b/include/egot2x.h
--- a/include/egot2x.h
+++ b/include/egot2x.h
@@ -93,6 +93,8 @@
     const float* d_logits_scale;
     const struct egx_ce* ce;
     const struct egx_token_ce* token_ce;
+    int speculate_bwd;
+    int spec_done;
 } egx_config;
 
 typedef struct egx_ce {
```

Measured after the change: 697,000 clips/s. About the same (-0.7%).
